# maxnorman569/Variational-Gridded-Gaussian-Processes

Hardware: AMD Instinct MI355X
Metric: ELBO-step grid-points/sec (value + 5-component gradient), 1024x1024 RBF grid per GPU (higher is better)
Workload: dtype f64; 1 GPU; 2D Kronecker rbf GP (points basis), 1024x1024 grid (1024x1024 per GPU), m_d=128, Adam fit loop (lr 0.01), eigensolver warm start on; parallelism=single GPU

## Files before the change

### variational_gridded_gaussian_processes_amd/build.py

```python
from __future__ import annotations

import os
import shutil
import subprocess
import sys

HERE = os.path.dirname(os.path.abspath(__file__))
CSRC = os.path.join(HERE, "csrc")
SOURCES = ["api.hip", "gemm.hip", "factor_build.hip", "chol.hip", "trsm.hip", "eigh.hip", "mspace.hip", "thin.hip", "masked.hip", "comm.hip", "paired.hip"]
HEADERS = ["common.h", "ctx.h", "factor_elem.h", "gemm_body.h", os.path.join("..", "..", "include", "vggp.h")]
LIB = os.path.join(HERE, "libvggp_hip.so")


def _stale() -> bool:
    if not os.path.exists(LIB):
        return True
    t = os.path.getmtime(LIB)
    deps = [os.path.join(CSRC, s) for s in SOURCES] + [os.path.normpath(os.path.join(CSRC, h)) for h in HEADERS]
    return any(os.path.getmtime(d) > t for d in deps)


def build(force: bool = False, verbose: bool = False) -> str:
    if not force and not _stale():
        return LIB
    hipcc = shutil.which("hipcc") or "/opt/rocm/bin/hipcc"
    if not os.path.exists(hipcc):
        raise RuntimeError("hipcc not found: libvggp_hip.so cannot be built (ROCm toolchain required)")
    cmd = [hipcc, "--offload-arch=gfx950", "-O3", "-std=c++17", "-shared", "-fPIC", "-o", LIB + ".tmp"] + \
          [os.path.join(CSRC, s) for s in SOURCES] + ["-ldl"]
    if verbose:
        print(" ".join(cmd), file=sys.stderr)
    subprocess.run(cmd, check=True, cwd=CSRC)
    os.replace(LIB + ".tmp", LIB)
    return LIB


if __name__ == "__main__":
    print(build(force="--force" in sys.argv, verbose=True))
```

### variational_gridded_gaussian_processes_amd/csrc/api.hip

```cpp
#include "common.h"

#include <math.h>
#include <stdarg.h>
#include <stdio.h>
#include <stdlib.h>
#include <string.h>
#include <time.h>

#include <algorithm>
#include <vector>

static thread_local char g_err[512] = "";
void vg_set_error(const char* fmt, ...) {
    va_list ap;
    va_start(ap, fmt);
    vsnprintf(g_err, sizeof(g_err), fmt, ap);
    va_end(ap);
}
extern "C" const char* vggp_last_error(void) { return g_err; }
extern "C" int vggp_version(void) { return VGGP_VERSION; }

#include "ctx.h"
#include "factor_elem.h"
#define VG_CHOL_MAXJOBS_HOST 8
// ... 167 lines not shown
    c->P3 = b.take<double>(3 * m1 * m2);
    c->T3 = b.take<double>(3 * m1 * m2);
    for (int k = 0; k < 2; ++k) {
        VgDim& d = c->d[k];
        const long m = d.m;
        d.TM = b.take<double>(m * m);
        d.TH = b.take<double>(m * m);
        d.Qt = b.take<double>(m * m);
        d.QtPrev = b.take<double>(m * m);
        d.QtPrev2 = b.take<double>(m * m);
        d.U = b.take<double>(m * m);
        d.Ep = b.take<double>(m * m);
        d.Fp = b.take<double>(m * m);
        d.Wp = b.take<double>(m * m);
        d.Id = b.take<double>(m * m);
        d.Gw = b.take<double>(m * m);
        d.GH = b.take<double>(2 * m * m);
        d.Mk = b.take<double>(m * m);
    }
    c->payload_len = 2 * m2 * m2 + 3 * m1 * m2;
    c->payload = b.take<double>(c->payload_len + 8);
    for (int k = 0; k < 2; ++k) {
        VgDim& d = c->d[k];
        const long m = d.m;
        const int glen = (int)vg_grid_len(d.basis, m);
        d.grid = b.take<double>(glen);
        d.K0 = b.take<double>(m * m);
        d.dK0 = b.take<double>(m * m);
        d.L0 = b.take<double>(m * m);
        d.Linv0 = b.take<double>(m * m);
        d.Dinv0 = b.take<double>(((m + 15) / 16) * 256);
        if (m > 128) {
            d.Kc = b.take<double>(4 * m * m); d.Lc = b.take<double>(4 * m * m); d.Dc = b.take<double>(4 * ((m + 15) / 16) * 256);
            d.st8 = b.take<int>(8);
        }
        d.X = b.take<double>(m * m);
        d.chol_scratch = b.take<double>(m * (m + 1));
        d.RQ = b.take<double>(m * m);
        d.RQsq = b.take<double>(m * m);
    }
    c->wq = b.take<double>(2 * m1 * m2);
    for (int k = 0; k < 2; ++k) {
        VgDim& d = c->d[k];
        const long m = d.m, n = d.n, m2e = m + (m & 1);
        d.x = b.take<double>(n);
        d.AD = b.take<double>(2 * m * n);
        d.BV = b.take<double>(2 * m * n);
        static const char* ghe = getenv("VGGP_GH_TARGET");
        d.gh_split = pick_split((int)(((m + 63) / 64) * ((m + 63) / 64)), (int)n, ghe ? atoi(ghe) : 32);
        d.GHslab = b.take<double>((size_t)d.gh_split * 2 * m * m);
        d.gwork = b.take<double>(m2e * (m2e + 1));
        d.max_rounds = (int)(VG_EIG_MAXSWEEP * (m2e - 1));
        d.rotlog = b.take<double2>(vg_eigh_log_bytes((int)m) / sizeof(double2) + 1);
        d.roundlog = b.take<int>(d.max_rounds);
        if (m >= 24 && m <= 256) {
            d.gwork2 = b.take<double>(m2e * (m2e + 1));
            d.rotlog2 = b.take<double2>(vg_eigh_log_bytes((int)m) / sizeof(double2) + 1);
            d.roundlog2 = b.take<int>(d.max_rounds);
            d.Zs = b.take<double>(m * m); d.V1s = b.take<double>(m * m); d.Hs = b.take<double>(m * m); d.Ws = b.take<double>(m * m);
            d.tMV = b.take<double>(VG_THIN_MAXR * m); d.tHV = b.take<double>(VG_THIN_MAXR * m);
            d.tAM = b.take<double>(VG_THIN_MAXR * VG_THIN_MAXR); d.tAH = b.take<double>(VG_THIN_MAXR * VG_THIN_MAXR);
            d.Omega = b.take<double>(VG_THIN_MAXR * m);
        }
    }
    const int st_tiles = (int)(((2 * m2 + 63) / 64) * ((n1 + 63) / 64));
    static const char* ste = getenv("VGGP_ST_TARGET");
    c->st_split = pick_split(st_tiles, (int)n2, ste ? atoi(ste) : 256);
    c->St = b.take<double>((size_t)std::max(c->st_split, VG_SP_SLABS) * 2 * m2 * n1);
    c->Sp = b.take<double>((size_t)VG_SP_SLABS * 2 * m2 * n1);
    const int cc_tiles = (int)(((2 * m1 + 63) / 64) * ((m2 + 63) / 64));
    const char* cce = getenv("VGGP_CC_TARGET");
    c->cc_split = pick_split(cc_tiles, (int)n1, cce ? atoi(cce) : 64);
    c->CCslab = b.take<double>((size_t)c->cc_split * 3 * m1 * m2);
    c->tCV = b.take<double>(3 * m1 * VG_THIN_MAXR);
    c->tAC = b.take<double>(3 * VG_THIN_MAXR * VG_THIN_MAXR + 64);
}

static int check_dim(int kind, int basis, long n, long m, const char* which) {
    VG_REQUIRE(kind >= 0 && kind <= 3, "vggp_plan: bad kind for %s", which);
    VG_REQUIRE(basis >= 0 && basis <= 4, "vggp_plan: bad basis for %s", which);
    VG_REQUIRE(!((basis == VGGP_BASIS_VFF || basis == VGGP_BASIS_B1) && kind != VGGP_KIND_MATERN12),
               "vggp_plan: the VFF and B1 features exist for Matern-1/2 only (%s)", which);
    VG_REQUIRE(!(basis == VGGP_BASIS_VFF && (m < 3 || (m & 1) == 0)), "vggp_plan: VFF needs m = 2M + 1 >= 3 (%s)", which);
    VG_REQUIRE(!(basis == VGGP_BASIS_B1 && m < 2), "vggp_plan: B1 needs at least 2 knots (%s)", which);
    VG_REQUIRE(!(basis == VGGP_BASIS_B0 && kind != VGGP_KIND_MATERN12),
               "vggp_plan: the B0 basis exists for Matern-1/2 only (%s)", which);
    VG_REQUIRE(n >= 1, "vggp_plan: %s has no observations", which);
    VG_REQUIRE(m >= 1 && m <= 256, "vggp_plan: m=%ld for %s outside [1, 256]", m, which);
    VG_REQUIRE(!(basis == VGGP_BASIS_ONE && m != 1), "vggp_plan: BASIS_ONE needs m=1 (%s)", which);
    return VGGP_OK;
}

extern "C" int vggp_plan(vggp_ctx* c, const vggp_desc* desc) {
    if (!c || !desc) { vg_set_error("vggp_plan: null argument"); return VGGP_EINVAL; }
    VG_ENTER_DEVICE(c->device);
    int rc;
    if (desc->flags & VGGP_FLAG_PAIRED_Z) {
        c->planned = false;
        graphs_clear(c);
        VG_HIP(hipDeviceSynchronize());
        c->have_partials = c->have_step = c->have_masked = false;
        c->acc_valid = false; c->last_payload = nullptr;
        c->is_paired = false;
        if ((rc = vg_paired_plan(c, desc))) return rc;
        c->desc = *desc;
        c->desc.x1 = c->desc.x2 = c->desc.grid1 = c->desc.grid2 = nullptr;
        c->desc.n_total = (desc->flags & VGGP_FLAG_SCATTERED) ? desc->n1 : desc->n1 * desc->n2;
        c->payload_len = 0;
        c->is_paired = true;
        c->planned = true;
        return VGGP_OK;
    }
    if (c->is_paired || c->paired) { VG_HIP(hipDeviceSynchronize()); vg_paired_free(c); c->is_paired = false; }
    if ((rc = check_dim(desc->kind1, desc->basis1, desc->n1, desc->m1, "dimension 1"))) return rc;
    if ((rc = check_dim(desc->kind2, desc->basis2, desc->n2, desc->m2, "dimension 2"))) return rc;
    VG_REQUIRE(desc->x1 && desc->x2, "vggp_plan: null coordinate arrays");
    VG_REQUIRE((desc->basis1 == VGGP_BASIS_ONE || desc->grid1) && (desc->basis2 == VGGP_BASIS_ONE || desc->grid2),
               "vggp_plan: null grid arrays");
    if (desc->flags & VGGP_FLAG_SCATTERED)
        VG_REQUIRE(desc->n1 == desc->n2 && desc->basis1 != VGGP_BASIS_ONE && desc->basis2 != VGGP_BASIS_ONE,
                   "vggp_plan: scattered points need n1 == n2 (one coordinate pair per point) and two real dimensions");
    else
        VG_REQUIRE(desc->n_total >= desc->n1 * desc->n2, "vggp_plan: n_total smaller than the local grid");
    VG_REQUIRE(desc->n1 < (1L << 24) && desc->n2 < (1L << 24), "vggp_plan: grid axis too long");
    c->planned = false;
    graphs_clear(c);
    VG_HIP(hipDeviceSynchronize());
    c->warm_run = 0;
    c->refine_next = false;
    c->sub_next = false; c->sub_mode = false; c->sub_r_cap[0] = c->sub_r_cap[1] = 0;
    c->pred_consumed = false;
    c->acc_valid = false; c->last_warm = false; c->last_slabs = false; c->last_payload = nullptr;
    c->last_thin = false; c->thin_off = false; c->thin_block = 0;
    c->cur_newton = 0; c->last_newton = false; c->newton_next = false; c->newton_block = 0; c->newton_iters = 3; c->newton_ok_run = 0;
    c->desc = *desc;
    c->d[0] = VgDim();
    c->d[1] = VgDim();
    c->d[0].kind = desc->kind1; c->d[0].basis = desc->basis1; c->d[0].n = (int)desc->n1; c->d[0].m = (int)desc->m1;
    c->d[1].kind = desc->kind2; c->d[1].basis = desc->basis2; c->d[1].n = (int)desc->n2; c->d[1].m = (int)desc->m2;
    Bump dry{nullptr, 0, true};
    layout(c, dry);
    const size_t need = dry.off + 4096;
    if (need > c->arena_bytes) {
        if (c->arena) { VG_HIP(hipFree(c->arena)); c->arena = nullptr; c->arena_bytes = 0; }
        VG_HIP(hipMalloc(&c->arena, need));
        c->arena_bytes = need;
    }
    Bump wet{reinterpret_cast<char*>(c->arena), 0, false};
    layout(c, wet);
    c->arena_used = wet.off;
    VG_HIP(hipMemset(c->arena, 0, c->arena_used));
    const double one = 1.0;
    for (int k = 0; k < 2; ++k) {
        VgDim& d = c->d[k];
        const double* hx = k == 0 ? desc->x1 : desc->x2;
        const double* hg = k == 0 ? desc->grid1 : desc->grid2;
        VG_HIP(hipMemcpy(d.x, hx, sizeof(double) * d.n, hipMemcpyHostToDevice));
        if (d.basis == VGGP_BASIS_ONE) {
            VG_HIP(hipMemcpy(d.grid, &one, sizeof(double), hipMemcpyHostToDevice));
        } else {
            const int glen = (int)vg_grid_len(d.basis, d.m);
            VG_HIP(hipMemcpy(d.grid, hg, sizeof(double) * glen, hipMemcpyHostToDevice));
        }
    }
    for (int k = 0; k < 2; ++k) VG_HIP(vg_identity_launch(c->d[k].Id, c->d[k].m, nullptr));
    for (int k = 0; k < 2; ++k) {
        VgDim& d = c->d[k];
        if (!d.Omega) continue;
        std::vector<double> om((size_t)VG_THIN_MAXR * d.m);
        unsigned long long z = 0x9E3779B97F4A7C15ull * (unsigned long long)(k + 1);
        for (double& v : om) {
            z += 0x9E3779B97F4A7C15ull;
            unsigned long long x = z;
            x = (x ^ (x >> 30)) * 0xBF58476D1CE4E5B9ull; x = (x ^ (x >> 27)) * 0x94D049BB133111EBull; x ^= x >> 31;
            v = (double)(x >> 11) * (2.0 / 9007199254740992.0) - 1.0;
        }
        VG_HIP(hipMemcpy(d.Omega, om.data(), sizeof(double) * om.size(), hipMemcpyHostToDevice));
    }
    VG_HIP(hipDeviceSynchronize());
    c->desc.x1 = c->desc.x2 = c->desc.grid1 = c->desc.grid2 = nullptr;
    c->have_partials = c->have_step = c->have_masked = false;
    vg_masked_new_plan(c);
    c->planned = true;
    return VGGP_OK;
}

extern "C" int vggp_set_inducing(vggp_ctx* c, int dim, const double* z, int64_t m) {
    if (c && c->is_paired) {
        if (!c->planned) { vg_set_error("context not planned"); return VGGP_ESTATE; }
        VG_ENTER_DEVICE(c->device);
        return vg_paired_set_inducing(c, dim, z, m);
    }
    if (!c || !c->planned) { vg_set_error("vggp_set_inducing: context not planned"); return VGGP_ESTATE; }
    VG_REQUIRE(dim == 0 || dim == 1, "vggp_set_inducing: dim must be 0 or 1");
    VgDim& d = c->d[dim];
    VG_REQUIRE(d.basis == VGGP_BASIS_POINTS, "vggp_set_inducing: dimension %d does not use the points basis", dim + 1);
    VG_REQUIRE(z && m == d.m, "vggp_set_inducing: expected %d coordinates, got %lld", d.m, (long long)m);
    for (int64_t i = 0; i < m; ++i) VG_REQUIRE(std::isfinite(z[i]), "vggp_set_inducing: z[%lld] is not finite", (long long)i);
    VG_ENTER_DEVICE(c->device);
    VG_HIP(hipStreamSynchronize(c->own_stream));
    VG_HIP(hipMemcpy(d.grid, z, sizeof(double) * m, hipMemcpyHostToDevice));
    c->have_step = false; c->have_partials = false; c->have_masked = false; c->acc_valid = false;
    return VGGP_OK;
}

extern "C" int64_t vggp_payload_len(const vggp_ctx* c) { return (c && c->planned) ? c->payload_len : 0; }
extern "C" int64_t vggp_workspace_bytes(const vggp_ctx* c) { return c ? (int64_t)c->arena_used : 0; }

static int trsm_batch(const VgTrsmSpec* sp, int n, hipStream_t st) {
    int max_nblk = 0;
    for (int j = 0; j < n; ++j) max_nblk = std::max(max_nblk, (int)((sp[j].m + VG_TRSM_BLK - 1) / VG_TRSM_BLK));
    for (int s = 0; s < max_nblk; ++s) {
        VgGemmBatch g;
        vg_gemm_init(&g);
        VgTrsmJob tj[12];
        int nt = 0;
        for (int j = 0; j < n; ++j) {
            const VgTrsmSpec& q = sp[j];
            const int nblk = (int)((q.m + VG_TRSM_BLK - 1) / VG_TRSM_BLK);
            if (s >= nblk) continue;
            const int b = q.trans ? nblk - 1 - s : s;
            const long r0 = (long)b * VG_TRSM_BLK, rb = std::min<long>(VG_TRSM_BLK, q.m - r0), r1 = r0 + rb;
            const long k0 = q.trans ? r1 : 0, kn = q.trans ? q.m - r1 : r0;
            if (kn > 0) {
                const double* Tp = q.trans ? q.L + k0 * q.ldl + r0 : q.L + r0 * q.ldl + k0;
                const long t_i = q.trans ? 1 : q.ldl, t_k = q.trans ? q.ldl : 1;
                if (q.sc == 1)
                    vg_gemm_add(&g, Tp, t_i, t_k, q.X + k0 * q.sk, q.sk, 1, q.X + r0 * q.sk, (int)q.sk, (int)rb, (int)q.ncols, (int)kn,
                                1, 0, 1, 0, -1.0, 1);
                else
                    vg_gemm_add(&g, q.X + k0, q.sc, 1, Tp, t_k, t_i, q.X + r0, (int)q.sc, (int)q.ncols, (int)rb, (int)kn, 1, 0, 1, 0,
                                -1.0, 1);
            }
            if (nt >= 12) { vg_set_error("trsm_batch: too many jobs"); return VGGP_EINVAL; }
            tj[nt++] = VgTrsmJob{q.L + r0 * q.ldl + r0, q.Dinv + (r0 / 16) * q.dinv_blk, q.X + r0 * q.sk, q.X + r0 * q.sk, q.ldl,
                                 q.dinv_blk, q.dinv_ld, q.sk, q.sc, q.sk, q.sc, q.ncols, (int)rb, q.trans};
        }
        if (g.nprob) VG_HIP(vg_gemm_launch(&g, st));
        if (nt) VG_HIP(vg_trsm_launch(tj, nt, st));
    }
    return VGGP_OK;
}
static int trsm_inplace(const double* L, long m, long ldl, const double* Dinv, double* X, long x_sk, long x_sc, long ncols,
                        int trans, hipStream_t st) {
    VgTrsmSpec q{L, ldl, Dinv, 256, 16, X, x_sk, x_sc, ncols, m, trans};
    return trsm_batch(&q, 1, st);
}

static bool vg_ride(const vggp_ctx* c) {
    static const bool off = getenv("VGGP_NO_RIDE") != nullptr;
    return !off && !c->prof && c->desc.m1 <= 128 && c->desc.m2 <= 128;
}

static int vg_chol_big_enqueue(vggp_ctx* c, const int* dims, int ndims, hipStream_t st) {
    VgCholJob cj[VG_CHOL_MAXJOBS_HOST];
    int nj = 0;
    for (int t = 0; t < ndims; ++t) {
        VgDim& d = c->d[dims[t]];
        VG_HIP(vg_jitcopy_launch(d.K0, d.m, d.Kc, st));
    }
    const long NB = 128;
    for (int stage = 0; stage < 2; ++stage) {
        if (stage == 1) {
            VgTrsmJob tj[8];
            int nt = 0;
            VgGemmBatch g;
            vg_gemm_init(&g);
            for (int t = 0; t < ndims; ++t) {
                VgDim& d = c->d[dims[t]];
                const long m = d.m, mm = m * m, rest = m - NB, nb16 = (m + 15) / 16;
                for (int l = 0; l < 4; ++l) {
                    double* Kl = d.Kc + l * mm;
                    double* Ll = d.Lc + l * mm;
                    tj[nt++] = VgTrsmJob{Ll, d.Dc + l * nb16 * 256, Kl + NB * m, Ll + NB * m, m, 256, 16, 1, m, 1, m, rest, (int)NB, 0};
                    vg_gemm_add(&g, Ll + NB * m, m, 1, Ll + NB * m, 1, m, Kl + NB * m + NB, (int)m, (int)rest, (int)rest, (int)NB, 1, 0, 1, 0, -1.0, 1);
                }
            }
            VG_HIP(vg_trsm_launch(tj, nt, st));
            VG_HIP(vg_gemm_launch(&g, st));
        }
        nj = 0;
        for (int t = 0; t < ndims; ++t) {
            VgDim& d = c->d[dims[t]];
            const long m = d.m, mm = m * m, nb16 = (m + 15) / 16;
            const long o = stage ? NB : 0;
            const int mb = stage ? (int)(m - NB) : (int)NB;
            for (int l = 0; l < 4; ++l) {
                VgCholJob j{d.Kc + l * mm + o * m + o, d.Lc + l * mm + o * m + o, nullptr, d.chol_scratch, nullptr, d.st8 + 2 * l + stage, mb};
                j.ldk = (int)m; j.ldl = (int)m; j.only_level0 = 1;
                j.Dinv_out = d.Dc + l * nb16 * 256 + (o / 16) * 256;
                cj[nj++] = j;
            }
        }
        VG_HIP(vg_chol_launch(cj, nj, st));
    }
    for (int t = 0; t < ndims; ++t) {
        VgDim& d = c->d[dims[t]];
        VG_HIP(vg_cholsel_launch(d.Lc, d.Dc, d.st8, d.m, d.L0, d.Dinv0, d.jitter, d.status, st));
    }
    return VGGP_OK;
}

int vg_partials_enqueue(vggp_ctx* c, const double* Y, double* payload, hipStream_t st, bool reduce, bool extrap, bool fused, bool apply_ns,
                        int early) {
    const long n1 = c->desc.n1, n2 = c->desc.n2, m1 = c->desc.m1, m2 = c->desc.m2;
    VgDim &d1 = c->d[0], &d2 = c->d[1];
    hipStream_t sx = vg_side(c, st);
    VgGemmBatch g;
    VG_MARK(-1);

    VgFactorJob fj[2];
    VgCholJob cj[2];
    static const bool chol_legacy = getenv("VGGP_CHOL_LEGACY") != nullptr;
    const bool dinv_path = d1.m <= VG_TRSM_BLK && d2.m <= VG_TRSM_BLK && !chol_legacy;
    VgClearArgs clr;
    clr.n = 0;
    for (int k = 0; k < 2; ++k) {
        VgDim& d = c->d[k];
        fj[k] = VgFactorJob{d.x, d.grid, d.AD, d.AD + (long)d.m * d.n, d.K0, d.dK0, d.n, d.m, d.kind, d.basis, k, 0.0, c->desc.flags};
        clr.ptr[clr.n] = d.status; clr.nwords[clr.n++] = 2;
        clr.ptr[clr.n] = reinterpret_cast<int*>(d.chol_scratch); clr.nwords[clr.n++] = 16;
        clr.ptr[clr.n] = d.counters; clr.nwords[clr.n++] = 8;
        if (k == 0) { clr.ptr[clr.n] = reinterpret_cast<int*>(c->payload + c->payload_len); clr.nwords[clr.n++] = 2; }
        if (d.st8) { clr.ptr[clr.n] = d.st8; clr.nwords[clr.n++] = 8; }
        cj[k] = VgCholJob{d.K0, d.L0, dinv_path ? nullptr : d.Linv0, d.chol_scratch, d.jitter, d.status, d.m};
        cj[k].Dinv_out = d.Dinv0;
    }
    VG_HIP(vg_factor_build_launch(fj, 2, c->d_htheta, st, c->theta, &clr));
    VG_MARK(0);

    const bool ns_on_chol = extrap && apply_ns && dinv_path;
    VgGemmBatch gns;
    vg_gemm_init(&gns);
    if (ns_on_chol)
        for (int k = 0; k < 2; ++k) {
            VgDim& d = c->d[k];
            vg_gemm_add(&gns, d.Wp, d.m, 1, d.Ep, d.m, 1, d.Fp, d.m, d.m, d.m, d.m, 1, 0, 1, 0, -0.5, 1);
        }
    static const bool chol_big_off = getenv("VGGP_NO_CHOL_BIG") != nullptr;
    const bool any_big = (d1.m > VG_TRSM_BLK || d2.m > VG_TRSM_BLK) && !chol_legacy && !chol_big_off;
    VgGemmBatch gsp;
    vg_gemm_init(&gsp);
    int sp_slabs = 1;
    if (early) {
        const bool ok_fused = fused && !reduce && (vg_ride(c) || c->prof);
        const bool ok_partials = reduce;
        if (!(dinv_path && !any_big && (ok_fused || ok_partials) && Y && sx == st)) {
            vg_set_error("internal: the early projection was requested where it cannot run");
            return VGGP_ESTATE;
        }
        vg_gemm_add(&gsp, d2.AD, n2, 1, Y, n1, 1, c->Sp, (int)n1, (int)(2 * m2), (int)n1, (int)n2, std::min(c->st_split, VG_SP_SLABS), 2L * m2 * n1);
        sp_slabs = gsp.p[0].ksplit;
        if (c->prof) {
            vg_gemm_xcd_group(&gsp, 0);
            VG_HIP(vg_gemm_launch(&gsp, st, VG_GEMM_TAG_GRAM_PROJECT));
            VG_MARK(4);
        }
    }
    if (!any_big) {
        VgGemmBatch gr2 = gns;
        if (early && !c->prof) {
            gr2 = gsp;
            if (ns_on_chol)
                for (int k = 0; k < 2; ++k) {
                    VgDim& d = c->d[k];
                    vg_gemm_add(&gr2, d.Wp, d.m, 1, d.Ep, d.m, 1, d.Fp, d.m, d.m, d.m, d.m, 1, 0, 1, 0, -0.5, 1);
                }
        }
        VG_HIP(vg_chol_launch(cj, 2, st, ((early && !c->prof) || ns_on_chol) ? &gr2 : nullptr));
    } else {
        int big[2], nbig = 0;
        for (int k = 0; k < 2; ++k) {
            if (c->d[k].m > VG_TRSM_BLK) big[nbig++] = k;
            else { cj[k].Linv = nullptr; VG_HIP(vg_chol_launch(&cj[k], 1, st)); }
        }
        const int rcb = vg_chol_big_enqueue(c, big, nbig, st);
        if (rcb) return rcb;
    }
    c->dinv_valid = dinv_path || any_big;
    VG_MARK(1);

    {
        const bool big = d1.m > VG_TRSM_BLK || d2.m > VG_TRSM_BLK;
        if (!big) {
            VgTrsmJob tj[16];
            int nt = 0;
            for (int k = 0; k < 2; ++k) {
                VgDim& d = c->d[k];
                const long mn = (long)d.m * d.n;
                const double* dv = dinv_path ? d.Dinv0 : d.Linv0;
                const long dblk = dinv_path ? 256 : 16L * d.m + 16, dld = dinv_path ? 16 : d.m;
                for (int b = 0; b < 2; ++b)
                    tj[nt++] = VgTrsmJob{d.L0, dv, d.AD + b * mn, d.BV + b * mn, d.m, dblk, dld, d.n, 1, d.n, 1, d.n, d.m, 0};
                tj[nt++] = VgTrsmJob{d.L0, dv, d.dK0, d.X, d.m, dblk, dld, d.m, 1, d.m, 1, d.m, d.m, 0};
                if (dinv_path) {
                    tj[nt] = VgTrsmJob{d.L0, dv, d.L0, d.Linv0, d.m, dblk, dld, d.m, 1, d.m, 1, d.m, d.m, 0};
                    tj[nt++].rhs_ident = 1;
                }
            }
            if (early)
                for (int sl = 0; sl < sp_slabs; ++sl)
                    for (int b = 0; b < 2; ++b) {
                        const long o = (long)sl * 2 * m2 * n1 + (long)b * m2 * n1;
                        tj[nt++] = VgTrsmJob{d2.L0, d2.Dinv0, c->Sp + o, c->St + o, m2, 256, 16, n1, 1, n1, 1, n1, (int)m2, 0};
                    }
            VG_HIP(vg_trsm_launch(tj, nt, st));
        } else {
            VgTrsmSpec q[8];
            int nq = 0;
            for (int k = 0; k < 2; ++k) {
                VgDim& d = c->d[k];
                const long mn = (long)d.m * d.n;
                const double* dv = any_big ? d.Dinv0 : d.Linv0;
                const long dblk = any_big ? 256 : 16L * d.m + 16, dld = any_big ? 16 : d.m;
                VG_HIP(hipMemcpyAsync(d.BV, d.AD, sizeof(double) * 2 * mn, hipMemcpyDeviceToDevice, st));
                VG_HIP(hipMemcpyAsync(d.X, d.dK0, sizeof(double) * d.m * d.m, hipMemcpyDeviceToDevice, st));
                for (int b = 0; b < 2; ++b) q[nq++] = VgTrsmSpec{d.L0, d.m, dv, dblk, dld, d.BV + b * mn, d.n, 1, d.n, d.m, 0};
                q[nq++] = VgTrsmSpec{d.L0, d.m, dv, dblk, dld, d.X, d.m, 1, d.m, d.m, 0};
                if (any_big) {
                    VG_HIP(hipMemcpyAsync(d.Linv0, d.Id, sizeof(double) * d.m * d.m, hipMemcpyDeviceToDevice, st));
                    q[nq++] = VgTrsmSpec{d.L0, d.m, dv, dblk, dld, d.Linv0, d.m, 1, d.m, d.m, 0};
                }
            }
            const int rc = trsm_batch(q, nq, st);
            if (rc) return rc;
        }
    }
    VG_MARK(2);

    if (!Y) {
        vg_gemm_init(&g);
        for (int k = 0; k < 2; ++k) {
            VgDim& d = c->d[k];
            vg_gemm_add(&g, d.X, d.m, 1, d.Linv0, 1, d.m, d.Mk, d.m, d.m, d.m, d.m);
        }
        VG_HIP(vg_gemm_launch(&g, st));
        return VGGP_OK;
    }
    hipStream_t sp = (fused && !extrap) ? sx : st;
    const bool ride = fused && !reduce && sp == st && vg_ride(c);
    if (sp != st) VG_FORK(1);
    VgGemmBatch gp, gc;
    vg_gemm_init(&gp);
    vg_gemm_add(&gp, d2.BV, n2, 1, Y, n1, 1, c->St, (int)n1, (int)(2 * m2), (int)n1, (int)n2, c->st_split, 2L * m2 * n1);
    const int st_slabs = early ? sp_slabs : gp.p[0].ksplit;
    vg_gemm_xcd_group(&gp, 0);
    auto add_ns = [&](VgGemmBatch* b) {
        if (extrap && apply_ns && !ns_on_chol)
            for (int k = 0; k < 2; ++k) {
                VgDim& d = c->d[k];
                vg_gemm_add(b, d.Wp, d.m, 1, d.Ep, d.m, 1, d.Fp, d.m, d.m, d.m, d.m, 1, 0, 1, 0, -0.5, 1);
            }
    };
    if (!ride && !early) {
        add_ns(&gp);
        VG_HIP(vg_gemm_launch(&gp, sp, VG_GEMM_TAG_GRAM_PROJECT));
        if (sp == st) VG_MARK(4);
    }
    vg_gemm_init(&gc);
    const long cc_slab = 3L * m1 * m2;
    vg_gemm_add(&gc, d1.BV, n1, 1, c->St, 1, n1, c->CCslab, (int)m2, (int)(2 * m1), (int)m2, (int)n1, c->cc_split, cc_slab,
                st_slabs, 2L * m2 * n1);
    vg_gemm_add(&gc, d1.BV, n1, 1, c->St + m2 * n1, 1, n1, c->CCslab + 2 * m1 * m2, (int)m2, (int)m1, (int)m2, (int)n1,
                c->cc_split, cc_slab, st_slabs, 2L * m2 * n1);
    const int cc_slabs = gc.p[0].ksplit;
    int gh_slabs[2] = {1, 1};
    auto add_gram = [&](VgGemmBatch* b) {
        for (int k = 0; k < 2; ++k) {
            VgDim& d = c->d[k];
            const int ig = vg_gemm_add(b, d.BV, d.n, 1, d.BV, 1, d.n, d.GHslab, d.m, 2 * d.m, d.m, d.n, d.gh_split, 2L * d.m * d.m);
            gh_slabs[k] = b->p[ig].ksplit;
            vg_gemm_add(b, d.X, d.m, 1, d.Linv0, 1, d.m, d.Mk, d.m, d.m, d.m, d.m);
        }
    };
    if (ride) {
        vg_gemm_init(&g);
        add_gram(&g);
        add_ns(&g);
        VG_HIP(vg_gemm_launch(&g, st));
        c->ride_proj = gp; c->ride_cc = gc;
        c->ride_pending = early != 1;
        c->ride_stage0 = early == 2 ? 1 : 0;
    } else {
        if (sp == st) add_gram(&gc);
        VG_HIP(vg_gemm_launch(&gc, sp));
        if (sp == st) { VG_MARK(5); VG_MARK(6); }
        if (sp != st) {
            VG_JOIN_RECORD(1);
            vg_gemm_init(&g);
            add_gram(&g);
            VG_HIP(vg_gemm_launch(&g, st));
            VG_MARK(6);
        }
    }

    c->gh_slabs[0] = gh_slabs[0]; c->gh_slabs[1] = gh_slabs[1]; c->cc_slabs = cc_slabs; c->st_slabs = st_slabs;
    if (!reduce) return VGGP_OK;
    if (sp != st) VG_JOIN_WAIT(1);
    VgRedBatch r;
    vg_red_init(&r);
    vg_red_add(&r, d1.GHslab, d1.GH, 2L * m1 * m1, 2L * m1 * m1, gh_slabs[0]);
    vg_red_add(&r, d2.GHslab, payload, 2L * m2 * m2, 2L * m2 * m2, gh_slabs[1]);
    vg_red_add(&r, c->CCslab, payload + 2 * m2 * m2, 3L * m1 * m2, cc_slab, cc_slabs);
    VG_HIP(vg_red_launch(&r, st));
    VG_MARK(7);
    return VGGP_OK;
}

static bool vg_sub_ident() { static const bool ex = getenv("VGGP_SUB_EXTRAP") != nullptr; return !ex; }

static int finish_enqueue(vggp_ctx* c, const double* payload, double yy_total, bool warm, hipStream_t st, bool copy_theta,
                          bool from_slabs = false, bool extrap = false, bool refine = false, bool subspace = false, bool thin = false,
                          int newton = 0, bool thin_early = false) {
    if (copy_theta) VG_HIP(hipMemcpyAsync(c->theta, c->h_theta, 6 * sizeof(double), hipMemcpyHostToDevice, st));
    const long m1 = c->desc.m1, m2 = c->desc.m2;
    VgDim &d1 = c->d[0], &d2 = c->d[1];
    const double* G0[2] = {from_slabs ? d1.GHslab : d1.GH, from_slabs ? d2.GHslab : payload};
    const double* H0[2] = {G0[0] + m1 * m1, G0[1] + m2 * m2};
    const double* C3 = from_slabs ? c->CCslab : payload + 2 * m2 * m2;
    const int ghn[2] = {from_slabs ? c->gh_slabs[0] : 1, from_slabs ? c->gh_slabs[1] : 1};
    const long ghs[2] = {2L * m1 * m1, 2L * m2 * m2};
    const int ccn = from_slabs ? c->cc_slabs : 1;
    const long ccs = 3L * m1 * m2;
    VgGemmBatch g;
    const bool ride = from_slabs && c->ride_pending;
    int ride_stage = ride ? c->ride_stage0 : 0;

    hipStream_t sx = vg_side(c, st);
    VG_MARK(-1);
    const double* Hr[2] = {H0[0], H0[1]};
    int hrn[2] = {ghn[0], ghn[1]};
    VgEigJob ej[2];
    if (warm && subspace && thin) {
        const bool early = thin_early && !ride;
        const double* Gr[2] = {G0[0], G0[1]};
        int grn[2] = {ghn[0], ghn[1]};
        double* gdst[2] = {d1.GH, c->payload};
        vg_gemm_init(&g);
        for (int k = 0; k < 2; ++k) {
            VgDim& d = c->d[k];
            vg_gemm_add(&g, d.QtPrev, d.m, 1, G0[k], d.m, 1, d.TM, d.m, d.sub_r, d.m, d.m, 1, 0, ghn[k], ghs[k]);
            if (from_slabs && ghn[k] > 1) {
                vg_gemm_add(&g, d.Id, d.m, 1, G0[k], d.m, 1, gdst[k], d.m, d.m, d.m, d.m, 1, 0, ghn[k], ghs[k]);
                vg_gemm_add(&g, d.Id, d.m, 1, H0[k], d.m, 1, gdst[k] + (long)d.m * d.m, d.m, d.m, d.m, d.m, 1, 0, ghn[k], ghs[k]);
            }
        }
        VG_HIP(vg_gemm_launch(&g, st));
        VG_MARK(8);
        for (int k = 0; k < 2; ++k)
            if (from_slabs && ghn[k] > 1) { Gr[k] = gdst[k]; grn[k] = 1; Hr[k] = gdst[k] + (long)c->d[k].m * c->d[k].m; hrn[k] = 1; }
        VgRowQrJob qj[2];
        for (int k = 0; k < 2; ++k) { VgDim& d = c->d[k]; qj[k] = VgRowQrJob{d.TM, d.V1s, d.sub_r, d.m, nullptr, nullptr, 0}; }
        VG_HIP(vg_rowqr_launch(qj, 2, st, early ? ((c->prof || !from_slabs) ? nullptr : &c->ride_cc) : (ride ? &c->ride_proj : nullptr)));
        if (ride) ride_stage = 1;
        VG_MARK(9);
        vg_gemm_init(&g);
        for (int k = 0; k < 2; ++k) {
            VgDim& d = c->d[k];
            const int r = d.sub_r;
            vg_gemm_add(&g, d.V1s, d.m, 1, Gr[k], d.m, 1, d.Zs, d.m, r, d.m, d.m, 1, 0, grn[k], ghs[k]);
            vg_gemm_add(&g, d.V1s, d.m, 1, d.Mk, d.m, 1, d.tMV, d.m, r, d.m, d.m);
            vg_gemm_add(&g, d.V1s, d.m, 1, Hr[k], d.m, 1, d.tHV, d.m, r, d.m, d.m, 1, 0, hrn[k], ghs[k]);
        }
        if (early) {
            const int ic = vg_gemm_add(&g, C3, m2, 1, d2.V1s, 1, m2, c->tCV, d2.sub_r, (int)(3 * m1), d2.sub_r, (int)m2);
            g.p[ic].a_nslab = ccn; g.p[ic].a_slab = ccs;
        }
        VG_HIP(vg_gemm_launch(&g, st));
        VG_MARK(10);
        VgGemmBatch gx;
        vg_gemm_init(&gx);
        if (ride) gx = c->ride_cc;
        for (int k = 0; k < 2; ++k) {
            VgDim& d = c->d[k];
            const int r = d.sub_r;
            vg_gemm_add(&gx, d.tMV, d.m, 1, d.V1s, 1, d.m, d.tAM, r, r, r, d.m);
            vg_gemm_add(&gx, d.tHV, d.m, 1, d.V1s, 1, d.m, d.tAH, r, r, r, d.m);
        }
        if (early)
            for (int q = 0; q < 3; ++q)
                vg_gemm_add(&gx, d1.V1s, m1, 1, c->tCV + (long)q * m1 * d2.sub_r, d2.sub_r, 1, c->tAC + (long)q * d1.sub_r * d2.sub_r,
                            d2.sub_r, d1.sub_r, d2.sub_r, (int)m1);
        VgEigJob sj[2];
        for (int k = 0; k < 2; ++k) {
            VgDim& d = c->d[k];
            sj[k] = VgEigJob{nullptr, d.lam_s, d.Ws, nullptr, d.gwork2, d.rotlog2, d.roundlog2, d.counters2, d.sub_r, d.max_rounds,
                             (long)vg_eigh_log_bytes(d.m), 0};
            sj[k].Hl = d.Zs; sj[k].Hr = d.V1s; sj[k].hk = d.m;
            sj[k].perm = d.perm2;
            sj[k].err = d.status + 1;
            sj[k].newton = 1;
        }
        VG_HIP(vg_eigh_launch(sj, 2, st, &gx));
        if (ride) ride_stage = 2;
        c->ride_pending = false;
        VG_MARK(11);
        const int ac_nslab = 1;
        const long ac_slab = 3L * d1.sub_r * d2.sub_r;
        if (!early) {
            vg_gemm_init(&g);
            {
                const int ic = vg_gemm_add(&g, C3, m2, 1, d2.V1s, 1, m2, c->tCV, d2.sub_r, (int)(3 * m1), d2.sub_r, (int)m2);
                g.p[ic].a_nslab = ccn; g.p[ic].a_slab = ccs;
            }
            for (int k = 0; k < 2; ++k) {
                VgDim& d = c->d[k];
                vg_gemm_add(&g, d.Ws, d.sub_r, 1, d.V1s, d.m, 1, d.QtPrev, d.m, d.sub_r, d.m, d.sub_r);
            }
            VG_HIP(vg_gemm_launch(&g, st));
            VG_MARK(14);
            vg_gemm_init(&g);
            for (int q = 0; q < 3; ++q)
                vg_gemm_add(&g, d1.V1s, m1, 1, c->tCV + (long)q * m1 * d2.sub_r, d2.sub_r, 1, c->tAC + (long)q * d1.sub_r * d2.sub_r, d2.sub_r,
                            d1.sub_r, d2.sub_r, (int)m1);
            VG_HIP(vg_gemm_launch(&g, st));
            VG_MARK(15);
        }
        VgThinTail tt{};
        tt.theta = c->theta; tt.n_total = (double)c->desc.n_total; tt.yy = yy_total;
        tt.r1 = d1.sub_r; tt.r2 = d2.sub_r; tt.m1 = (int)m1; tt.m2 = (int)m2;
        tt.W1 = d1.Ws; tt.W2 = d2.Ws; tt.lam1 = d1.lam_s; tt.lam2 = d2.lam_s;
        tt.AM1 = d1.tAM; tt.AH1 = d1.tAH; tt.AM2 = d2.tAM; tt.AH2 = d2.tAH; tt.AC = c->tAC;
        tt.ac_nslab = ac_nslab; tt.ac_slab = ac_slab;
        tt.G1 = Gr[0]; tt.H1 = Hr[0]; tt.G2 = Gr[1]; tt.H2 = Hr[1];
        tt.out = c->out; tt.hout = c->d_hout;
        tt.beta_out = c->beta; tt.invd_out = c->invD;
        tt.peer_fail = (payload == c->payload && (c->n_ranks > 1 || c->comm || c->cb)) ? c->payload + c->payload_len : nullptr;
        for (int k = 0; k < 2; ++k) { tt.jit[k] = c->d[k].jitter; tt.status[k] = c->d[k].status; tt.rcounters[k] = c->d[k].counters2; }
#ifdef VGGP_DIAG
        tt.stamps = reinterpret_cast<unsigned long long*>(c->tAC + 3 * VG_THIN_MAXR * VG_THIN_MAXR);
#endif
        VG_HIP(vg_thin_tail_launch(&tt, st));
        VG_MARK(18);
        if (early) {
            vg_gemm_init(&g);
            for (int k = 0; k < 2; ++k) {
                VgDim& d = c->d[k];
                vg_gemm_add(&g, d.Ws, d.sub_r, 1, d.V1s, d.m, 1, d.QtPrev, d.m, d.sub_r, d.m, d.sub_r);
            }
            VG_HIP(vg_gemm_launch(&g, st));
        }
        return VGGP_OK;
    }
    if (warm && subspace) {
        VgRowQrJob qj[2];
        const double* Gr[2] = {G0[0], G0[1]};
        int grn[2] = {ghn[0], ghn[1]};
        double* gdst[2] = {d1.GH, c->payload};
        vg_gemm_init(&g);
        for (int k = 0; k < 2; ++k) {
            VgDim& d = c->d[k];
            vg_gemm_add(&g, d.Fp, d.m, 1, G0[k], d.m, 1, d.TM, d.m, d.m, d.m, d.m, 1, 0, ghn[k], ghs[k]);
            if (from_slabs && ghn[k] > 1) {
                vg_gemm_add(&g, d.Id, d.m, 1, G0[k], d.m, 1, gdst[k], d.m, d.m, d.m, d.m, 1, 0, ghn[k], ghs[k]);
                vg_gemm_add(&g, d.Id, d.m, 1, H0[k], d.m, 1, gdst[k] + (long)d.m * d.m, d.m, d.m, d.m, d.m, 1, 0, ghn[k], ghs[k]);
            }
        }
        VG_HIP(vg_gemm_launch(&g, st));
        VG_MARK(8);
        for (int k = 0; k < 2; ++k)
            if (from_slabs && ghn[k] > 1) { Gr[k] = gdst[k]; grn[k] = 1; Hr[k] = gdst[k] + (long)c->d[k].m * c->d[k].m; hrn[k] = 1; }
        for (int k = 0; k < 2; ++k) {
            VgDim& d = c->d[k];
            const long r = d.sub_r;
            qj[k] = VgRowQrJob{d.TM, d.V1s, d.sub_r, d.m, d.Fp + r * d.m, d.E + r * d.m, (long)(d.m - r) * d.m};
        }
        VG_HIP(vg_rowqr_launch(qj, 2, st, ride ? &c->ride_proj : nullptr));
        if (ride) ride_stage = 1;
        VG_MARK(9);
        vg_gemm_init(&g);
        for (int k = 0; k < 2; ++k) {
            VgDim& d = c->d[k];
// ... 282 lines not shown
        const int idot[4] = {
            vg_gemm_add(&g, d1.E, 1, m1, c->beta, m2, 1, nullptr, (int)m2, (int)m1, (int)m2, (int)m1),
            vg_gemm_add(&g, d1.F, 1, m1, c->bl2, m2, 1, nullptr, (int)m2, (int)m1, (int)m2, (int)m1),
            vg_gemm_add(&g, c->beta, m2, 1, d2.E, m2, 1, nullptr, (int)m2, (int)m1, (int)m2, (int)m2),
            vg_gemm_add(&g, c->bl1, m2, 1, d2.F, m2, 1, nullptr, (int)m2, (int)m1, (int)m2, (int)m2)};
        for (int q = 0; q < 4; ++q) { g.p[idot[q]].dotw = c->beta; g.p[idot[q]].dotw_ld = (int)m2; g.p[idot[q]].dot_out = c->dotpart + 64 * q; }
        vg_gemm_add(&g, c->ol, m1, 1, c->invD, m2, 1, c->r2, (int)m2, 2, (int)m2, (int)m1);
    }
    if (predict)
        for (int k = 0; k < 2; ++k) {
            VgDim& d = c->d[k];
            vg_gemm_add(&g, d.Ep, d.m, 1, d.Ep, 1, d.m, d.Wp, d.m, d.m, d.m, d.m);
        }
    VG_HIP(vg_gemm_launch(&g, st));
    VG_MARK(17);
    VG_HIP(vg_final_launch(&ms, st));
    VG_MARK(18);

    return VGGP_OK;
}

enum { VG_G_PARTIALS = 0, VG_G_PARTIALS_X, VG_G_FINISH_COLD, VG_G_FINISH_WARM, VG_G_FINISH_WARM_X, VG_G_STEP_COLD, VG_G_STEP_WARM,
       VG_G_STEP_WARM_X, VG_G_FINISH_WARM_XR, VG_G_STEP_WARM_XR, VG_G_FINISH_WARM_S, VG_G_STEP_WARM_S, VG_G_FINISH_WARM_T, VG_G_STEP_WARM_T,
       VG_G_FINISH_WARM_N, VG_G_STEP_WARM_N, VG_G_PARTIALS_E, VG_G_FINISH_WARM_TE, VG_G_STEP_COLD_T, VG_G_PARTIALS_XE, VG_G_COUNT };
static_assert(VG_G_COUNT <= 20, "vggp_ctx::gexec");

static void graphs_clear(vggp_ctx* c) {
    (void)vg_quiesce(c);
    for (int i = 0; i < VG_G_COUNT; ++i) {
        if (c->gexec[i]) { (void)hipGraphExecDestroy(c->gexec[i]); c->gexec[i] = nullptr; }
        c->gkey[i] = VgGraphKey();
    }
}

template <typename F>
static int run_graph(vggp_ctx* c, int which, const VgGraphKey& key, hipStream_t st, F enqueue, bool bypass = false) {
    if (!c->use_graph || c->prof || bypass) return enqueue();
    if (!c->gexec[which] || !(c->gkey[which] == key)) {
        if (c->gexec[which]) { (void)vg_quiesce(c); (void)hipGraphExecDestroy(c->gexec[which]); c->gexec[which] = nullptr; }
        VG_HIP(hipStreamBeginCapture(st, hipStreamCaptureModeThreadLocal));
        const int rc = enqueue();
        hipGraph_t graph = nullptr;
        const hipError_t e = hipStreamEndCapture(st, &graph);
        if (rc) { if (graph) (void)hipGraphDestroy(graph); return rc; }
        if (e != hipSuccess) { vg_set_error("hipStreamEndCapture -> %s", hipGetErrorString(e)); return VGGP_EHIP; }
        const hipError_t ei = hipGraphInstantiate(&c->gexec[which], graph, nullptr, nullptr, 0);
        (void)hipGraphDestroy(graph);
        if (ei != hipSuccess) { c->gexec[which] = nullptr; vg_set_error("hipGraphInstantiate -> %s", hipGetErrorString(ei)); return VGGP_EHIP; }
        c->gkey[which] = key;
    }
    VG_HIP(hipGraphLaunch(c->gexec[which], st));
    return VGGP_OK;
}

static bool vg_refine(const vggp_ctx* c, bool extrap) {
    static const bool off = getenv("VGGP_NO_REFINE") != nullptr;
    return !off && extrap && c->refine_next;
}

static bool vg_extrapolate(const vggp_ctx* c) {
    static const bool off = getenv("VGGP_NO_EXTRAP") != nullptr;
    return !off && c->desc.warm_start && !(c->desc.flags & VGGP_FLAG_BLOCK_JACOBI) && c->d[0].have_prev && c->d[1].have_prev &&
           c->d[0].have_prev2 && c->d[1].have_prev2;
}

struct VgStart { bool extrap, refine, subspace, thin; int newton; };
static bool vg_thin_ok(const vggp_ctx* c, bool own_payload) {
    static const bool off = getenv("VGGP_NO_THIN") != nullptr;
    if (off || c->thin_off || c->thin_block > 0 || !own_payload || !c->desc.warm_start || (c->desc.flags & VGGP_FLAG_BLOCK_JACOBI) || !c->sub_next) return false;
    for (int k = 0; k < 2; ++k) {
        const VgDim& d = c->d[k];
        if (!d.have_prev || !d.tMV || d.sub_r < 1 || d.sub_r > VG_THIN_MAXR || d.sub_r > d.thin_rows) return false;
    }
    return true;
}
static bool vg_warm(vggp_ctx* c, bool own_payload) {
    bool warm = c->desc.warm_start && c->d[0].have_prev && c->d[1].have_prev;
    if (warm && (c->d[0].thin_rows < c->d[0].m || c->d[1].thin_rows < c->d[1].m) && !vg_thin_ok(c, own_payload)) {
        c->warm_run = 0;
        for (int k = 0; k < 2; ++k) c->d[k].have_prev = c->d[k].have_prev2 = false;
        warm = false;
    }
    return warm;
}
static int vg_start_prepare(vggp_ctx* c, bool warm, hipStream_t st, VgStart* out, bool own_payload) {
    out->thin = warm && vg_thin_ok(c, own_payload);
    out->extrap = !out->thin && vg_extrapolate(c);
    const bool lds_sized = c->d[0].m <= 128 && c->d[1].m <= 128;
    out->subspace = out->thin || (lds_sized && warm && out->extrap && c->sub_next && c->d[0].sub_r > 0 && c->d[1].sub_r > 0);
    {
        static const bool off = getenv("VGGP_NO_NEWTON_CHAIN") != nullptr;
        static const char* ite = getenv("VGGP_NEWTON_ITERS");
        const bool big = c->d[0].m > 128 || c->d[1].m > 128;
        const bool roomy = c->d[0].m >= 96 && c->d[1].m >= 96;
        const bool want = warm && !out->subspace && out->extrap && !off && c->newton_block == 0 && (big || (c->newton_next && roomy)) &&
                          !(c->desc.flags & VGGP_FLAG_BLOCK_JACOBI) && c->d[0].m >= 8 && c->d[1].m >= 8;
        out->newton = want ? (ite ? atoi(ite) : c->newton_iters) : 0;
        if (c->newton_block > 0) --c->newton_block;
    }
    out->refine = warm && !out->subspace && !out->newton && vg_refine(c, out->extrap);
    c->sub_mode = out->subspace;
    if (out->subspace && (c->sub_r_cap[0] != c->d[0].sub_r || c->sub_r_cap[1] != c->d[1].sub_r)) {
        for (int v : {(int)VG_G_FINISH_WARM_S, (int)VG_G_STEP_WARM_S, (int)VG_G_FINISH_WARM_T, (int)VG_G_STEP_WARM_T, (int)VG_G_FINISH_WARM_TE})
            if (c->gexec[v]) { (void)vg_quiesce(c); (void)hipGraphExecDestroy(c->gexec[v]); c->gexec[v] = nullptr; c->gkey[v] = VgGraphKey(); }
        c->sub_r_cap[0] = c->d[0].sub_r; c->sub_r_cap[1] = c->d[1].sub_r;
    }
    if (out->newton && out->newton != c->newton_cap) {
        for (int v : {(int)VG_G_FINISH_WARM_N, (int)VG_G_STEP_WARM_N})
            if (c->gexec[v]) { (void)vg_quiesce(c); (void)hipGraphExecDestroy(c->gexec[v]); c->gexec[v] = nullptr; c->gkey[v] = VgGraphKey(); }
        c->newton_cap = out->newton;
    }
    c->cur_thin = out->thin;
    c->cur_extrap = out->extrap;
    c->cur_newton = out->newton;
    c->cur_r[0] = c->d[0].sub_r; c->cur_r[1] = c->d[1].sub_r;
    return VGGP_OK;
}

static int set_theta(vggp_ctx* c, const double theta[5]) {
    for (int i = 0; i < 5; ++i) {
        VG_REQUIRE(theta[i] > 0.0 && std::isfinite(theta[i]), "theta[%d]=%g must be positive and finite", i, theta[i]);
        c->h_theta[i] = theta[i];
    }
    c->h_theta[5] = (double)(++c->seq);
    return VGGP_OK;
}

static int vg_quiesce(vggp_ctx* c) {
    if (c->poll_stream_valid) { c->poll_stream_valid = false; VG_HIP(hipStreamSynchronize(c->poll_stream)); }
    return VGGP_OK;
}
static int vg_wait_step(vggp_ctx* c, hipStream_t st) {
    static const bool nopoll = getenv("VGGP_NO_POLL") != nullptr;
    const volatile double* seq = &c->h_out->seq;
    const double want = c->h_theta[5];
    if (nopoll || c->prof || (c->n_ranks > 1 && !c->comm && !c->cb)) { c->poll_stream_valid = false; return vg_comm_wait(c, st); }
    if (c->comm && !c->cb) {
        const int wrc = vg_comm_wait(c, st, seq, want);
        c->poll_stream = st; c->poll_stream_valid = (wrc == VGGP_OK);
        return wrc;
    }
    timespec t0, t1;
    clock_gettime(CLOCK_MONOTONIC, &t0);
    for (long spin = 0;; ++spin) {
        if (*seq == want) {
            __atomic_thread_fence(__ATOMIC_ACQUIRE);
            c->poll_stream = st; c->poll_stream_valid = true;
            return VGGP_OK;
        }
        __builtin_ia32_pause();
        if ((spin & 4095) == 4095) {
            clock_gettime(CLOCK_MONOTONIC, &t1);
            if ((double)(t1.tv_sec - t0.tv_sec) + 1e-9 * (double)(t1.tv_nsec - t0.tv_nsec) > 0.02) break;
        }
    }
    c->poll_stream_valid = false;
    VG_HIP(hipStreamSynchronize(st));
    return VGGP_OK;
}

static int finish_collect(vggp_ctx* c, double* elbo_out, double grad_out[5], vggp_info* info, hipStream_t st) {
    {
        const int wrc = vg_wait_step(c, st);
        if (wrc) {
            c->warm_run = 0;
            for (int k = 0; k < 2; ++k) c->d[k].have_prev = c->d[k].have_prev2 = false;
            c->have_step = false;
            return wrc;
        }
    }
    c->pred_consumed = false;
    c->acc_valid = false;
    if (c->prof && c->nev > 1) {
        for (int i = 1; i < c->nev; ++i) {
            const int id = c->ev_stage[i];
            float ms = 0.f;
            if (id >= 0 && id < VGGP_NSTAGE && hipEventElapsedTime(&ms, c->ev[i - 1], c->ev[i]) == hipSuccess) c->prof_ms[id] += ms;
        }
        c->prof_steps++;
    }
    c->nev = 0;
    if (c->h_out->seq != c->h_theta[5]) {
        vg_set_error("step %.0f: the result block carries sequence number %.0f (stale results)", c->h_theta[5], c->h_out->seq);
        c->warm_run = 0;
        for (int k = 0; k < 2; ++k) c->d[k].have_prev = c->d[k].have_prev2 = false;
        c->have_step = false;
        return VGGP_ESTATE;
    }
    if (c->h_out->out[6] != 0.0) {
        vg_set_error("rank %d / %d: %.0f rank(s) of the job failed their half of this step; the result is discarded", c->rank,
                     c->n_ranks, c->h_out->out[6]);
        c->warm_run = 0;
        for (int k = 0; k < 2; ++k) c->d[k].have_prev = c->d[k].have_prev2 = false;
        c->have_step = false;
        return VGGP_ERCCL;
    }
    *elbo_out = c->h_out->out[0];
    for (int i = 0; i < 5; ++i) grad_out[i] = c->h_out->out[1 + i];
    int status = 0;
    for (int k = 0; k < 2; ++k) {
        if (c->h_out->status[k]) status = c->h_out->status[k];
        else if (c->h_out->counters[k][2]) status = c->h_out->counters[k][2];
    }
    if (info) {
        info->jitter1 = c->h_out->jitter[0]; info->jitter2 = c->h_out->jitter[1];
        info->sweeps1 = c->h_out->counters[0][1] & 0xff; info->sweeps2 = c->h_out->counters[1][1] & 0xff;
        info->rounds1 = c->h_out->counters[0][0]; info->rounds2 = c->h_out->counters[1][0];
        info->status = status;
        info->polished = ((c->h_out->counters[0][3] >> 28) & 1) | (((c->h_out->counters[1][3] >> 28) & 1) << 1);
    }
    {
        static const bool off = getenv("VGGP_NO_SUBSPACE") != nullptr;
        bool ok = !status && !off && c->desc.warm_start && !(c->desc.flags & VGGP_FLAG_BLOCK_JACOBI);
        for (int k = 0; k < 2; ++k) {
            VgDim& d = c->d[k];
            const int rank = (c->h_out->counters[k][1] >> 8) & 0x1ff;
            int want = 0;
            static const bool relax = getenv("VGGP_NO_SUB_RELAX") == nullptr;
            if (d.Zs && rank >= 1 && 3 * rank <= d.m) {
                static const bool m8 = getenv("VGGP_SUB_MARGIN8") != nullptr;
                want = m8 ? ((rank + 4 + 7) / 8) * 8 : ((rank + 3 + 1) / 2) * 2;
                if (want < 16) want = 16;
                if (want > 64 || 2 * want > d.m) want = 0;
            } else if (relax && d.Zs && rank >= 1 && d.m <= 64 && rank + 2 <= d.m - 8) {
                want = ((rank + 2 + 3) / 4) * 4;
                if (want > d.m - 8) want = d.m - 8;
                if (want < 8 || want > 48) want = 0;
            }
            if (d.m > 128 && want > VG_THIN_MAXR) want = 0;
            if (want == 0) d.sub_r = 0;
            else if (want > d.sub_r || want < d.sub_r - 8) d.sub_r = want;
            ok = ok && d.sub_r > 0;
        }
        c->sub_next = ok;
    }
    c->refine_next = !status && ((c->h_out->counters[0][3] >> 28) & 1) && ((c->h_out->counters[1][3] >> 28) & 1) &&
                     (c->h_out->counters[0][1] & 0xff) <= 1 && (c->h_out->counters[1][1] & 0xff) <= 1;
    if (status == VG_ESUBMISS && c->cur_newton) {
        static const bool dbg = getenv("VGGP_NEWTON_DBG") != nullptr;
        if (dbg)
            fprintf(stderr, "[vggp] step %ld: Newton chain (%d iterations) missed: dim1 flags %d, 10 log10(offdiag / thr) = %d; dim2 flags %d, %d\n",
                    c->seq, c->cur_newton, c->h_out->counters[0][3] & 0xff, (c->h_out->counters[0][3] >> 8) - 100,
                    c->h_out->counters[1][3] & 0xff, (c->h_out->counters[1][3] >> 8) - 100);
        c->newton_block = (c->d[0].m > 128 || c->d[1].m > 128) ? 2 : 16; c->newton_next = false;
        if (c->newton_iters < 5) ++c->newton_iters;
        c->newton_ok_run = 0;
        c->have_step = false;
        return VG_ESUBMISS;
    }
    if (status) {
        c->warm_run = 0;
        for (int k = 0; k < 2; ++k) c->d[k].have_prev = c->d[k].have_prev2 = false;
        c->have_step = false;
    }
    if (status == VG_ESUBMISS) {
        c->sub_next = false;
        if (c->cur_thin) c->thin_block = 32;
        return VG_ESUBMISS;
    }
    if (status == VGGP_ENOTPD) { vg_set_error("a Kuu factor is not positive definite after jitter 1e-6"); return VGGP_ENOTPD; }
    if (status == VGGP_ENOCONV) { vg_set_error("Jacobi eigensolver did not converge"); return VGGP_ENOCONV; }
    for (int k = 0; k < 2; ++k) {
        c->d[k].have_prev2 = c->d[k].have_prev;
        c->d[k].have_prev = true;
        c->d[k].thin_rows = c->cur_thin ? c->cur_r[k] : c->d[k].m;
    }
    c->last_thin = c->cur_thin;
    if (c->thin_block > 0) --c->thin_block;
    c->last_newton = c->cur_newton > 0;
    if (c->cur_newton > 0 && ++c->newton_ok_run >= 64) {
        c->newton_ok_run = 0;
        if (c->newton_iters > 3) --c->newton_iters;
    }
    {
        const bool polished = ((c->h_out->counters[0][3] >> 28) & 1) && ((c->h_out->counters[1][3] >> 28) & 1);
        c->newton_next = c->cur_newton > 0 ||
                         (c->last_warm && c->cur_extrap && !c->cur_thin && !polished && (c->h_out->counters[0][0] + c->h_out->counters[1][0]) > 0) ||
                         (c->last_warm && c->cur_extrap && !c->cur_thin && c->d[0].m >= 96 && c->d[1].m >= 96 &&
                          (2 * c->h_out->counters[0][0] >= 3 * c->d[0].m || 2 * c->h_out->counters[1][0] >= 3 * c->d[1].m));
    }
    if (++c->warm_run >= 512) {
        c->warm_run = 0;
        for (int k = 0; k < 2; ++k) c->d[k].have_prev = c->d[k].have_prev2 = false;
    }
    c->have_step = true;
    return VGGP_OK;
}

extern "C" int vggp_elbo_partials(vggp_ctx* c, const double* Y, const double theta[5], double* payload, void* stream) {
    VG_NOT_PAIRED(c, "vggp_elbo_partials");
    if (!c || !c->planned) { vg_set_error("vggp_elbo_partials: context not planned"); return VGGP_ESTATE; }
    VG_REQUIRE(Y && theta && payload, "vggp_elbo_partials: null argument");
    VG_ENTER_DEVICE(c->device);
    hipStream_t st = stream ? (hipStream_t)stream : c->own_stream;
    int rc = set_theta(c, theta);
    if (rc) return rc;
    c->nev = 0;
    const VgGraphKey key{Y, payload, 0.0};
    VgStart sp;
    if ((rc = vg_start_prepare(c, vg_warm(c, false), st, &sp, false))) return rc;
    const bool extrap = sp.extrap;
    const bool apply_ns = extrap && !c->pred_consumed;
    rc = run_graph(c, extrap ? VG_G_PARTIALS_X : VG_G_PARTIALS, key, st,
                   [&] { return vg_partials_enqueue(c, Y, payload, st, true, extrap, false, apply_ns); }, extrap && !apply_ns);
    if (rc) return rc;
    if (extrap) c->pred_consumed = true;
    c->have_partials = true;
    return VGGP_OK;
}

static int elbo_finish_once(vggp_ctx* c, const double* payload, double yy_total, const double theta[5],
                            double* elbo_out, double grad_out[5], vggp_info* info, void* stream);
extern "C" int vggp_elbo_finish(vggp_ctx* c, const double* payload, double yy_total, const double theta[5],
                                double* elbo_out, double grad_out[5], vggp_info* info, void* stream) {
    VG_NOT_PAIRED(c, "vggp_elbo_finish");
    int rc = elbo_finish_once(c, payload, yy_total, theta, elbo_out, grad_out, info, stream);
    if (rc == VG_ESUBMISS) rc = elbo_finish_once(c, payload, yy_total, theta, elbo_out, grad_out, info, stream);
    if (rc == VG_ESUBMISS) { vg_set_error("the eigensolver chain failed twice on the same step"); rc = VGGP_ENOCONV; }
    return rc;
}

static int elbo_finish_once(vggp_ctx* c, const double* payload, double yy_total, const double theta[5],
                            double* elbo_out, double grad_out[5], vggp_info* info, void* stream) {
    if (!c || !c->planned || !c->have_partials) { vg_set_error("vggp_elbo_finish: call vggp_elbo_partials first"); return VGGP_ESTATE; }
    VG_REQUIRE(payload && theta && elbo_out && grad_out, "vggp_elbo_finish: null argument");
    VG_ENTER_DEVICE(c->device);
    hipStream_t st = stream ? (hipStream_t)stream : c->own_stream;
    int rc = set_theta(c, theta);
    if (rc) return rc;
    const bool warm = vg_warm(c, false);
    const VgGraphKey key{nullptr, payload, yy_total};
    VgStart sp;
    if ((rc = vg_start_prepare(c, warm, st, &sp, false))) return rc;
    const bool extrap = sp.extrap, refine = sp.refine, subspace = sp.subspace;
    const int newton = sp.newton;
    rc = run_graph(c, warm ? (newton ? VG_G_FINISH_WARM_N : subspace ? VG_G_FINISH_WARM_S : extrap ? (refine ? VG_G_FINISH_WARM_XR : VG_G_FINISH_WARM_X) : VG_G_FINISH_WARM)
                            : VG_G_FINISH_COLD, key, st,
                   [&] { return finish_enqueue(c, payload, yy_total, warm, st, true, false, extrap, refine, subspace, false, newton); });
    if (rc) return rc;
    c->last_warm = warm; c->last_slabs = false; c->last_payload = payload; c->last_yy = yy_total;
    return finish_collect(c, elbo_out, grad_out, info, st);
}

#define VG_COLD_THIN_R 32
static bool vg_cold_thin_ok(const vggp_ctx* c) {
    static const bool off = getenv("VGGP_NO_COLD_THIN") != nullptr || getenv("VGGP_NO_THIN") != nullptr || getenv("VGGP_NO_SUBSPACE") != nullptr;
    if (off || c->thin_off || c->thin_block > 0 || c->prof || (c->desc.flags & (VGGP_FLAG_BLOCK_JACOBI | VGGP_FLAG_SCATTERED))) return false;
    if (c->n_ranks > 1 || c->comm || c->cb) return false;
    for (int k = 0; k < 2; ++k) {
        const VgDim& d = c->d[k];
        if (!d.Omega || !d.tMV || d.kind != VGGP_KIND_RBF || d.m < 3 * VG_COLD_THIN_R || d.m > 256) return false;
    }
    return true;
}
static int vg_cold_thin_prepass(vggp_ctx* c, const double* payload, hipStream_t st) {
    const double* Gk[2] = {c->d[0].GH, payload};
    VgPivCholJob pj[2];
    for (int k = 0; k < 2; ++k) { VgDim& d = c->d[k]; pj[k] = VgPivCholJob{Gk[k], d.Omega, d.TM, d.m, VG_COLD_THIN_R}; }
    VG_HIP(vg_pivchol_launch(pj, 2, st));
    VgRowQrJob qj[2];
    for (int k = 0; k < 2; ++k) { VgDim& d = c->d[k]; qj[k] = VgRowQrJob{d.TM, d.QtPrev, VG_COLD_THIN_R, d.m, nullptr, nullptr, 0}; }
    VG_HIP(vg_rowqr_launch(qj, 2, st, nullptr));
    return VGGP_OK;
}

static int elbo_step_once(vggp_ctx* c, const double* Y, double yy_total, const double theta[5], double* elbo_out,
                          double grad_out[5], vggp_info* info, void* stream);
extern "C" int vggp_elbo_step(vggp_ctx* c, const double* Y, double yy_total, const double theta[5], double* elbo_out,
                              double grad_out[5], vggp_info* info, void* stream) {
    if (c && c->is_paired) {
        if (!c->planned) { vg_set_error("context not planned"); return VGGP_ESTATE; }
        VG_ENTER_DEVICE(c->device);
        return vg_paired_step(c, Y, yy_total, theta, elbo_out, grad_out, info, stream ? (hipStream_t)stream : c->own_stream, false);
    }
    if (c && c->planned && theta) {
        bool jump = false;
        for (int k = 0; k < 2; ++k) jump = jump || (c->last_ell[k] > 0.0 && std::fabs(theta[k] / c->last_ell[k] - 1.0) > 0.05);
        if (jump && c->sub_next) { c->warm_run = 0; for (int k = 0; k < 2; ++k) c->d[k].have_prev = c->d[k].have_prev2 = false; }
        c->last_ell[0] = theta[0]; c->last_ell[1] = theta[1];
    }
    int rc = elbo_step_once(c, Y, yy_total, theta, elbo_out, grad_out, info, stream);
    if (rc == VG_ESUBMISS) rc = elbo_step_once(c, Y, yy_total, theta, elbo_out, grad_out, info, stream);
    if (rc == VG_ESUBMISS) { vg_set_error("the eigensolver chain failed twice on the same step"); rc = VGGP_ENOCONV; }
    return rc;
}

static int elbo_step_once(vggp_ctx* c, const double* Y, double yy_total, const double theta[5], double* elbo_out,
                          double grad_out[5], vggp_info* info, void* stream) {
    if (!c || !c->planned) { vg_set_error("vggp_elbo_step: context not planned"); return VGGP_ESTATE; }
    if (c->desc.flags & VGGP_FLAG_SCATTERED) { vg_set_error("vggp_elbo_step: the context was planned for scattered points (use vggp_elbo_step_scattered)"); return VGGP_ESTATE; }
    VG_REQUIRE(Y && theta && elbo_out && grad_out, "vggp_elbo_step: null argument");
    VG_ENTER_DEVICE(c->device);
    hipStream_t st = stream ? (hipStream_t)stream : c->own_stream;
    int rc = set_theta(c, theta);
    if (rc) return rc;
    c->nev = 0;
    const bool warm = vg_warm(c, true);
    VgStart sp;
    if ((rc = vg_start_prepare(c, warm, st, &sp, true))) return rc;
    const bool extrap = sp.extrap, refine = sp.refine, subspace = sp.subspace, thin = sp.thin;
    const int newton = sp.newton;
    const bool apply_ns = extrap && !c->pred_consumed;
    if (c->n_ranks > 1 || c->comm || c->cb) {
        const VgGraphKey kp{Y, c->payload, 0.0}, kf{nullptr, c->payload, yy_total};
        static const bool no_early_mr = getenv("VGGP_NO_EARLY") != nullptr;
        const bool early_ok = !no_early_mr && !c->prof && c->desc.m1 <= 128 && c->desc.m2 <= 128 && vg_side(c, st) == st &&
                              getenv("VGGP_CHOL_LEGACY") == nullptr;
        const bool thin_early = thin && early_ok && !extrap;
        static const bool no_early_reg_mr = getenv("VGGP_NO_EARLY_REG") != nullptr;
        const bool early_mr = thin_early || (warm && !thin && !subspace && early_ok && !no_early_reg_mr);
        rc = run_graph(c, early_mr ? (extrap ? VG_G_PARTIALS_XE : VG_G_PARTIALS_E) : extrap ? VG_G_PARTIALS_X : VG_G_PARTIALS, kp, st,
                       [&] { return vg_partials_enqueue(c, Y, c->payload, st, true, extrap, false, apply_ns, early_mr ? 1 : 0); }, extrap && !apply_ns);
        {
            static const long fault_at = [] { const char* e = getenv("VGGP_FAULT_PARTIALS_AT"); return e ? atol(e) : -1L; }();
            if (!rc && fault_at >= 0 && c->seq == fault_at) { vg_set_error("injected fault in the partials of step %ld", c->seq); rc = VGGP_EHIP; }
        }
        if (rc) {
            char msg[512];
            snprintf(msg, sizeof(msg), "%s", vggp_last_error());
            static const double one = 1.0;
            hipStreamCaptureStatus cs = hipStreamCaptureStatusNone;
            if (hipStreamIsCapturing(st, &cs) == hipSuccess && cs != hipStreamCaptureStatusNone) { hipGraph_t gdrop = nullptr; (void)hipStreamEndCapture(st, &gdrop); if (gdrop) (void)hipGraphDestroy(gdrop); }
            (void)hipMemsetAsync(c->payload, 0, sizeof(double) * c->payload_len, st);
            (void)hipMemcpyAsync(c->payload + c->payload_len, &one, sizeof(double), hipMemcpyHostToDevice, st);
            if (vg_allreduce(c, c->payload, c->payload_len + 1, st) == VGGP_OK) (void)vg_comm_wait(c, st);
            else vg_comm_abort(c);
            c->warm_run = 0;
            for (int k = 0; k < 2; ++k) c->d[k].have_prev = c->d[k].have_prev2 = false;
            c->have_step = false;
            vg_set_error("%s", msg);
            return rc;
        }
        if (extrap) c->pred_consumed = true;
        c->have_partials = true;
        if ((rc = vg_allreduce(c, c->payload, c->payload_len + 1, st))) return rc;
        rc = run_graph(c, warm ? (thin ? (thin_early ? VG_G_FINISH_WARM_TE : VG_G_FINISH_WARM_T) : newton ? VG_G_FINISH_WARM_N : subspace ? VG_G_FINISH_WARM_S : extrap ? (refine ? VG_G_FINISH_WARM_XR : VG_G_FINISH_WARM_X) : VG_G_FINISH_WARM)
                                : VG_G_FINISH_COLD, kf, st,
                       [&] { return finish_enqueue(c, c->payload, yy_total, warm, st, false, false, extrap, refine, subspace, thin, newton, thin_early); });
        if (rc) return rc;
        c->last_warm = warm; c->last_slabs = false; c->last_payload = c->payload; c->last_yy = yy_total;
        return finish_collect(c, elbo_out, grad_out, info, st);
    }
    const VgGraphKey key{Y, c->payload, yy_total};
    static const bool no_early = getenv("VGGP_NO_EARLY") != nullptr;
    static const bool no_ride = getenv("VGGP_NO_RIDE") != nullptr;
    if (!warm && vg_cold_thin_ok(c)) {
        const bool early = !no_early && c->desc.m1 <= 128 && c->desc.m2 <= 128 && vg_side(c, st) == st && getenv("VGGP_CHOL_LEGACY") == nullptr;
        const int keep[2] = {c->d[0].sub_r, c->d[1].sub_r};
        c->d[0].sub_r = c->d[1].sub_r = VG_COLD_THIN_R;
        rc = run_graph(c, VG_G_STEP_COLD_T, key, st, [&] {
            int r1 = vg_partials_enqueue(c, Y, c->payload, st, true, false, true, false, early);
            if (!r1) r1 = vg_cold_thin_prepass(c, c->payload, st);
            return r1 ? r1 : finish_enqueue(c, c->payload, yy_total, true, st, false, false, false, false, true,
                                            true, 0, early);
        });
        c->d[0].sub_r = keep[0]; c->d[1].sub_r = keep[1];
        if (rc) return rc;
        c->cur_thin = true; c->cur_extrap = false; c->cur_newton = 0;
        c->cur_r[0] = c->cur_r[1] = VG_COLD_THIN_R;
        c->have_partials = true;
        c->last_warm = true;
        c->last_slabs = false; c->last_payload = c->payload; c->last_yy = yy_total;
        return finish_collect(c, elbo_out, grad_out, info, st);
    }
    const bool thin_early = thin && !no_early && !no_ride && c->desc.m1 <= 128 && c->desc.m2 <= 128 && vg_side(c, st) == st &&
                            getenv("VGGP_CHOL_LEGACY") == nullptr;
    static const bool no_early_reg = getenv("VGGP_NO_EARLY_REG") != nullptr;
    const bool early_reg = warm && !thin && !subspace && !no_early && !no_early_reg && !no_ride && c->desc.m1 <= 128 && c->desc.m2 <= 128 &&
                           vg_side(c, st) == st && getenv("VGGP_CHOL_LEGACY") == nullptr && (vg_ride(c) || c->prof);
    const int early_mode = thin_early ? 1 : (early_reg ? 2 : 0);
    rc = run_graph(c, warm ? (thin ? VG_G_STEP_WARM_T : newton ? VG_G_STEP_WARM_N : subspace ? VG_G_STEP_WARM_S : extrap ? (refine ? VG_G_STEP_WARM_XR : VG_G_STEP_WARM_X) : VG_G_STEP_WARM)
                            : VG_G_STEP_COLD, key, st, [&] {
        const int r1 = vg_partials_enqueue(c, Y, c->payload, st, !warm, extrap, true, apply_ns, early_mode);
        return r1 ? r1 : finish_enqueue(c, c->payload, yy_total, warm, st, false, warm, extrap, refine, subspace, thin, newton,
                                        thin_early);
    }, extrap && !apply_ns);
    if (rc) return rc;
    if (extrap) c->pred_consumed = true;
    c->have_partials = true;
    c->last_warm = warm; c->last_slabs = warm; c->last_payload = c->payload; c->last_yy = yy_total;
    return finish_collect(c, elbo_out, grad_out, info, st);
}

static int vg_accurate_state(vggp_ctx* c, hipStream_t st) {
    static const bool skip = getenv("VGGP_FAST_READOUT") != nullptr;
    if ((skip && !c->last_thin) || !c->last_warm || c->acc_valid || !c->have_step) return VGGP_OK;
    if (c->last_payload != c->payload) return VGGP_OK;
    const long m1 = c->desc.m1, m2 = c->desc.m2;
    if (c->last_slabs) {
        VgRedBatch r;
        vg_red_init(&r);
        vg_red_add(&r, c->d[0].GHslab, c->d[0].GH, 2L * m1 * m1, 2L * m1 * m1, c->gh_slabs[0]);
        vg_red_add(&r, c->d[1].GHslab, c->payload, 2L * m2 * m2, 2L * m2 * m2, c->gh_slabs[1]);
        vg_red_add(&r, c->CCslab, c->payload + 2 * m2 * m2, 3L * m1 * m2, 3L * m1 * m2, c->cc_slabs);
        VG_HIP(vg_red_launch(&r, st));
    }
    VgClearArgs clr;
    clr.n = 0;
    for (int k = 0; k < 2; ++k) { clr.ptr[clr.n] = c->d[k].counters; clr.nwords[clr.n++] = 8; clr.ptr[clr.n] = c->d[k].status + 1; clr.nwords[clr.n++] = 1; }
    VG_HIP(vg_clear_launch(&clr, st));
    const bool prof = c->prof;
    c->prof = false;
    const int rc = finish_enqueue(c, c->payload, c->last_yy, false, st, false);
    c->prof = prof;
    if (rc) return rc;
    VG_HIP(hipStreamSynchronize(st));
    int status = 0;
    for (int k = 0; k < 2; ++k) {
        if (c->h_out->status[k]) status = c->h_out->status[k];
        else if (c->h_out->counters[k][2]) status = c->h_out->counters[k][2];
    }
    if (status) { vg_set_error("accurate read-out: the cold eigensolve failed (status %d)", status); return status; }
    for (int k = 0; k < 2; ++k) { c->d[k].have_prev2 = false; c->d[k].thin_rows = c->d[k].m; }
    c->last_thin = false;
    c->pred_consumed = false;
    c->acc_valid = true;
    return VGGP_OK;
}

static bool vg_thin_readout(const vggp_ctx* c) {
    static const bool off = getenv("VGGP_NO_THIN_READOUT") != nullptr;
    return !off && c->have_step && c->last_thin && !c->acc_valid;
}
__global__ void vg_rowsq_kernel(const double* L, int m, double* out) {
    const int a = blockIdx.x * blockDim.x + threadIdx.x;
    if (a >= m) return;
    double s = 0.0;
    for (int k = 0; k <= a; ++k) s += L[(long)a * m + k] * L[(long)a * m + k];
    out[a] = s;
}
__global__ void vg_add_outer_kernel(double* x, const double* u, const double* v, int m1, int m2) {
    const long i = (long)blockIdx.x * blockDim.x + threadIdx.x;
    if (i < (long)m1 * m2) x[i] += u[i / m2] * v[i % m2];
}
static int vg_qv_thin(vggp_ctx* c, double* mean, double* var, hipStream_t st) {
    const long m1 = c->desc.m1, m2 = c->desc.m2;
    VgDim &d1 = c->d[0], &d2 = c->d[1];
    const int r1 = d1.thin_rows, r2 = d2.thin_rows;
    VgGemmBatch g;
    vg_gemm_init(&g);
    for (int k = 0; k < 2; ++k) {
        VgDim& d = c->d[k];
        vg_gemm_add(&g, d.L0, d.m, 1, d.QtPrev, 1, d.m, d.RQ, d.thin_rows, d.m, d.thin_rows, d.m);
    }
    VG_HIP(vg_gemm_launch(&g, st));
    for (int k = 0; k < 2; ++k) VG_HIP(vg_scale_sq_launch(c->d[k].RQ, c->d[k].RQsq, (long)c->d[k].m * c->d[k].thin_rows, st));
    VG_HIP(vg_qv_weights_launch(c->theta, c->beta, c->invD, c->wq, (long)r1 * r2, st, vg_uexp(d1.basis), vg_uexp(d2.basis)));
    vg_gemm_init(&g);
    vg_gemm_add(&g, d1.RQ, r1, 1, c->wq, r2, 1, c->T3, r2, (int)m1, r2, r1);
    vg_gemm_add(&g, d1.RQsq, r1, 1, c->wq + (long)r1 * r2, r2, 1, c->T3 + m1 * m2, r2, (int)m1, r2, r1);
    VG_HIP(vg_gemm_launch(&g, st));
    vg_gemm_init(&g);
    vg_gemm_add(&g, c->T3, r2, 1, d2.RQ, 1, r2, mean, (int)m2, (int)m1, (int)m2, r2);
    vg_gemm_add(&g, c->T3 + m1 * m2, r2, 1, d2.RQsq, 1, r2, var, (int)m2, (int)m1, (int)m2, r2);
    VG_HIP(vg_gemm_launch(&g, st));
    double* rs1 = c->rowpart;
    double* rs2 = c->r2;
    hipLaunchKernelGGL(vg_rowsq_kernel, dim3((unsigned)((m1 + 127) / 128)), dim3(128), 0, st, d1.L0, (int)m1, rs1);
    hipLaunchKernelGGL(vg_rowsq_kernel, dim3((unsigned)((m2 + 127) / 128)), dim3(128), 0, st, d2.L0, (int)m2, rs2);
    hipLaunchKernelGGL(vg_add_outer_kernel, dim3((unsigned)((m1 * m2 + 255) / 256)), dim3(256), 0, st, var, rs1, rs2, (int)m1, (int)m2);
    VG_HIP(hipGetLastError());
    VG_HIP(vg_scale_launch(var, m1 * m2, c->theta, 0, st, vg_uexp(d1.basis), vg_uexp(d2.basis)));
    return VGGP_OK;
}

static int build_RQ(vggp_ctx* c, hipStream_t st) {
    VgGemmBatch g;
    vg_gemm_init(&g);
    for (int k = 0; k < 2; ++k) {
        VgDim& d = c->d[k];
        vg_gemm_add(&g, d.L0, d.m, 1, d.QtPrev, 1, d.m, d.RQ, d.m, d.m, d.m, d.m);
    }
    VG_HIP(vg_gemm_launch(&g, st));
    for (int k = 0; k < 2; ++k) VG_HIP(vg_scale_sq_launch(c->d[k].RQ, c->d[k].RQsq, (long)c->d[k].m * c->d[k].m, st));
    return VGGP_OK;
}

extern "C" int vggp_qv(vggp_ctx* c, double* mean, double* var, void* stream) {
    VG_NOT_PAIRED(c, "vggp_qv");
    if (!c || !c->have_step) { vg_set_error("vggp_qv: no finished ELBO step"); return VGGP_ESTATE; }
    VG_REQUIRE(mean && var, "vggp_qv: null output");
    VG_ENTER_DEVICE(c->device);
    hipStream_t st = stream ? (hipStream_t)stream : c->own_stream;
    const long m1 = c->desc.m1, m2 = c->desc.m2;
    VgDim &d1 = c->d[0], &d2 = c->d[1];
    if (vg_thin_readout(c)) return vg_qv_thin(c, mean, var, st);
    int rc = vg_accurate_state(c, st);
    if (rc) return rc;
    if ((rc = build_RQ(c, st))) return rc;
    VG_HIP(vg_qv_weights_launch(c->theta, c->beta, c->invD, c->wq, m1 * m2, st, vg_uexp(d1.basis), vg_uexp(d2.basis)));
    VgGemmBatch g;
    vg_gemm_init(&g);
    vg_gemm_add(&g, d1.RQ, m1, 1, c->wq, m2, 1, c->T3, (int)m2, (int)m1, (int)m2, (int)m1);
    vg_gemm_add(&g, d1.RQsq, m1, 1, c->invD, m2, 1, c->T3 + m1 * m2, (int)m2, (int)m1, (int)m2, (int)m1);
    VG_HIP(vg_gemm_launch(&g, st));
    vg_gemm_init(&g);
    vg_gemm_add(&g, c->T3, m2, 1, d2.RQ, 1, m2, mean, (int)m2, (int)m1, (int)m2, (int)m2);
    vg_gemm_add(&g, c->T3 + m1 * m2, m2, 1, d2.RQsq, 1, m2, var, (int)m2, (int)m1, (int)m2, (int)m2);
    VG_HIP(vg_gemm_launch(&g, st));
    VG_HIP(vg_scale_launch(var, m1 * m2, c->theta, 0, st, vg_uexp(d1.basis), vg_uexp(d2.basis)));
    return VGGP_OK;
}

__global__ void vg_kron_rows_kernel(const double* R1, const double* R2, const double* w, int m1, int m2, double* Rk,
                                    double* Rs) {
    const long M = (long)m1 * m2;
    const long idx = (long)blockIdx.x * blockDim.x + threadIdx.x;
    if (idx >= M * M) return;
    const long row = idx / M, col = idx - row * M;
    const int a = (int)(row / m2), b = (int)(row - (long)a * m2);
    const int i1 = (int)(col / m2), i2 = (int)(col - (long)i1 * m2);
    const double v = R1[a * m1 + i1] * R2[b * m2 + i2];
    Rk[idx] = v;
    Rs[idx] = v * w[col];
}

extern "C" int vggp_qv_cov(vggp_ctx* c, double* cov, void* stream) {
    VG_NOT_PAIRED(c, "vggp_qv_cov");
    if (!c || !c->have_step) { vg_set_error("vggp_qv_cov: no finished ELBO step"); return VGGP_ESTATE; }
    VG_REQUIRE(cov, "vggp_qv_cov: null output");
    VG_ENTER_DEVICE(c->device);
    hipStream_t st = stream ? (hipStream_t)stream : c->own_stream;
    const long m1 = c->desc.m1, m2 = c->desc.m2, M = m1 * m2;
    VG_REQUIRE(M <= 8192, "vggp_qv_cov: M=%ld too large for a dense covariance (use vggp_qv for mean/variance)", M);
    int rc = vg_accurate_state(c, st);
    if (rc) return rc;
    if ((rc = build_RQ(c, st))) return rc;
    rc = vg_ensure_misc(c, 2 * M * M * sizeof(double));
    if (rc) return rc;
    double* Rk = (double*)c->misc;
    double* Rs = Rk + M * M;
    hipLaunchKernelGGL(vg_kron_rows_kernel, dim3((unsigned)((M * M + 255) / 256)), dim3(256), 0, st, c->d[0].RQ,
                       c->d[1].RQ, c->invD, (int)m1, (int)m2, Rk, Rs);
    VG_HIP(hipGetLastError());
    VgGemmBatch g;
    vg_gemm_init(&g);
    vg_gemm_add(&g, Rs, M, 1, Rk, 1, M, cov, (int)M, (int)M, (int)M, (int)M);
    VG_HIP(vg_gemm_launch(&g, st));
    VG_HIP(vg_scale_launch(cov, M * M, c->theta, 0, st, vg_uexp(c->d[0].basis), vg_uexp(c->d[1].basis)));
    return VGGP_OK;
}

extern "C" int vggp_posterior(vggp_ctx* c, const double* xs1, const double* xs2, int64_t ns, double* mean, double* var,
                              void* stream) {
    VG_NOT_PAIRED(c, "vggp_posterior");
    if (!c || !c->have_step) { vg_set_error("vggp_posterior: no finished ELBO step"); return VGGP_ESTATE; }
    VG_REQUIRE(xs1 && xs2 && mean && var && ns >= 0, "vggp_posterior: bad argument");
    VG_ENTER_DEVICE(c->device);
    hipStream_t st = stream ? (hipStream_t)stream : c->own_stream;
    const long m1 = c->desc.m1, m2 = c->desc.m2;
    const long chunk = std::min<long>(ns, 65536);
    if (ns == 0) return VGGP_OK;
    const size_t per = (size_t)chunk * (2 * m1 + 3 * m2 + 2 * m1) + (size_t)(m1 * m1 + m2 * m2);
    const bool thin_ro = vg_thin_readout(c);
    int rc = thin_ro ? VGGP_OK : vg_accurate_state(c, st);
    if (rc) return rc;
    const int q1 = thin_ro ? c->d[0].thin_rows : (int)m1, q2 = thin_ro ? c->d[1].thin_rows : (int)m2;
    if ((rc = vg_ensure_misc(c, per * sizeof(double)))) return rc;
    double* p = (double*)c->misc;
    double* A1 = p; p += m1 * chunk;
    double* T1 = p; p += m1 * chunk;
    double* A2 = p; p += m2 * chunk;
    double* T2 = p; p += m2 * chunk;
    double* T2sq = p; p += m2 * chunk;
    double* U = p; p += m1 * chunk;
    double* Uv = p; p += m1 * chunk;
    double* W1 = p; p += m1 * m1;
    double* W2 = p;
    VgDim &d1 = c->d[0], &d2 = c->d[1];
    VG_HIP(vg_qv_weights_launch(c->theta, c->beta, c->invD, c->wq, (long)q1 * q2, st));
    {
        VgGemmBatch g;
        vg_gemm_init(&g);
        vg_gemm_add(&g, d1.QtPrev, m1, 1, d1.Linv0, m1, 1, W1, (int)m1, q1, (int)m1, (int)m1);
        vg_gemm_add(&g, d2.QtPrev, m2, 1, d2.Linv0, m2, 1, W2, (int)m2, q2, (int)m2, (int)m2);
        VG_HIP(vg_gemm_launch(&g, st));
    }
    for (long off = 0; off < ns; off += chunk) {
        const int cn = (int)std::min<long>(chunk, ns - off);
        VgFactorJob fj[2] = {
            VgFactorJob{xs1 + off, d1.grid, A1, nullptr, nullptr, nullptr, cn, d1.m, d1.kind, d1.basis, 0, 0.0, c->desc.flags},
            VgFactorJob{xs2 + off, d2.grid, A2, nullptr, nullptr, nullptr, cn, d2.m, d2.kind, d2.basis, 1, 0.0, c->desc.flags}};
        VG_HIP(vg_factor_build_launch(fj, 2, c->theta, st));
        VgGemmBatch g;
        vg_gemm_init(&g);
        vg_gemm_add(&g, W1, m1, 1, A1, cn, 1, T1, cn, q1, cn, (int)m1);
        vg_gemm_add(&g, W2, m2, 1, A2, cn, 1, T2, cn, q2, cn, (int)m2);
        VG_HIP(vg_gemm_launch(&g, st));
        VG_HIP(vg_scale_sq_launch(T2, T2sq, (long)q2 * cn, st));
        vg_gemm_init(&g);
        vg_gemm_add(&g, c->wq, q2, 1, T2, cn, 1, U, cn, q1, cn, q2);
        vg_gemm_add(&g, c->wq + (long)q1 * q2, q2, 1, T2sq, cn, 1, Uv, cn, q1, cn, q2);
        VG_HIP(vg_gemm_launch(&g, st));
        VG_HIP(vg_post_combine_launch(c->theta, T1, U, Uv, nullptr, q1, q2, cn, mean + off, var + off, st));
    }
    return VGGP_OK;
}

__global__ void vg_khatri_rao_kernel(const double* U1, const double* U2, const double* w, int m1, int m2, long ns, double* T,
                                     double* Tw) {
    const long idx = (long)blockIdx.x * blockDim.x + threadIdx.x;
    const long total = (long)m1 * m2 * ns;
    if (idx >= total) return;
    const long u = idx / ns, p = idx - u * ns;
    const int i1 = (int)(u / m2), i2 = (int)(u - (long)i1 * m2);
    const double v = U1[(long)i1 * ns + p] * U2[(long)i2 * ns + p];
    T[idx] = v;
    if (Tw) Tw[idx] = v * w[u];
}
__global__ void vg_prior_cov_kernel(const double* xs1, const double* xs2, long ns, int kind1, int kind2, const double* theta,
                                    double* cov) {
    const long idx = (long)blockIdx.x * blockDim.x + threadIdx.x;
    if (idx >= ns * ns) return;
    const long p = idx / ns, q = idx - p * ns;
    double k1, k2, d;
    vg_kappa(kind1, fabs(xs1[p] - xs1[q]), 1.0 / theta[0], k1, d);
    vg_kappa(kind2, fabs(xs2[p] - xs2[q]), 1.0 / theta[1], k2, d);
    cov[idx] += theta[2] * theta[3] * k1 * k2;
}
hipError_t vg_prior_cov_launch(const double* xs1, const double* xs2, long ns, int kind1, int kind2, const double* theta,
                               double* cov, hipStream_t st) {
    hipLaunchKernelGGL(vg_prior_cov_kernel, dim3((unsigned)((ns * ns + 255) / 256)), dim3(256), 0, st, xs1, xs2, ns, kind1,
                       kind2, theta, cov);
    return hipGetLastError();
}

static int posterior_factors(vggp_ctx* c, const double* xs1, const double* xs2, int ns, double* A1, double* A2, double* U1,
                             double* U2, hipStream_t st, bool rotate) {
    VgDim &d1 = c->d[0], &d2 = c->d[1];
    VgFactorJob fj[2] = {
        VgFactorJob{xs1, d1.grid, A1, nullptr, nullptr, nullptr, ns, d1.m, d1.kind, d1.basis, 0, 0.0, c->desc.flags},
        VgFactorJob{xs2, d2.grid, A2, nullptr, nullptr, nullptr, ns, d2.m, d2.kind, d2.basis, 1, 0.0, c->desc.flags}};
    VG_HIP(vg_factor_build_launch(fj, 2, c->theta, st));
    VgTrsmSpec q[2] = {{d1.L0, d1.m, d1.Linv0, 16L * d1.m + 16, d1.m, A1, ns, 1, ns, d1.m, 0},
                       {d2.L0, d2.m, d2.Linv0, 16L * d2.m + 16, d2.m, A2, ns, 1, ns, d2.m, 0}};
    int rc = trsm_batch(q, 2, st);
    if (rc || !rotate) return rc;
    VgGemmBatch g;
    vg_gemm_init(&g);
    vg_gemm_add(&g, d1.QtPrev, d1.m, 1, A1, ns, 1, U1, ns, d1.m, ns, d1.m);
    vg_gemm_add(&g, d2.QtPrev, d2.m, 1, A2, ns, 1, U2, ns, d2.m, ns, d2.m);
    VG_HIP(vg_gemm_launch(&g, st));
    return VGGP_OK;
}

extern "C" int vggp_posterior_cov(vggp_ctx* c, const double* xs1, const double* xs2, int64_t ns, double* cov, void* stream) {
    VG_NOT_PAIRED(c, "vggp_posterior_cov");
    if (!c || !c->have_step) { vg_set_error("vggp_posterior_cov: no finished ELBO step"); return VGGP_ESTATE; }
    VG_REQUIRE(xs1 && xs2 && cov && ns >= 1, "vggp_posterior_cov: bad argument");
    const long m1 = c->desc.m1, m2 = c->desc.m2, M = m1 * m2;
    VG_REQUIRE(ns <= 8192 && M * ns <= (1L << 27), "vggp_posterior_cov: ns=%ld points x M=%ld is too large for a dense covariance "
               "(use vggp_posterior for mean / variance)", (long)ns, M);
    VG_ENTER_DEVICE(c->device);
    hipStream_t st = stream ? (hipStream_t)stream : c->own_stream;
    const size_t need = (size_t)(2 * (m1 + m2) * ns + 2 * M * ns + M) * sizeof(double);
    int rc = vg_accurate_state(c, st);
    if (rc) return rc;
    if ((rc = vg_ensure_misc(c, need))) return rc;
    double* p = (double*)c->misc;
    double* A1 = p; p += m1 * ns;
    double* A2 = p; p += m2 * ns;
    double* U1 = p; p += m1 * ns;
    double* U2 = p; p += m2 * ns;
    double* T = p; p += M * ns;
    double* Tw = p; p += M * ns;
    if ((rc = posterior_factors(c, xs1, xs2, (int)ns, A1, A2, U1, U2, st, true))) return rc;
    VG_HIP(vg_qv_weights_launch(c->theta, c->beta, c->invD, c->wq, M, st));
    hipLaunchKernelGGL(vg_khatri_rao_kernel, dim3((unsigned)((M * ns + 255) / 256)), dim3(256), 0, st, U1, U2, c->wq + M, (int)m1,
                       (int)m2, (long)ns, T, Tw);
    VG_HIP(hipGetLastError());
    VgGemmBatch g;
    vg_gemm_init(&g);
    vg_gemm_add(&g, Tw, 1, ns, T, ns, 1, cov, (int)ns, (int)ns, (int)ns, (int)M, 1, 0, 1, 0, c->h_theta[2] * c->h_theta[3], 0);
    VG_HIP(vg_gemm_launch(&g, st));
    VG_HIP(vg_prior_cov_launch(xs1, xs2, ns, c->d[0].kind, c->d[1].kind, c->theta, cov, st));
    return VGGP_OK;
// ... 477 lines not shown
```

### variational_gridded_gaussian_processes_amd/csrc/chol.hip

```cpp
#include "gemm_body.h"

#include <cstdlib>

static const int VG_CHOL_FAST_MAX_M = 128;
__constant__ double VG_JITTERS[4] = {0.0, 1e-8, 1e-7, 1e-6};

#define VG_CHOL_MAXJOBS 8
struct VgCholArgs {
    VgCholJob job[VG_CHOL_MAXJOBS];
    int njobs;
    int fast[VG_CHOL_MAXJOBS];
};

__device__ __forceinline__ int vg_ctri(int i) { return (i * (i + 1)) >> 1; }

template <int MT>
__device__ void vg_chol_fast(const VgCholJob& J, int lvl, double* W, double* rsd, double* rowbuf, int* s_i) {
    const int m = J.m;
    const int tid = threadIdx.x, tx = tid & 31, ty = tid >> 5;
    const double jit = VG_JITTERS[lvl];
    const int ldk = J.ldk ? J.ldk : m, ldl = J.ldl ? J.ldl : m;
    int* flags = reinterpret_cast<int*>(J.scratch);

    double a[MT][MT];
    int trow[MT], tcol[MT];
#pragma unroll
    for (int ia = 0; ia < MT; ++ia) {
        trow[ia] = vg_ctri(ty + 32 * ia);
        tcol[ia] = vg_ctri(tx + 32 * ia);
#pragma unroll
        for (int ib = 0; ib < MT; ++ib) {
            const int i = ty + 32 * ia, j = tx + 32 * ib;
            a[ia][ib] = (i < m && j <= i) ? J.K[(long)i * ldk + j] + (i == j ? jit : 0.0) : 0.0;
        }
    }

#ifdef VG_CHOL_STAMP
    unsigned long long tA = 0, tB = 0, tC = 0, s0, s1, tstart, tend;
#define CS(var) do { __builtin_amdgcn_sched_barrier(0); asm volatile("s_memtime %0\n\ts_waitcnt lgkmcnt(0)" : "=s"(var) :: "memory"); __builtin_amdgcn_sched_barrier(0); } while (0)
    CS(tstart);
#else
#define CS(var)
#endif
    bool ok = true;
    int pivoff = 0;
    for (int k = 0; k < m; ++k) {
#ifdef VG_CHOL_STAMP
        CS(s0);
#endif
        const int kb = k >> 5, kx = k & 31;
        if (tx == kx) {
#define VG_PUB(KB)                                                                  \
    if (KB < MT && kb == KB) {                                                      \
        _Pragma("unroll") for (int ia = 0; ia < MT; ++ia)                           \
            if (ty + 32 * ia >= k) W[trow[ia] + k] = a[ia][KB < MT ? KB : 0];       \
    }
            VG_PUB(0) else VG_PUB(1) else VG_PUB(2) else VG_PUB(3)
#undef VG_PUB
        }
#ifdef VG_CHOL_STAMP
        CS(s1); tA += s1 - s0;
#endif
        __syncthreads();
#ifdef VG_CHOL_STAMP
        CS(s0); tB += s0 - s1;
#endif
        const double piv = W[pivoff];
        pivoff += k + 2;
        double li[MT], lj[MT];
#pragma unroll
        for (int ia = 0; ia < MT; ++ia) {
            li[ia] = W[trow[ia] + k];
            lj[ia] = W[tcol[ia] + k];
        }
        if (!(piv > 0.0) || !(piv < 1.0e300)) { ok = false; break; }
        double rp = __builtin_amdgcn_rcp(piv);
        rp = fma(rp, fma(-piv, rp, 1.0), rp);
        rp = fma(rp, fma(-piv, rp, 1.0), rp);
#pragma unroll
        for (int ia = 0; ia < MT; ++ia) {
            const double lr = li[ia] * rp;
#pragma unroll
            for (int ib = 0; ib < MT; ++ib) a[ia][ib] -= lr * lj[ib];
        }
#ifdef VG_CHOL_STAMP
        CS(s1); tC += s1 - s0;
#endif
    }
#ifdef VG_CHOL_STAMP
    CS(tend);
    if ((tid & 63) == 0 && lvl == 0) {
        unsigned long long* dbg = reinterpret_cast<unsigned long long*>(J.scratch) + 16 + (tid >> 6) * 4;
        dbg[0] = tA; dbg[1] = tB; dbg[2] = tC; dbg[3] = tend - tstart;
    }
#endif

    __syncthreads();
    if (J.only_level0) {
        if (tid == 0) { s_i[0] = ok ? 1 : 0; s_i[1] = ok ? 0 : 1; }
    } else if (tid == 0) {
        __hip_atomic_store(&flags[lvl], ok ? 1 : 2, __ATOMIC_RELAXED, __HIP_MEMORY_SCOPE_AGENT);
        int win = ok ? 1 : 0, spins = 0;
        bool all_failed = !ok;
        for (int l = 0; l < lvl; ++l) {
            int f;
            while ((f = __hip_atomic_load(&flags[l], __ATOMIC_RELAXED, __HIP_MEMORY_SCOPE_AGENT)) == 0) {
                if (++spins > (1 << 22)) { f = 2; break; }
                __builtin_amdgcn_s_sleep(4);
            }
            if (f == 1) { win = 0; all_failed = false; }
        }
        s_i[0] = win;
        s_i[1] = (lvl == 3 && all_failed) ? 1 : 0;
    }
    __syncthreads();
    const bool winner = s_i[0] != 0, report_fail = s_i[1] != 0;
    if (report_fail) {
        if (tid == 0) { *J.status = VGGP_ENOTPD; if (J.jitter_out) *J.jitter_out = -1.0; }
        const double qnan = __longlong_as_double(0x7ff8000000000000LL);
        for (int idx = tid; idx < m * m; idx += blockDim.x) { J.L[(long)(idx / m) * ldl + idx % m] = qnan; J.Linv[idx] = qnan; }
    }
    if (!winner) return;
    if (tid == 0 && J.jitter_out) *J.jitter_out = jit;

    for (int k = tid; k < m; k += blockDim.x) rsd[k] = 1.0 / sqrt(W[vg_ctri(k) + k]);
    __syncthreads();
    for (int i = ty; i < m; i += 32)
        for (int k = tx; k <= i; k += 32) {
            const double v = W[vg_ctri(i) + k] * rsd[k];
            W[vg_ctri(i) + k] = v;
            J.L[(long)i * ldl + k] = v;
        }
    for (int i = ty; i < m; i += 32)
        for (int k = tx; k < m; k += 32)
            if (k > i) J.L[(long)i * ldl + k] = 0.0;
    __syncthreads();

#pragma unroll
    for (int ia = 0; ia < MT; ++ia)
#pragma unroll
        for (int ib = 0; ib < MT; ++ib) a[ia][ib] = (ty + 32 * ia == tx + 32 * ib) ? 1.0 : 0.0;
    for (int k = 0; k < m; ++k) {
        const int ka = k >> 5, ky = k & 31;
        double* rb = rowbuf + (k & 1) * 192;
        if (ty == ky) {
            const double rk = rsd[k];
#define VG_PUBR(KA)                                                                 \
    if (KA < MT && ka == KA) {                                                      \
        _Pragma("unroll") for (int ib = 0; ib < MT; ++ib) {                         \
            a[KA < MT ? KA : 0][ib] *= rk;                                          \
            rb[tx + 32 * ib] = a[KA < MT ? KA : 0][ib];                             \
        }                                                                           \
    }
            VG_PUBR(0) else VG_PUBR(1) else VG_PUBR(2) else VG_PUBR(3)
#undef VG_PUBR
        }
        __syncthreads();
        double li[MT], xr[MT];
#pragma unroll
        for (int ia = 0; ia < MT; ++ia) {
            const int i = ty + 32 * ia;
            li[ia] = (i > k) ? W[trow[ia] + k] : 0.0;
            xr[ia] = rb[tx + 32 * ia];
        }
#pragma unroll
        for (int ia = 0; ia < MT; ++ia)
#pragma unroll
            for (int ib = 0; ib < MT; ++ib) a[ia][ib] -= li[ia] * xr[ib];
    }
#pragma unroll
    for (int ia = 0; ia < MT; ++ia)
#pragma unroll
        for (int ib = 0; ib < MT; ++ib) {
            const int i = ty + 32 * ia, j = tx + 32 * ib;
            if (i < m && j < m) J.Linv[(long)i * m + j] = (j <= i) ? a[ia][ib] : 0.0;
        }
}

__device__ void vg_chol_generic(const VgCholJob& J, double* sd) {
    const int m = J.m, ld = m + 1;
    double* W = J.scratch;
    const int tid = threadIdx.x, nthr = blockDim.x;
    const int tx = tid & 31, ty = tid >> 5, nty = nthr >> 5;
    int used = -1;
    for (int attempt = 0; attempt < 4; ++attempt) {
        const double jit = VG_JITTERS[attempt];
        for (int idx = tid; idx < m * m; idx += nthr) {
            const int i = idx / m, j = idx - i * m;
            W[i * ld + j] = J.K[idx] + (i == j ? jit : 0.0);
        }
        __threadfence_block();
        __syncthreads();
        bool ok = true;
        for (int k = 0; k < m; ++k) {
            const double piv = W[k * ld + k];
            if (!(piv > 0.0) || !(piv < 1.0e300)) { ok = false; break; }
            const double rp = 1.0 / piv;
            for (int i = k + 1 + ty; i < m; i += nty) {
                const double lik = W[i * ld + k] * rp;
                for (int j = k + 1 + tx; j <= i; j += 32) W[i * ld + j] -= lik * W[j * ld + k];
            }
            __threadfence_block();
            __syncthreads();
        }
        if (ok) { used = attempt; break; }
        __syncthreads();
    }
    if (used < 0) {
        if (tid == 0) { *J.status = VGGP_ENOTPD; if (J.jitter_out) *J.jitter_out = -1.0; }
        const double qnan = __longlong_as_double(0x7ff8000000000000LL);
        for (int idx = tid; idx < m * m; idx += nthr) { J.L[idx] = qnan; J.Linv[idx] = qnan; }
        return;
    }
    if (tid == 0 && J.jitter_out) *J.jitter_out = VG_JITTERS[used];
    for (int k = tid; k < m; k += nthr) sd[k] = sqrt(W[k * ld + k]);
    __syncthreads();
    for (int idx = tid; idx < m * m; idx += nthr) {
        const int i = idx / m, k = idx - i * m;
        if (i > k) W[i * ld + k] /= sd[k];
        else if (i == k) W[i * ld + k] = sd[k];
    }
    __threadfence_block();
    __syncthreads();
    for (int idx = tid; idx < m * m; idx += nthr) {
        const int i = idx / m, j = idx - i * m;
        J.L[idx] = (j <= i) ? W[i * ld + j] : 0.0;
    }
    const int sub = tid & 7, grp = tid >> 3, ngrp = nthr >> 3;
    for (int jb = 0; jb < m; jb += ngrp) {
        const int j = jb + grp;
        if (j < m) {
            const double xj = 1.0 / W[j * ld + j];
            for (int i = j + 1; i < m; ++i) {
                double part = 0.0;
                for (int k = j + sub; k < i; k += 8) {
                    const double xk = (k == j) ? xj : W[j * ld + k];
                    part += W[i * ld + k] * xk;
                }
                part += __shfl_xor(part, 1);
                part += __shfl_xor(part, 2);
                part += __shfl_xor(part, 4);
                const double xi = -part / W[i * ld + i];
                if (sub == 0) W[j * ld + i] = xi;
                __threadfence_block();
            }
        }
    }
    __threadfence_block();
    __syncthreads();
    for (int idx = tid; idx < m * m; idx += nthr) {
        const int i = idx / m, j = idx - i * m;
        double v = 0.0;
        if (i == j) v = 1.0 / W[i * ld + i];
        else if (i > j) v = W[j * ld + i];
        J.Linv[idx] = v;
    }
}


#define VG_CB 16
#define VG_CLD 132
typedef double vg_cd4 __attribute__((ext_vector_type(4)));

__device__ __forceinline__ double vg_crcp(double x) {
    double r = __builtin_amdgcn_rcp(x);
    r = fma(r, fma(-x, r, 1.0), r);
    r = fma(r, fma(-x, r, 1.0), r);
    return r;
}
__device__ __forceinline__ double vg_crsq(double x) {
    double y = __builtin_amdgcn_rsq(x);
    y = fma(y * 0.5, fma(-x * y, y, 1.0), y);
    y = fma(y * 0.5, fma(-x * y, y, 1.0), y);
    return y;
}
#define VG_WAVE_SYNC() do { __builtin_amdgcn_fence(__ATOMIC_RELEASE, "wavefront"); __builtin_amdgcn_wave_barrier(); __builtin_amdgcn_fence(__ATOMIC_ACQUIRE, "wavefront"); } while (0)

__device__ void vg_chol_mfma(const VgCholJob& J, int lvl, double* Lm, double* Dinv, double* Db, double* colbuf, double* xrow,
                             double* sdv, int* s_i) {
    const int m = J.m, nb = (m + VG_CB - 1) / VG_CB, mp = nb * VG_CB;
    const int tid = threadIdx.x, nthr = blockDim.x, lane = tid & 63, wave = tid >> 6;
    const int fi = lane & 15, fk = lane >> 4;
    const double jit = VG_JITTERS[lvl];
    const int ldk = J.ldk ? J.ldk : m, ldl = J.ldl ? J.ldl : m;
    int* flags = reinterpret_cast<int*>(J.scratch);
#ifdef VG_CHOL_STAMP
    unsigned long long T[8] = {0, 0, 0, 0, 0, 0, 0, 0}, tF = 0, tU = 0, tS = 0, q0, q1;
#define CM(var) do { __builtin_amdgcn_sched_barrier(0); asm volatile("s_memtime %0\n\ts_waitcnt lgkmcnt(0)" : "=s"(var) :: "memory"); __builtin_amdgcn_sched_barrier(0); } while (0)
    CM(T[0]);
#else
#define CM(var)
#endif

    {
        const int nw = nthr >> 6;
        double v[16][2];
#pragma unroll
        for (int u = 0; u < 16; ++u) {
            const int i = wave + u * nw;
#pragma unroll
            for (int h = 0; h < 2; ++h) {
                const int j = lane + 64 * h;
                v[u][h] = (i < m && j <= i) ? J.K[(long)i * ldk + j] : 0.0;
            }
        }
#pragma unroll
        for (int u = 0; u < 16; ++u) {
            const int i = wave + u * nw;
#pragma unroll
            for (int h = 0; h < 2; ++h) {
                const int j = lane + 64 * h;
                if (i < mp && j < mp) Lm[i * VG_CLD + j] = v[u][h] + (i == j ? (i < m ? jit : 1.0) : 0.0);
            }
        }
        for (int i = wave + 16 * nw; i < mp; i += nw)
            for (int h = 0; h < 2; ++h) {
                const int j = lane + 64 * h;
                if (j < mp) Lm[i * VG_CLD + j] = ((i < m && j <= i) ? J.K[(long)i * ldk + j] : 0.0) + (i == j ? (i < m ? jit : 1.0) : 0.0);
            }
    }
    for (int idx = tid; idx < nb * VG_CB * VG_CB; idx += nthr) Dinv[idx] = 0.0;
    if (tid == 0) s_i[2] = 0;
    __syncthreads();
    CM(T[1]);

    bool ok = true;
    for (int p = 0; p < nb; ++p) {
        CM(q0);
        const int bi = p + wave;
        vg_cd4 ut = {0.0, 0.0, 0.0, 0.0};
        const bool mine = bi < nb;
        if (mine) {
            vg_cd4 acc = {0.0, 0.0, 0.0, 0.0};
            const double* ap = Lm + (p * VG_CB + fi) * VG_CLD + fk;
            const double* bp = Lm + (bi * VG_CB + fi) * VG_CLD + fk;
            if (wave > 0)
                for (int k0 = 0; k0 < p * VG_CB; k0 += 4) acc = __builtin_amdgcn_mfma_f64_16x16x4f64(ap[k0], bp[k0], acc, 0, 0, 0);
#pragma unroll
            for (int r = 0; r < 4; ++r) {
                const int c = fk + 4 * r, i = fi;
                int gr = bi * VG_CB + i, gc = p * VG_CB + c;
                if (gc > gr) { const int t = gr; gr = gc; gc = t; }
                ut[r] = Lm[gr * VG_CLD + gc] - acc[r];
            }
            if (wave == 0) {
#pragma unroll
                for (int r = 0; r < 4; ++r) Db[(fk + 4 * r) * 17 + fi] = ut[r];
            }
        }
        CM(q1);
#ifdef VG_CHOL_STAMP
        tU += q1 - q0;
#endif
        if (wave == 0) {
            VG_WAVE_SYNC();
            const int i = fi, q = fk;
            double a[4], x[4];
#pragma unroll
            for (int c = 0; c < 4; ++c) { a[c] = Db[i * 17 + 4 * q + c]; x[c] = (i == 4 * q + c) ? 1.0 : 0.0; }
            bool good = true;
#pragma unroll
            for (int k = 0; k < VG_CB; k += 4) {
                if (q == (k >> 2)) {
#pragma unroll
                    for (int c = 0; c < 4; ++c) colbuf[(k + c) * 16 + i] = a[c];
                }
                if ((i >> 2) == (k >> 2)) {
#pragma unroll
                    for (int c = 0; c < 4; ++c) xrow[(i & 3) * 16 + 4 * q + c] = x[c];
                }
                VG_WAVE_SYNC();
                double Cp[4][4], Ci[4], Cj[4][4], Yr[4][4];
#pragma unroll
                for (int r = 0; r < 4; ++r) {
                    Ci[r] = colbuf[(k + r) * 16 + i];
#pragma unroll
                    for (int c = 0; c < 4; ++c) {
                        Cp[r][c] = colbuf[(k + r) * 16 + k + c];
                        Cj[r][c] = colbuf[(k + r) * 16 + 4 * q + c];
                        Yr[r][c] = xrow[r * 16 + 4 * q + c];
                    }
                }
                double l[4];
#pragma unroll
                for (int r = 0; r < 4; ++r) {
                    const double pr = Cp[r][r];
                    if (!(pr > 0.0) || !(pr < 1.0e300)) { good = false; break; }
                    const double inv = vg_crcp(pr);
                    l[r] = (i > k + r) ? Ci[r] * inv : 0.0;
#pragma unroll
                    for (int t = r + 1; t < 4; ++t) {
                        const double f = Cp[r][t] * inv;
#pragma unroll
                        for (int sidx = t; sidx < 4; ++sidx) Cp[t][sidx] -= Cp[r][sidx] * f;
                        Ci[t] -= Ci[r] * f;
#pragma unroll
                        for (int c = 0; c < 4; ++c) { Cj[t][c] -= Cj[r][c] * f; Yr[t][c] -= Yr[r][c] * f; }
                    }
                }
                if (!good) break;
                VG_WAVE_SYNC();
                if (q == 0 && i > k) {
#pragma unroll
                    for (int t = 1; t < 4; ++t) colbuf[(k + t) * 16 + i] = Ci[t];
                }
#pragma unroll
                for (int c = 0; c < 4; ++c) {
                    a[c] -= l[0] * Cj[0][c] + l[1] * Cj[1][c] + l[2] * Cj[2][c] + l[3] * Cj[3][c];
                    x[c] -= l[0] * Yr[0][c] + l[1] * Yr[1][c] + l[2] * Yr[2][c] + l[3] * Yr[3][c];
                }
            }
            if (good) {
                if (lane < 16) sdv[lane] = vg_crsq(colbuf[lane * 16 + lane]);
                VG_WAVE_SYNC();
                const double si = sdv[i];
#pragma unroll
                for (int c = 0; c < 4; ++c) {
                    const int k = 4 * q + c;
                    Lm[(p * VG_CB + i) * VG_CLD + p * VG_CB + k] = (k <= i) ? colbuf[k * 16 + i] * sdv[k] : 0.0;
                    Dinv[(p * VG_CB + i) * VG_CB + k] = (k <= i) ? x[c] * si : 0.0;
                }
            } else if (lane == 0) {
                s_i[2] = 1;
            }
        }
        CM(q0);
#ifdef VG_CHOL_STAMP
        tF += q0 - q1;
#endif
        __syncthreads();
        if (s_i[2]) { ok = false; break; }
        if (mine && wave > 0) {
            vg_cd4 lt = {0.0, 0.0, 0.0, 0.0};
            const double* xp = Dinv + (p * VG_CB + fi) * VG_CB + fk;
#pragma unroll
            for (int r = 0; r < 4; ++r) lt = __builtin_amdgcn_mfma_f64_16x16x4f64(xp[4 * r], ut[r], lt, 0, 0, 0);
#pragma unroll
            for (int r = 0; r < 4; ++r) Lm[(bi * VG_CB + fi) * VG_CLD + p * VG_CB + fk + 4 * r] = lt[r];
            vg_cd4 dd = {0.0, 0.0, 0.0, 0.0};
#pragma unroll
            for (int r = 0; r < 4; ++r) dd = __builtin_amdgcn_mfma_f64_16x16x4f64(lt[r], lt[r], dd, 0, 0, 0);
#pragma unroll
            for (int r = 0; r < 4; ++r) {
                const int row = fk + 4 * r;
                if (fi <= row) Lm[(bi * VG_CB + row) * VG_CLD + bi * VG_CB + fi] -= dd[r];
            }
        }
        __syncthreads();
        CM(q1);
#ifdef VG_CHOL_STAMP
        tS += q1 - q0;
#endif
    }
    CM(T[2]);

    if (J.only_level0) {
        if (tid == 0) { s_i[0] = ok ? 1 : 0; s_i[1] = ok ? 0 : 1; }
    } else if (tid == 0) {
        __hip_atomic_store(&flags[lvl], ok ? 1 : 2, __ATOMIC_RELAXED, __HIP_MEMORY_SCOPE_AGENT);
        int win = ok ? 1 : 0, spins = 0;
        bool all_failed = !ok;
        for (int l = 0; l < lvl; ++l) {
            int f;
            while ((f = __hip_atomic_load(&flags[l], __ATOMIC_RELAXED, __HIP_MEMORY_SCOPE_AGENT)) == 0) {
                if (++spins > (1 << 22)) { f = 2; break; }
                __builtin_amdgcn_s_sleep(4);
            }
            if (f == 1) { win = 0; all_failed = false; }
        }
        s_i[0] = win;
        s_i[1] = (lvl == 3 && all_failed) ? 1 : 0;
    }
    __syncthreads();
    const bool winner = s_i[0] != 0, report_fail = s_i[1] != 0;
    if (report_fail) {
        if (tid == 0) { *J.status = VGGP_ENOTPD; if (J.jitter_out) *J.jitter_out = -1.0; }
        const double qnan = __longlong_as_double(0x7ff8000000000000LL);
        for (int idx = tid; idx < m * m; idx += nthr) { J.L[(long)(idx / m) * ldl + idx % m] = qnan; if (J.Linv) J.Linv[idx] = qnan; }
        if (J.Dinv_out) for (int idx = tid; idx < nb * VG_CB * VG_CB; idx += nthr) J.Dinv_out[idx] = qnan;
    }
    if (!winner) return;
    if (tid == 0 && J.jitter_out) *J.jitter_out = jit;
    CM(T[3]);
    if (J.Dinv_out) for (int idx = tid; idx < nb * VG_CB * VG_CB; idx += nthr) J.Dinv_out[idx] = Dinv[idx];

    for (int i = wave; i < m; i += (nthr >> 6))
#pragma unroll
        for (int h = 0; h < 2; ++h) {
            const int j = lane + 64 * h;
            if (j < m) J.L[(long)i * ldl + j] = (j <= i) ? Lm[i * VG_CLD + j] : 0.0;
        }
    CM(T[4]);
    if (!J.Linv) return;
    for (int bj = wave; bj < nb; bj += (nthr >> 6)) {
        for (int bi = bj + 1; bi < nb; ++bi) {
            vg_cd4 t = {0.0, 0.0, 0.0, 0.0};
            const double* ap = Lm + (bi * VG_CB + fi) * VG_CLD + fk;
            {
                const double* bp = Dinv + (bj * VG_CB + fk) * VG_CB + fi;
#pragma unroll
                for (int k0 = 0; k0 < VG_CB; k0 += 4)
                    t = __builtin_amdgcn_mfma_f64_16x16x4f64(ap[bj * VG_CB + k0], bp[k0 * VG_CB], t, 0, 0, 0);
            }
            for (int bk = bj + 1; bk < bi; ++bk) {
                const double* bp = Lm + (bj * VG_CB + fk) * VG_CLD + bk * VG_CB + fi;
#pragma unroll
                for (int k0 = 0; k0 < VG_CB; k0 += 4)
                    t = __builtin_amdgcn_mfma_f64_16x16x4f64(ap[bk * VG_CB + k0], bp[k0 * VG_CLD], t, 0, 0, 0);
            }
            vg_cd4 xb = {0.0, 0.0, 0.0, 0.0};
            const double* xp = Dinv + (bi * VG_CB + fi) * VG_CB + fk;
#pragma unroll
            for (int r = 0; r < 4; ++r) xb = __builtin_amdgcn_mfma_f64_16x16x4f64(xp[4 * r], t[r], xb, 0, 0, 0);
#pragma unroll
            for (int r = 0; r < 4; ++r) Lm[(bj * VG_CB + fk + 4 * r) * VG_CLD + bi * VG_CB + fi] = -xb[r];
            VG_WAVE_SYNC();
        }
    }
    __syncthreads();
    CM(T[5]);
    for (int i = wave; i < m; i += (nthr >> 6))
#pragma unroll
        for (int h = 0; h < 2; ++h) {
            const int j = lane + 64 * h;
            const int bi = i >> 4, bj = j >> 4;
            double v = 0.0;
            if (bi == bj) v = Dinv[i * VG_CB + (j & 15)];
            else if (bi > bj) v = Lm[(bj * VG_CB + (i & 15)) * VG_CLD + bi * VG_CB + (j & 15)];
            if (j < m) J.Linv[(long)i * m + j] = v;
        }
#ifdef VG_CHOL_STAMP
    CM(T[6]);
    if (lane == 0) {
        unsigned long long* dbg = reinterpret_cast<unsigned long long*>(J.scratch) + 16 + wave * 12;
        for (int i = 0; i < 7; ++i) dbg[i] = T[i] - T[0];
        dbg[7] = tU; dbg[8] = tF; dbg[9] = tS;
    }
#endif
}

__global__ __launch_bounds__(512) void vg_chol_mfma_kernel(const VgCholArgs a, const VgGemmBatch rider) {
    extern __shared__ double vg_cm_dyn[];
    if ((int)blockIdx.x >= 4 * a.njobs) {
        vg_gemm_body<64, 16, 512>(rider, vg_cm_dyn, blockIdx.x - 4 * a.njobs);
        return;
    }
    __shared__ double Db[16 * 17];
    __shared__ double colbuf[16 * 16];
    __shared__ double xrow[4 * 16];
    __shared__ double sdv[16];
    __shared__ int s_i[4];
    const VgCholJob& J = a.job[blockIdx.x >> 2];
    const int lvl = blockIdx.x & 3;
    if (J.only_level0 && lvl > 0) return;
    const int nb = (J.m + VG_CB - 1) / VG_CB, mp = nb * VG_CB;
    vg_chol_mfma(J, lvl, vg_cm_dyn, vg_cm_dyn + mp * VG_CLD, Db, colbuf, xrow, sdv, s_i);
}

__global__ __launch_bounds__(1024) void vg_chol_kernel(const VgCholArgs a) {
    extern __shared__ double vg_chol_dyn[];
    __shared__ double sd[1024];
    __shared__ double rowbuf[2 * 192];
    __shared__ int s_i[2];
    const VgCholJob& J = a.job[blockIdx.y];
    const int lvl = blockIdx.x;
    if (J.only_level0 && lvl > 0) return;
    if (a.fast[blockIdx.y]) {
        if (J.m <= 64) vg_chol_fast<2>(J, lvl, vg_chol_dyn, sd, rowbuf, s_i);
        else vg_chol_fast<4>(J, lvl, vg_chol_dyn, sd, rowbuf, s_i);
    } else if (lvl == 0) {
        vg_chol_generic(J, sd);
    }
}


__global__ void vg_jitcopy_kernel(const double* K, int m, double* Kc) {
    const long idx = (long)blockIdx.x * blockDim.x + threadIdx.x, mm = (long)m * m;
    if (idx >= 4 * mm) return;
    const int lvl = (int)(idx / mm);
    const long e = idx - lvl * mm;
    Kc[idx] = K[e] + ((e / m == e % m) ? VG_JITTERS[lvl] : 0.0);
}
hipError_t vg_jitcopy_launch(const double* K, int m, double* Kc, hipStream_t st) {
    hipLaunchKernelGGL(vg_jitcopy_kernel, dim3((unsigned)((4L * m * m + 255) / 256)), dim3(256), 0, st, K, m, Kc);
    return hipGetLastError();
}
__global__ void vg_cholsel_kernel(const double* Lc, const double* Dc, const int* st8, int m, int nb16, double* L0, double* Dinv0,
                                  double* jitter_out, int* status) {
    __shared__ int s_lvl;
    if (threadIdx.x == 0 && blockIdx.x == 0) {}
    if (threadIdx.x == 0) {
        int lvl = -1;
        for (int l = 3; l >= 0; --l) if (st8[2 * l] == 0 && st8[2 * l + 1] == 0) lvl = l;
        s_lvl = lvl;
    }
    __syncthreads();
    const int lvl = s_lvl;
    const long mm = (long)m * m;
    if (blockIdx.x == 0 && threadIdx.x == 0) {
        if (lvl < 0) { *status = VGGP_ENOTPD; *jitter_out = -1.0; }
        else *jitter_out = VG_JITTERS[lvl];
    }
    const double qnan = __longlong_as_double(0x7ff8000000000000LL);
    for (long e = (long)blockIdx.x * blockDim.x + threadIdx.x; e < mm; e += (long)gridDim.x * blockDim.x) {
        const int i = (int)(e / m), j = (int)(e - (long)i * m);
        L0[e] = lvl < 0 ? qnan : (j <= i ? Lc[lvl * mm + e] : 0.0);
    }
    for (long e = (long)blockIdx.x * blockDim.x + threadIdx.x; e < (long)nb16 * 256; e += (long)gridDim.x * blockDim.x)
        Dinv0[e] = lvl < 0 ? qnan : Dc[(long)lvl * nb16 * 256 + e];
}
hipError_t vg_cholsel_launch(const double* Lc, const double* Dc, const int* st8, int m, double* L0, double* Dinv0, double* jitter_out,
                             int* status, hipStream_t st) {
    hipLaunchKernelGGL(vg_cholsel_kernel, dim3(64), dim3(256), 0, st, Lc, Dc, st8, m, (m + 15) / 16, L0, Dinv0, jitter_out, status);
    return hipGetLastError();
}

hipError_t vg_chol_setup() {
    hipError_t e = hipFuncSetAttribute(reinterpret_cast<const void*>(vg_chol_mfma_kernel),
                                       hipFuncAttributeMaxDynamicSharedMemorySize, 152 * 1024);
    if (e != hipSuccess) return e;
    return hipFuncSetAttribute(reinterpret_cast<const void*>(vg_chol_kernel),
                               hipFuncAttributeMaxDynamicSharedMemorySize, 140 * 1024);
}

hipError_t vg_chol_launch(const VgCholJob* jobs, int njobs, hipStream_t st, const VgGemmBatch* rider) {
    if (njobs < 1 || njobs > VG_CHOL_MAXJOBS) return hipErrorInvalidValue;
    VgCholArgs a;
    a.njobs = njobs;
    size_t lds = 0;
    static const bool legacy = getenv("VGGP_CHOL_LEGACY") != nullptr;
    bool all_fast = !legacy;
    for (int j = 0; j < njobs; ++j) all_fast = all_fast && jobs[j].m >= 1 && jobs[j].m <= VG_CHOL_FAST_MAX_M;
    for (int j = 0; j < njobs; ++j)
        if (!jobs[j].Linv && !all_fast) return hipErrorInvalidValue;
    if (all_fast) {
        for (int j = 0; j < njobs; ++j) {
            a.job[j] = jobs[j];
            a.fast[j] = 1;
            const size_t mp = (size_t)((jobs[j].m + VG_CB - 1) / VG_CB) * VG_CB;
            const size_t need = (mp * VG_CLD + mp * VG_CB) * sizeof(double);
            if (need > lds) lds = need;
        }
        VgGemmBatch rb;
        rb.nprob = 0; rb.total_tiles = 0;
        if (rider && rider->nprob > 0 && rider->total_tiles > 0) {
            rb = *rider;
            const size_t rl = 2 * VgTile<64, 16>::TILE * sizeof(double);
            if (rl > lds) lds = rl;
        }
        hipLaunchKernelGGL(vg_chol_mfma_kernel, dim3(4 * njobs + rb.total_tiles), dim3(512), lds, st, a, rb);
        return hipGetLastError();
    }
    if (rider && rider->nprob > 0) return hipErrorInvalidValue;
    for (int j = 0; j < njobs; ++j) {
        a.job[j] = jobs[j];
        if (jobs[j].m > 1024 || jobs[j].m < 1) return hipErrorInvalidValue;
        a.fast[j] = jobs[j].m <= VG_CHOL_FAST_MAX_M;
        if (a.fast[j]) {
            const size_t mp = jobs[j].m <= 64 ? 64 : 128;
            const size_t need = mp * (mp + 1) / 2 * sizeof(double);
            if (need > lds) lds = need;
        }
    }
    hipLaunchKernelGGL(vg_chol_kernel, dim3(4, njobs), dim3(1024), lds, st, a);
    return hipGetLastError();
}
```

### variational_gridded_gaussian_processes_amd/csrc/common.h

```cpp
#pragma once
#if defined(__HIP_DEVICE_COMPILE__) && !defined(__gfx950__)
#error "libvggp_hip is written for gfx950 (MI355X) only: kernels rely on its wave64 barrier semantics, MFMA shapes and LDS size"
#endif
#include <hip/hip_runtime.h>
#include <stdint.h>
#include "../../include/vggp.h"

#define VG_WAVE 64

void vg_set_error(const char* fmt, ...);
#define VG_HIP(call)                                                              \
    do {                                                                          \
        hipError_t _e = (call);                                                   \
        if (_e != hipSuccess) {                                                   \
            vg_set_error("%s:%d: %s -> %s", __FILE__, __LINE__, #call,            \
                         hipGetErrorString(_e));                                  \
            return VGGP_EHIP;                                                     \
        }                                                                         \
    } while (0)
#define VG_REQUIRE(cond, ...)                                                     \
    do {                                                                          \
        if (!(cond)) {                                                            \
            vg_set_error(__VA_ARGS__);                                            \
            return VGGP_EINVAL;                                                   \
        }                                                                         \
    } while (0)

struct VgDeviceGuard {
    int prev = -1;
    bool switched = false;
    hipError_t enter(int dev) {
        hipError_t e = hipGetDevice(&prev);
        if (e != hipSuccess) return e;
        if (prev != dev) { e = hipSetDevice(dev); switched = (e == hipSuccess); }
        return e;
    }
    ~VgDeviceGuard() { if (switched) (void)hipSetDevice(prev); }
};
#define VG_ENTER_DEVICE(dev) VgDeviceGuard vg_dev_guard_; VG_HIP(vg_dev_guard_.enter(dev))

#define VG_GEMM_MAXP 12
#define VG_BM 64
#define VG_BN 64
#define VG_BK 16

struct VgGemmP {
    const double* A;
    const double* B;
    double* C;
    long sa_m, sa_k, sb_k, sb_n;
    long c_slab;
    long b_slab;
    long a_slab;
    int a_nslab;
    int M, N, K;
    int ldc;
    int ksplit;
    int b_nslab;
    int tiles_m, tiles_n;
    int tile_start;
    int kchunk;
    double alpha;
    int accum;
    int xcd_group;
    int tri;
    const double* dotw;
    double* dot_out;
    int dotw_ld;
    int deep;
    int rev;
};
#define VG_TRI_NONE 0
#define VG_TRI_A_LOWER 1
#define VG_TRI_A_UPPER 2
#define VG_TRI_B_UPPER 3
#define VG_TRI_B_LOWER 4
#define VG_TRI_A_UPPER_B_LOWER 5
struct VgGemmBatch {
    int nprob;
    int total_tiles;
    VgGemmP p[VG_GEMM_MAXP];
};

void vg_gemm_init(VgGemmBatch* b);
int vg_gemm_add(VgGemmBatch* b, const double* A, long sa_m, long sa_k, const double* B, long sb_k,
                long sb_n, double* C, int ldc, int M, int N, int K, int ksplit = 1, long c_slab = 0,
                int b_nslab = 1, long b_slab = 0, double alpha = 1.0, int accum = 0);
#define VG_GEMM_TAG_GRAM_PROJECT 1
#define VG_GEMM_TAG_WIDE 2
void vg_gemm_xcd_group(VgGemmBatch* b, int prob);
hipError_t vg_gemm_launch(const VgGemmBatch* b, hipStream_t st, int tag = 0);
const char* vg_last_project_kernel();

#define VG_RED_MAXSEG 8
struct VgRedSeg { const double* in; double* out; long n; long slab; int nslab; int block_start; };
struct VgRedBatch { int nseg; int total_blocks; VgRedSeg s[VG_RED_MAXSEG]; };
void vg_red_init(VgRedBatch* b);
void vg_red_add(VgRedBatch* b, const double* in, double* out, long n, long slab, int nslab);
hipError_t vg_red_launch(const VgRedBatch* b, hipStream_t st);

struct VgFactorJob {
    const double* x;
    const double* grid;
    double* A0;
    double* dA0;
    double* K0;
    double* dK0;
    int n, m, kind, basis;
    int theta_idx;
    double ell_imm;
    int flags;
};
struct VgClearArgs;
hipError_t vg_factor_build_launch(const VgFactorJob* jobs, int njobs, const double* theta_dev, hipStream_t st,
                                  double* theta_copy = nullptr, const VgClearArgs* clr = nullptr);

struct VgCholJob {
    const double* K;
    double* L;
    double* Linv;
    double* scratch;
    double* jitter_out;
    int* status;
    int m;
    int ldk = 0, ldl = 0;
    int only_level0 = 0;
    double* Dinv_out = nullptr;
};
struct VgGemmBatch;
hipError_t vg_chol_launch(const VgCholJob* jobs, int njobs, hipStream_t st, const VgGemmBatch* rider = nullptr);
hipError_t vg_chol_setup();
hipError_t vg_jitcopy_launch(const double* K, int m, double* Kc, hipStream_t st);
hipError_t vg_cholsel_launch(const double* Lc, const double* Dc, const int* st8, int m, double* L0, double* Dinv0, double* jitter_out,
                             int* status, hipStream_t st);

struct VgTrsmJob {
    const double* L;
    const double* Dinv;
    const double* R;
    double* X;
    long ldl, dinv_blk, dinv_ld;
    long r_sk, r_sc, x_sk, x_sc;
    long ncols;
    int m;
    int trans;
    int rhs_ident = 0;
};
hipError_t vg_trsm_launch(const VgTrsmJob* jobs, int njobs, hipStream_t st);
hipError_t vg_trsm_setup();
hipError_t vg_tri_diaginv_launch(const double* L, long ldl, int m, double* out , hipStream_t st,
                                 const double* L2 = nullptr, long ldl2 = 0, int m2 = 0, double* out2 = nullptr);

#define VG_EIG_MAXSWEEP 60
struct VgEigJob {
    const double* G;
    double* lam;
    double* Qt;
    const double* Qt0;
    double* gwork;
    double2* rotlog;
    int* roundlog;
    int* counters;
    int m;
    int max_rounds;
    long log_bytes;
    int block;
    double tol = 0.0;
    double* Qt2 = nullptr;
    const double* cp_src = nullptr;
    double* cp_dst = nullptr;
    int* perm = nullptr;
    int fast_switch = 112;
    int polish = 1;
    int* err = nullptr;
    int polish0 = 0;
    const double* Hl = nullptr;
    const double* Hr = nullptr;
    int hk = 0;
    int null_from = 0;
    int newton = 0;
    int sparse_first = 0;
};
#define VG_EIG_RANK_CUT 1e-14
struct VgRowQrJob { const double* Z; double* V1; int r; int m; const double* cp_src; double* cp_dst; long cp_n; };
struct VgGemmBatch;
hipError_t vg_rowqr_launch(const VgRowQrJob* jobs, int njobs, hipStream_t st, const VgGemmBatch* rider = nullptr);
hipError_t vg_identity_launch(double* A, int m, hipStream_t st);
struct VgRefineJob { const double* Gw; double* E; double* R1; int m; double tol;
                     double emax = 0.0;
                     int* flag = nullptr;
                     double noise = 0.0;
                     const double* lam_prev = nullptr;
                     double null_cut = 0.0;
};
struct VgNewtonCheckJob { const double* Gw; double* lam; int* counters; int* err; const int* flag; int m; int iters; double tol; double noise;
                          double null_cut = 0.0;
};
hipError_t vg_newton_check_launch(const VgNewtonCheckJob* jobs, int njobs, hipStream_t st);
hipError_t vg_copy_if_launch(const int* const* err, const double* const* src_a, double* const* dst_a, const double* const* src_b,
                             double* const* dst_b, const long* n, int njobs, hipStream_t st);
hipError_t vg_refine_launch(const VgRefineJob* jobs, int njobs, hipStream_t st, const VgGemmBatch* rider = nullptr);
size_t vg_eigh_log_bytes(int m);
hipError_t vg_eigh_launch(const VgEigJob* jobs, int njobs, hipStream_t st, const VgGemmBatch* rider = nullptr);
hipError_t vg_eigh_setup();

#define VG_ESUBMISS (-100)
struct VgHostOut {
    double out[8];
    double jitter[2];
    int counters[2][4];
    int status[2];
    double seq;
};
struct VgMspace {
    const double* theta;
    const double* lam1;
    const double* lam2;
    const double* P3;
    const double* E1;
    const double* F1;
    const double* E2;
    const double* F2;
    double* beta;
    double* bl2;
    double* bl1;
    double* invD;
    double* rowpart;
    double* r1;
    double* r1l;
    double* ol;
    const double* dotp;
    double* r2;
    double* r2l;
    double* dotpart;
    double* out;
    int m1, m2;
    double n_total;
    double yy;
    int* ticket = nullptr;
    VgHostOut* hout = nullptr;
    const double* peer_fail = nullptr;
    const double* jit[2] = {nullptr, nullptr};
    const int* status[2] = {nullptr, nullptr};
    const int* counters[2] = {nullptr, nullptr};
};
hipError_t vg_dstage_launch(const VgMspace* ms, hipStream_t st);
#define VG_THIN_MAXR 32
#define VG_THIN_ELBO_TOL 1e-10
#define VG_THIN_MISS 1e-12
struct VgThinTail {
    const double* theta;
    double n_total, yy;
    int r1, r2, m1, m2;
    const double *W1, *W2;
    const double *lam1, *lam2;
    const double *AM1, *AH1, *AM2, *AH2;
    const double* AC;
    int ac_nslab; long ac_slab;
    const double *G1, *H1, *G2, *H2;
    double* out;
    double *beta_out, *invd_out;
    VgHostOut* hout;
    const double* peer_fail;
    const double* jit[2];
    const int* status[2];
    const int* rcounters[2];
    unsigned long long* stamps = nullptr;
};
hipError_t vg_thin_tail_launch(const VgThinTail* tt, hipStream_t st);
struct VgPivCholJob { const double* G; const double* Omega; double* V; int m; int r; };
struct VgPivCholArgs { VgPivCholJob job[2]; };
hipError_t vg_pivchol_launch(const VgPivCholJob* jobs, int njobs, hipStream_t st);
hipError_t vg_thin_tail_setup();
hipError_t vg_final_launch(const VgMspace* ms, hipStream_t st);
hipError_t vg_zw_launch(const double* theta, int self, const double* lam_self, const double* lam_other, int m, int m_other,
                        const double* X, const double* Xl, const double* r, const double* rl, double* WE, double* WFs, hipStream_t st);
hipError_t vg_zdot_launch(const double* theta, int self, const double* z, const double* x, int m, long n, const double* Abar,
                          const double* dA0, const double* Kbar, const double* dK0, double* out, hipStream_t st);

#define VG_CLEAR_MAX 12
struct VgClearArgs { int* ptr[VG_CLEAR_MAX]; int nwords[VG_CLEAR_MAX]; int n; };
hipError_t vg_clear_launch(const VgClearArgs* a, hipStream_t st);

hipError_t vg_readout_weights_launch(const double* theta, const double* beta, const double* invD, double* w, long n, int literal,
                                     hipStream_t st);
hipError_t vg_readout_var_launch(const double* theta, const double* kd1, const double* kd2, long mv1, long mv2, double* var, hipStream_t st);
hipError_t vg_scale_sq_launch(const double* in, double* out_sq, long n, hipStream_t st);
hipError_t vg_qv_weights_launch(const double* theta, const double* beta, const double* invD, double* w_mean,
                                long n, hipStream_t st, int e1 = 1, int e2 = 1);
hipError_t vg_sumsq_launch(const double* y, long n, double* partial, double* out, hipStream_t st);
hipError_t vg_post_combine_launch(const double* theta, const double* T1, const double* T2, const double* beta,
                                  const double* invD, int m1, int m2, long ns, double* mean, double* var,
                                  hipStream_t st);
hipError_t vg_scale_launch(double* x, long n, const double* theta, int mode, hipStream_t st, int e1 = 1, int e2 = 1);
```

### variational_gridded_gaussian_processes_amd/csrc/ctx.h

```cpp
#pragma once
#include "common.h"

#define VG_MAXEV 40
#define VG_NFORK 4

struct VgDim {
    int kind = 0, basis = 0, n = 0, m = 0;
    double *x = nullptr, *grid = nullptr;
    double *K0 = nullptr, *dK0 = nullptr, *AD = nullptr, *L0 = nullptr, *Linv0 = nullptr, *BV = nullptr;
    double *Kc = nullptr, *Lc = nullptr, *Dc = nullptr;
    int* st8 = nullptr;
    double* Dinv0 = nullptr;
    double *X = nullptr, *Mk = nullptr, *GH = nullptr, *GHslab = nullptr, *Gw = nullptr;
    double *lam0 = nullptr, *Qt = nullptr, *QtPrev = nullptr, *QtPrev2 = nullptr, *U = nullptr;
    double *Ep = nullptr, *Fp = nullptr, *Wp = nullptr;
    double *TM = nullptr, *TH = nullptr, *E = nullptr, *F = nullptr, *RQ = nullptr, *RQsq = nullptr;
    double *chol_scratch = nullptr, *gwork = nullptr, *jitter = nullptr;
    double2* rotlog = nullptr;
    int *roundlog = nullptr, *counters = nullptr, *status = nullptr, *perm = nullptr;
    int gh_split = 1, max_rounds = 0;
    double* Id = nullptr;
    double *Zs = nullptr, *V1s = nullptr, *Hs = nullptr, *Ws = nullptr, *lam_s = nullptr, *gwork2 = nullptr;
    double2* rotlog2 = nullptr;
    int *roundlog2 = nullptr, *counters2 = nullptr, *perm2 = nullptr;
    int sub_r = 0;
    double *tMV = nullptr, *tHV = nullptr, *tAM = nullptr, *tAH = nullptr;
    double* Omega = nullptr;
    int thin_rows = 0;
    bool have_prev = false, have_prev2 = false;
};

struct VgGraphKey {
    const void* y = nullptr;
    const void* payload = nullptr;
    double yy = 0.0;
    bool operator==(const VgGraphKey& o) const { return y == o.y && payload == o.payload && yy == o.yy; }
};

typedef VgHostOut HostOut;

struct vggp_ctx {
    int device = 0;
    bool planned = false;
    vggp_desc desc{};
    VgDim d[2];
    void* arena = nullptr;
    size_t arena_bytes = 0, arena_used = 0;
    double* Sp = nullptr;
    double *St = nullptr, *CCslab = nullptr, *payload = nullptr, *GH1 = nullptr;
    double *T3 = nullptr, *P3 = nullptr, *beta = nullptr, *bl2 = nullptr, *bl1 = nullptr, *invD = nullptr;
    double *rowpart = nullptr, *r1 = nullptr, *r1l = nullptr, *r2 = nullptr, *r2l = nullptr, *dotpart = nullptr, *ol = nullptr;
    double *out = nullptr, *theta = nullptr, *wq = nullptr;
    int st_split = 1, cc_split = 1;
    int st_slabs = 1;
    bool dinv_valid = false;
    int ride_stage0 = 0;
    int gh_slabs[2] = {1, 1}, cc_slabs = 1;
    long payload_len = 0;
    bool have_partials = false, have_step = false, have_masked = false;
    void* masked = nullptr;
    void* paired = nullptr;
    bool is_paired = false;
    double* h_theta = nullptr;
    HostOut* h_out = nullptr;
    HostOut* d_hout = nullptr;
    double* d_htheta = nullptr;
    int* ticket = nullptr;
    void* misc = nullptr;
    size_t misc_bytes = 0;
    double* sumsq_partial = nullptr;
    double* sumsq_out = nullptr;
    hipStream_t own_stream = nullptr;
    hipStream_t side_stream = nullptr;
    hipEvent_t ev_fork[VG_NFORK] = {}, ev_join[VG_NFORK] = {};
    bool use_graph = true;
    hipGraphExec_t gexec[20] = {};
    VgGraphKey gkey[20];
    bool last_warm = false, last_slabs = false, acc_valid = false;
    const double* last_payload = nullptr;
    double last_yy = 0.0;
    VgGemmBatch ride_proj, ride_cc;
    bool ride_pending = false;
    double last_ell[2] = {0.0, 0.0};
    bool pred_consumed = false;
    bool refine_next = false;
    bool sub_next = false;
    int sub_r_cap[2] = {0, 0};
    double *tCV = nullptr, *tAC = nullptr;
    bool cur_thin = false;
    int cur_r[2] = {0, 0};
    bool cur_extrap = false;
    int cur_newton = 0;
    bool last_newton = false, newton_next = false;
    int newton_block = 0;
    int newton_iters = 3, newton_cap = 0;
    int newton_ok_run = 0;
    bool last_thin = false;
    int thin_block = 0;
    bool thin_off = false;
    bool sub_mode = false;
    int n_ranks = 1, rank = 0;
    void* comm = nullptr;
    bool comm_dead = false;
    vggp_allreduce_fn cb = nullptr;
    void* cb_user = nullptr;
    double* h_stage = nullptr;
    long h_stage_count = 0;
    hipStream_t poll_stream = nullptr;
    bool poll_stream_valid = false;
    long seq = 0;
    int warm_run = 0;
    bool prof = false;
    hipEvent_t ev[VG_MAXEV] = {};
    int ev_stage[VG_MAXEV] = {};
    int nev = 0;
    double prof_ms[VGGP_NSTAGE] = {};
    int prof_steps = 0;
};


int vg_ensure_misc(vggp_ctx* c, size_t bytes);
int vg_comm_init(vggp_ctx* c, int n_ranks, int rank, const void* unique_id);
void vg_comm_destroy(vggp_ctx* c);
int vg_allreduce(vggp_ctx* c, double* buf, long count, hipStream_t st);
void vg_comm_abort(vggp_ctx* c);
int vg_comm_wait(vggp_ctx* c, hipStream_t st, const volatile double* seq = nullptr, double want = 0.0);
#define VG_DENSE_MB 128
struct VgDenseChol { double *S, *L, *X, *DI, *Tmp, *scratch, *jit; int* status; long M; double* Sinv; };
int vg_blocked_chol_inverse(const VgDenseChol& w, hipStream_t st);
int vg_partials_enqueue(vggp_ctx* c, const double* Y, double* payload, hipStream_t st, bool reduce = true, bool extrap = false, bool fused = false,
                        bool apply_ns = false, int early = 0);
void vg_masked_free(vggp_ctx* c);
int vg_paired_plan(vggp_ctx* c, const vggp_desc* desc);
void vg_paired_free(vggp_ctx* c);
int vg_paired_set_inducing(vggp_ctx* c, int dim, const double* z, int64_t m);
int vg_paired_step(vggp_ctx* c, const double* Y, double yy, const double theta[5], double* elbo_out, double grad_out[5],
                   vggp_info* info, hipStream_t st, bool scattered_entry);
int vg_paired_zgrad(vggp_ctx* c, const double* Y, double* gz1, double* gz2, hipStream_t st, bool scattered_entry);
int vg_paired_qv(vggp_ctx* c, double* mean, double* var, hipStream_t st);
int vg_paired_qv_cov(vggp_ctx* c, double* cov, hipStream_t st);
int vg_paired_readout(vggp_ctx* c, const double* C1, int64_t mv1, const double* C2, int64_t mv2, const double* kd1, const double* kd2,
                      double* mean, double* var, int flags, hipStream_t st);
int vg_paired_posterior(vggp_ctx* c, const double* xs1, const double* xs2, int64_t ns, double* mean, double* var, hipStream_t st);
int vg_paired_posterior_cov(vggp_ctx* c, const double* xs1, const double* xs2, int64_t ns, double* cov, hipStream_t st);
#define VG_NOT_PAIRED(c, fn)                                                                                            \
    do {                                                                                                                \
        if ((c) && (c)->is_paired) {                                                                                    \
            vg_set_error("%s: not available on a context planned with VGGP_FLAG_PAIRED_Z (see vggp.h)", fn);          \
            return VGGP_EINVAL;                                                                                         \
        }                                                                                                               \
    } while (0)
void vg_masked_new_plan(vggp_ctx* c);
#define VG_TRSM_BLK 128
struct VgTrsmSpec {
    const double* L; long ldl;
    const double* Dinv; long dinv_blk, dinv_ld;
    double* X; long sk, sc, ncols;
    long m; int trans;
};
int vg_trsm_batch(const VgTrsmSpec* sp, int n, hipStream_t st);
```

### variational_gridded_gaussian_processes_amd/csrc/factor_build.hip

```cpp
#include "common.h"
#include "factor_elem.h"

#define VG_FB_MAXJOBS 4
struct VgFactorArgs {
    VgFactorJob job[VG_FB_MAXJOBS];
    int block_start[2 * VG_FB_MAXJOBS + 1];
    int njobs;
};

#define VG_FB_TN_WIDE 512
#define VG_FB_TN_TALL 128
#define VG_FB_MAXROWS 64

struct VgFbPart {
    int job, kpart;
    int ncols, tiles_c, tmw, wide, block_start;
};
struct VgFactorArgs2 {
    VgFactorJob job[VG_FB_MAXJOBS];
    VgFbPart part[2 * VG_FB_MAXJOBS];
    int nparts;
};

__global__ __launch_bounds__(256) void vg_factor_kernel(const VgFactorArgs2 args, const double* __restrict__ theta,
                                                       double* theta_copy, const VgClearArgs clr) {
    __shared__ double s_grid[VG_FB_MAXROWS + 2];
    const int bid = blockIdx.x, tid = threadIdx.x;
    if (bid == 0) {
        if (theta_copy && tid < 6) theta_copy[tid] = theta[tid];
        for (int k = 0; k < clr.n; ++k)
            for (int i = tid; i < clr.nwords[k]; i += 256) clr.ptr[k][i] = 0;
    }
    int pi = 0;
    for (int i = 1; i < args.nparts; ++i)
        if (bid >= args.part[i].block_start) pi = i;
    const VgFbPart& P = args.part[pi];
    const VgFactorJob& J = args.job[P.job];
    const bool kpart = P.kpart != 0;
    const double ell = (J.theta_idx >= 0) ? theta[J.theta_idx] : J.ell_imm;
    const int m = J.m, ncols = P.ncols, tmw = P.tmw;
    const int t = bid - P.block_start;
    const int tr = t / P.tiles_c, tc = t - tr * P.tiles_c;
    const int lane = tid & 63, wave = tid >> 6;
    const int rows_tile = P.wide ? tmw : 4 * tmw;
    const int row0 = tr * rows_tile;
    const int c = tc * (P.wide ? VG_FB_TN_WIDE : VG_FB_TN_TALL) + (P.wide ? wave * 128 : 0) + 2 * lane;
    const int rw0 = P.wide ? 0 : wave * tmw;

    const int glen = (J.basis == VGGP_BASIS_B0) ? m + 1 : m;
    const bool rowgrid = J.basis == VGGP_BASIS_B0 || J.basis == VGGP_BASIS_POINTS || J.basis == VGGP_BASIS_B1;
    if (tid <= rows_tile) {
        const int gi = row0 + tid;
        s_grid[tid] = (rowgrid && gi < glen) ? J.grid[gi] : 0.0;
    }
    const double* __restrict__ xsrc = kpart ? J.grid : J.x;
    const bool colcoord = !(kpart && (J.basis == VGGP_BASIS_VFF)) && J.basis != VGGP_BASIS_ONE && xsrc != nullptr;
    double x0 = 0.0, x1 = 0.0;
    if (colcoord) {
        if (c + 1 < ncols && ((reinterpret_cast<uintptr_t>(xsrc + c) & 15) == 0)) {
            const double2 xx = *reinterpret_cast<const double2*>(xsrc + c);
            x0 = xx.x; x1 = xx.y;
        } else {
            if (c < ncols) x0 = xsrc[c];
            if (c + 1 < ncols) x1 = xsrc[c + 1];
        }
    }
    __syncthreads();
    if (c >= ncols) return;
    double* __restrict__ O = kpart ? J.K0 : J.A0;
    double* __restrict__ dO = kpart ? J.dK0 : J.dA0;
    const bool vec = c + 1 < ncols && (ncols & 1) == 0 && ((reinterpret_cast<uintptr_t>(O) | reinterpret_cast<uintptr_t>(dO)) & 15) == 0;
    const bool two = c + 1 < ncols;

    if (J.basis == VGGP_BASIS_B0 && !kpart) {
        auto edge = [&](double g, double x, double& E, double& dE) {
            const double u = fabs(x - g), e = exp(-u / ell);
            E = ell * e;
            dE = e * (1.0 + u / ell);
        };
        double Ea0, dEa0, Ea1, dEa1;
        edge(s_grid[rw0], x0, Ea0, dEa0);
        edge(s_grid[rw0], x1, Ea1, dEa1);
        for (int r = 0; r < tmw; ++r) {
            const int k = row0 + rw0 + r;
            if (k >= m) break;
            const double a = s_grid[rw0 + r], b = s_grid[rw0 + r + 1];
            double Eb0, dEb0, Eb1, dEb1;
            edge(b, x0, Eb0, dEb0);
            edge(b, x1, Eb1, dEb1);
            double v0, d0, v1, d1;
            if (x0 > a && x0 <= b) { v0 = 2.0 * ell - (Ea0 + Eb0); d0 = 2.0 - (dEa0 + dEb0); }
            else { const double sg = (x0 <= a) ? 1.0 : -1.0; v0 = sg * (Ea0 - Eb0); d0 = sg * (dEa0 - dEb0); }
            if (x1 > a && x1 <= b) { v1 = 2.0 * ell - (Ea1 + Eb1); d1 = 2.0 - (dEa1 + dEb1); }
            else { const double sg = (x1 <= a) ? 1.0 : -1.0; v1 = sg * (Ea1 - Eb1); d1 = sg * (dEa1 - dEb1); }
            const long o = (long)k * ncols + c;
            if (vec) {
                if (O) *reinterpret_cast<double2*>(O + o) = make_double2(v0, v1);
                if (dO) *reinterpret_cast<double2*>(dO + o) = make_double2(d0, d1);
            } else {
                if (O) { O[o] = v0; if (two) O[o + 1] = v1; }
                if (dO) { dO[o] = d0; if (two) dO[o + 1] = d1; }
            }
            Ea0 = Eb0; dEa0 = dEb0; Ea1 = Eb1; dEa1 = dEb1;
        }
        return;
    }
    if (J.basis == VGGP_BASIS_B0 && kpart && !(J.flags & VGGP_FLAG_B0_F32_KDELTA)) {
        const double t = (J.grid[1] - J.grid[0]) / ell, sh = sinh(0.5 * t), s4 = 4.0 * sh * sh, sh2 = 2.0 * sinh(t);
        const double em1 = expm1(-t), l2 = ell * ell, toe = t / ell;
        const double v_diag = l2 * 2.0 * (em1 + t), d_diag = 2.0 * ell * 2.0 * (em1 + t) + l2 * (2.0 * toe) * em1;
        auto el = [&](int kd, double& v, double& dv) {
            const double e = exp(-(double)kd * t), r = e * s4, dr = toe * e * ((double)kd * s4 - sh2);
            v = kd ? l2 * r : v_diag;
            dv = kd ? 2.0 * ell * r + l2 * dr : d_diag;
        };
        for (int r = 0; r < tmw; ++r) {
            const int k = row0 + rw0 + r;
            if (k >= m) break;
            double v0, d0, v1, d1;
            el(k > c ? k - c : c - k, v0, d0);
            el(k > c + 1 ? k - c - 1 : c + 1 - k, v1, d1);
            const long o = (long)k * ncols + c;
            if (vec) {
                if (O) *reinterpret_cast<double2*>(O + o) = make_double2(v0, v1);
                if (dO) *reinterpret_cast<double2*>(dO + o) = make_double2(d0, d1);
            } else {
                if (O) { O[o] = v0; if (two) O[o + 1] = v1; }
                if (dO) { dO[o] = d0; if (two) dO[o + 1] = d1; }
            }
        }
        return;
    }
    for (int r = 0; r < tmw; ++r) {
        const int k = row0 + rw0 + r;
        if (k >= m) break;
        const double gk = s_grid[rw0 + r], gk1 = s_grid[rw0 + r + 1];
        double v0, d0, v1 = 0.0, d1 = 0.0;
        vg_factor_elem(J, kpart, k, c, x0, gk, gk1, ell, v0, d0);
        if (two) vg_factor_elem(J, kpart, k, c + 1, x1, gk, gk1, ell, v1, d1);
        const long o = (long)k * ncols + c;
        if (vec) {
            if (O) *reinterpret_cast<double2*>(O + o) = make_double2(v0, v1);
            if (dO) *reinterpret_cast<double2*>(dO + o) = make_double2(d0, d1);
        } else {
            if (O) { O[o] = v0; if (two) O[o + 1] = v1; }
            if (dO) { dO[o] = d0; if (two) dO[o + 1] = d1; }
        }
    }
}

hipError_t vg_factor_build_launch(const VgFactorJob* jobs, int njobs, const double* theta_dev, hipStream_t st,
                                  double* theta_copy, const VgClearArgs* clr) {
    if (njobs < 1 || njobs > VG_FB_MAXJOBS) return hipErrorInvalidValue;
    VgFactorArgs2 a;
    a.nparts = 0;
    int blocks = 0;
    long total = 0;
    for (int j = 0; j < njobs; ++j) {
        total += ((jobs[j].A0 || jobs[j].dA0) ? (long)jobs[j].m * jobs[j].n : 0) + ((jobs[j].K0 || jobs[j].dK0) ? (long)jobs[j].m * jobs[j].m : 0);
    }
    const int tmw = total >= (1L << 24) ? 16 : (total >= (1L << 21) ? 8 : (total >= (1L << 18) ? 4 : 2));
    for (int j = 0; j < njobs; ++j) {
        a.job[j] = jobs[j];
        for (int kp = 0; kp < 2; ++kp) {
            const bool want = kp ? (jobs[j].K0 || jobs[j].dK0) : (jobs[j].A0 || jobs[j].dA0);
            const int ncols = kp ? jobs[j].m : jobs[j].n;
            if (!want || ncols <= 0 || jobs[j].m <= 0) continue;
            VgFbPart& P = a.part[a.nparts++];
            P.job = j; P.kpart = kp; P.ncols = ncols; P.tmw = tmw;
            P.wide = ncols >= VG_FB_TN_WIDE ? 1 : 0;
            const int tn = P.wide ? VG_FB_TN_WIDE : VG_FB_TN_TALL, rows = P.wide ? tmw : 4 * tmw;
            P.tiles_c = (ncols + tn - 1) / tn;
            P.block_start = blocks;
            blocks += P.tiles_c * ((jobs[j].m + rows - 1) / rows);
        }
    }
    if (blocks == 0) return hipSuccess;
    VgClearArgs c0;
    c0.n = 0;
    hipLaunchKernelGGL(vg_factor_kernel, dim3(blocks), dim3(256), 0, st, a, theta_dev, theta_copy, clr ? *clr : c0);
    return hipGetLastError();
}
```

### variational_gridded_gaussian_processes_amd/csrc/gemm_body.h

```cpp
#pragma once
#include "common.h"

typedef double vg_d4 __attribute__((ext_vector_type(4)));

template <int T, int BK>
struct VgTile {
    static constexpr int RPAD = BK == 16 ? 1 : 4;
    static constexpr int RS = BK + RPAD;
    static constexpr int KS = T + 16;
    static constexpr int TILE = (BK * KS > T * RS) ? BK * KS : T * RS;
    static constexpr int MB = T / 32;
};

template <int T, int BK, int NT = 256>
__device__ __forceinline__ void vg_gemm_body(const VgGemmBatch& b, double* lds, const int bid) {
    using C_ = VgTile<T, BK>;
    constexpr int NR = T * BK / NT;
    constexpr int WC = NT / 128;
    constexpr int MB = T / 32;
    constexpr int NB = T / (16 * WC);
    double* As = lds;
    double* Bs = lds + C_::TILE;

    int pi = 0;
    for (int i = 1; i < b.nprob; ++i)
        if (bid >= b.p[i].tile_start) pi = i;
    const VgGemmP& p = b.p[pi];

    int t = bid - p.tile_start;
    const int tiles = p.tiles_m * p.tiles_n;
    int ks, tm, tn;
    if (p.xcd_group) {
        const int nx = 8 / p.ksplit;
        const int xcd = t & 7, j = t >> 3;
        ks = xcd / nx;
        const int gi = j / p.tiles_m;
        tm = j - gi * p.tiles_m;
        tn = gi * nx + (xcd - ks * nx);
    } else {
        ks = t / tiles;
        t -= ks * tiles;
        tm = t / p.tiles_n;
        tn = t - tm * p.tiles_n;
    }
    const int row0 = tm * T, col0 = tn * T;
    int k_begin = ks * p.kchunk;
    int k_end = min(p.K, k_begin + p.kchunk);
    if (p.tri) {
        if (p.tri == VG_TRI_A_LOWER) k_end = min(k_end, ((row0 + T + 127) >> 7) << 7);
        else if (p.tri == VG_TRI_A_UPPER) k_begin = max(k_begin, (row0 >> 7) << 7);
        else if (p.tri == VG_TRI_B_UPPER) k_end = min(k_end, ((col0 + T + 127) >> 7) << 7);
        else if (p.tri == VG_TRI_B_LOWER) k_begin = max(k_begin, (col0 >> 7) << 7);
        else k_begin = max(k_begin, (max(row0, col0) >> 7) << 7);
    }

    const int tid = threadIdx.x;
    const int lane = tid & 63, wave = tid >> 6;
    const int wr = wave / WC, wc = wave % WC;

    const double* __restrict__ A = p.A;
    const double* __restrict__ B = p.B;
    const long sa_m = p.sa_m, sa_k = p.sa_k, sb_k = p.sb_k, sb_n = p.sb_n;
    const bool a_kc = (sa_k == 1);
    const bool b_nc = (sb_n == 1);
    const int M = p.M, N = p.N;
    const int nslab = p.b_nslab, anslab = p.a_nslab;
    const long bslab = p.b_slab, aslab = p.a_slab;

    int a_i[NR], a_k[NR], b_k[NR], b_j[NR];
#pragma unroll
    for (int r = 0; r < NR; ++r) {
        if (a_kc) { a_k[r] = tid % BK; a_i[r] = tid / BK + (NT / BK) * r; }
        else      { a_i[r] = tid % T; a_k[r] = tid / T + (NT / T) * r; }
        if (b_nc) { b_j[r] = tid % T; b_k[r] = tid / T + (NT / T) * r; }
        else      { b_k[r] = tid % BK; b_j[r] = tid / BK + (NT / BK) * r; }
    }
    const int a_si = a_kc ? C_::RS : 1, a_sk = a_kc ? 1 : C_::KS;
    const int b_sj = b_nc ? 1 : C_::RS, b_sk = b_nc ? C_::KS : 1;

    double ra0[NR], rb0[NR], ra1[NR], rb1[NR];
    auto load_tile = [&](int k0, double (&ra)[NR], double (&rb)[NR]) {
        const double* bp[NR];
        const double* ap[NR];
        bool bok[NR], aok[NR];
#pragma unroll
        for (int r = 0; r < NR; ++r) {
            const int gi = row0 + a_i[r], gk = k0 + a_k[r];
            aok[r] = gi < M && gk < k_end;
            ap[r] = A + (aok[r] ? gi * sa_m + gk * sa_k : 0);
            ra[r] = aok[r] ? ap[r][0] : 0.0;
            const int gj = col0 + b_j[r], gkb = k0 + b_k[r];
            bok[r] = gj < N && gkb < k_end;
            bp[r] = B + (bok[r] ? gkb * sb_k + gj * sb_n : 0);
            rb[r] = bok[r] ? bp[r][0] : 0.0;
        }
        for (int s = 1; s < nslab; s += 3) {
            double t[3][NR];
#pragma unroll
            for (int u = 0; u < 3; ++u)
#pragma unroll
                for (int r = 0; r < NR; ++r) t[u][r] = (bok[r] && s + u < nslab) ? bp[r][(long)(s + u) * bslab] : 0.0;
#pragma unroll
            for (int r = 0; r < NR; ++r) rb[r] += (t[0][r] + t[1][r]) + t[2][r];
        }
        for (int s = 1; s < anslab; s += 3) {
            double t[3][NR];
#pragma unroll
            for (int u = 0; u < 3; ++u)
#pragma unroll
                for (int r = 0; r < NR; ++r) t[u][r] = (aok[r] && s + u < anslab) ? ap[r][(long)(s + u) * aslab] : 0.0;
#pragma unroll
            for (int r = 0; r < NR; ++r) ra[r] += (t[0][r] + t[1][r]) + t[2][r];
        }
    };

    vg_d4 acc[MB][NB];
#pragma unroll
    for (int i = 0; i < MB; ++i)
#pragma unroll
        for (int j = 0; j < NB; ++j) acc[i][j] = (vg_d4){0.0, 0.0, 0.0, 0.0};

    const int fi = lane & 15, fk = lane >> 4;
    constexpr int WT = T / 2, WTC = T / WC;
    auto ktile = [&](double (&ra)[NR], double (&rb)[NR], int knext) {
#pragma unroll
        for (int r = 0; r < NR; ++r) {
            As[a_i[r] * a_si + a_k[r] * a_sk] = ra[r];
            Bs[b_k[r] * b_sk + b_j[r] * b_sj] = rb[r];
        }
        __syncthreads();
        if (knext < k_end) load_tile(knext, ra, rb);
#pragma unroll
        for (int kk = 0; kk < BK; kk += 4) {
            double av[MB], bv[NB];
#pragma unroll
            for (int mb = 0; mb < MB; ++mb)
                av[mb] = As[(wr * WT + mb * 16 + fi) * a_si + (kk + fk) * a_sk];
#pragma unroll
            for (int nb = 0; nb < NB; ++nb)
                bv[nb] = Bs[(kk + fk) * b_sk + (wc * WTC + nb * 16 + fi) * b_sj];
#pragma unroll
            for (int mb = 0; mb < MB; ++mb)
#pragma unroll
                for (int nb = 0; nb < NB; ++nb)
                    acc[mb][nb] = __builtin_amdgcn_mfma_f64_16x16x4f64(av[mb], bv[nb], acc[mb][nb], 0, 0, 0);
        }
        __syncthreads();
    };
    const bool fast = row0 + T <= M && col0 + T <= N && k_begin < k_end && ((k_end - k_begin) % BK) == 0 &&
                      ((nslab == 1 && anslab == 1) || p.K <= 512);
    if (fast) {
        const double* pa[NR];
        const double* pb[NR];
        int la[NR], lb[NR];
#pragma unroll
        for (int r = 0; r < NR; ++r) {
            pa[r] = A + (long)(row0 + a_i[r]) * sa_m + (long)(k_begin + a_k[r]) * sa_k;
            pb[r] = B + (long)(k_begin + b_k[r]) * sb_k + (long)(col0 + b_j[r]) * sb_n;
            la[r] = a_i[r] * a_si + a_k[r] * a_sk;
            lb[r] = b_k[r] * b_sk + b_j[r] * b_sj;
        }
        const long da = (long)BK * sa_k, db = (long)BK * sb_k;
        const int nk = (k_end - k_begin) / BK;
        auto ld = [&](double (&ra)[NR], double (&rb)[NR]) {
#pragma unroll
            for (int r = 0; r < NR; ++r) { ra[r] = *pa[r]; rb[r] = *pb[r]; }
            for (int sl = 1; sl < nslab; sl += 3) {
                const long o0 = (long)sl * bslab, o1 = sl + 1 < nslab ? o0 + bslab : o0, o2 = sl + 2 < nslab ? o0 + 2 * bslab : o0;
                const double w1 = sl + 1 < nslab ? 1.0 : 0.0, w2 = sl + 2 < nslab ? 1.0 : 0.0;
#pragma unroll
                for (int r = 0; r < NR; ++r) rb[r] += (pb[r][o0] + w1 * pb[r][o1]) + w2 * pb[r][o2];
            }
            for (int sl = 1; sl < anslab; sl += 3) {
                const long o0 = (long)sl * aslab, o1 = sl + 1 < anslab ? o0 + aslab : o0, o2 = sl + 2 < anslab ? o0 + 2 * aslab : o0;
                const double w1 = sl + 1 < anslab ? 1.0 : 0.0, w2 = sl + 2 < anslab ? 1.0 : 0.0;
#pragma unroll
                for (int r = 0; r < NR; ++r) ra[r] += (pa[r][o0] + w1 * pa[r][o1]) + w2 * pa[r][o2];
            }
#pragma unroll
            for (int r = 0; r < NR; ++r) { pa[r] += da; pb[r] += db; }
        };
        auto kt = [&](double (&ra)[NR], double (&rb)[NR], bool more) {
#pragma unroll
            for (int r = 0; r < NR; ++r) { As[la[r]] = ra[r]; Bs[lb[r]] = rb[r]; }
            __syncthreads();
            if (more) ld(ra, rb);
#pragma unroll
            for (int kk = 0; kk < BK; kk += 4) {
                double av[MB], bv[NB];
#pragma unroll
                for (int mb = 0; mb < MB; ++mb) av[mb] = As[(wr * WT + mb * 16 + fi) * a_si + (kk + fk) * a_sk];
#pragma unroll
                for (int nb = 0; nb < NB; ++nb) bv[nb] = Bs[(kk + fk) * b_sk + (wc * WTC + nb * 16 + fi) * b_sj];
#pragma unroll
                for (int mb = 0; mb < MB; ++mb)
#pragma unroll
                    for (int nb = 0; nb < NB; ++nb)
                        acc[mb][nb] = __builtin_amdgcn_mfma_f64_16x16x4f64(av[mb], bv[nb], acc[mb][nb], 0, 0, 0);
            }
            __syncthreads();
        };
        ld(ra0, rb0);
        if (nk > 1) ld(ra1, rb1);
        for (int it = 0; it < nk; it += 2) {
            kt(ra0, rb0, it + 2 < nk);
            if (it + 1 < nk) kt(ra1, rb1, it + 3 < nk);
        }
    } else {
        if (k_begin < k_end) load_tile(k_begin, ra0, rb0);
        if (k_begin + BK < k_end) load_tile(k_begin + BK, ra1, rb1);
        for (int k0 = k_begin; k0 < k_end; k0 += 2 * BK) {
            ktile(ra0, rb0, k0 + 2 * BK);
            if (k0 + BK < k_end) ktile(ra1, rb1, k0 + 3 * BK);
        }
    }

    double* __restrict__ C = p.C ? p.C + (long)ks * p.c_slab : nullptr;
    const int ldc = p.ldc;
    const double* __restrict__ dotw = p.dotw;
    double dsum = 0.0;
#pragma unroll
    for (int mb = 0; mb < MB; ++mb)
#pragma unroll
        for (int nb = 0; nb < NB; ++nb)
#pragma unroll
            for (int r = 0; r < 4; ++r) {
                const int row = row0 + wr * WT + mb * 16 + fk + 4 * r;
                const int col = col0 + wc * WTC + nb * 16 + fi;
                if (row < M && col < N) {
                    const double v = p.alpha * acc[mb][nb][r];
                    if (dotw) dsum += v * dotw[(long)row * p.dotw_ld + col];
                    if (C) {
                        double* cp = C + (long)row * ldc + col;
                        *cp = p.accum ? *cp + v : v;
                    }
                }
            }
    if (p.dot_out) {
#pragma unroll
        for (int off = 32; off > 0; off >>= 1) dsum += __shfl_xor(dsum, off);
        if (lane == 0) lds[wave] = dsum;
        __syncthreads();
        if (tid == 0) {
            double tot = 0.0;
            for (int w = 0; w < NT / 64; ++w) tot += lds[w];
            p.dot_out[bid - p.tile_start] = tot;
        }
    }
}
```

Measured before the change: 5.428 billion grid-points/s.

## Fuse factor build into Cholesky launch and generate kernel entries on the fly

The separate factor-build kernel launch is removed on the points-basis path. Its tiles now run as extra blocks inside a combined Cholesky kernel. The Cholesky blocks rebuild the Gram matrix directly in LDS from the grid and theta, and the early projection GEMM computes its A operand (kernel values and derivatives) on the fly instead of reading it from memory. Level flags carry a theta-derived tag so that stale flags are not cleared between launches, which removes some clearing work but makes correctness depend on the tag changing each step.

```diff
diff --git a/variational_gridded_gaussian_processes_amd/build.py b/variational_gridded_gaussian_processes_amd/build.py
--- a/variational_gridded_gaussian_processes_amd/build.py
+++ b/variational_gridded_gaussian_processes_amd/build.py
@@ -8,7 +8,7 @@
 HERE = os.path.dirname(os.path.abspath(__file__))
 CSRC = os.path.join(HERE, "csrc")
 SOURCES = ["api.hip", "gemm.hip", "factor_build.hip", "chol.hip", "trsm.hip", "eigh.hip", "mspace.hip", "thin.hip", "masked.hip", "comm.hip", "paired.hip"]
-HEADERS = ["common.h", "ctx.h", "factor_elem.h", "gemm_body.h", os.path.join("..", "..", "include", "vggp.h")]
+HEADERS = ["common.h", "ctx.h", "factor_elem.h", "factor_tile.h", "gemm_body.h", os.path.join("..", "..", "include", "vggp.h")]
 LIB = os.path.join(HERE, "libvggp_hip.so")
 
 
diff --git a/variational_gridded_gaussian_processes_amd/csrc/api.hip b/variational_gridded_gaussian_processes_amd/csrc/api.hip
--- a/variational_gridded_gaussian_processes_amd/csrc/api.hip
+++ b/variational_gridded_gaussian_processes_amd/csrc/api.hip
@@ -493,7 +493,7 @@
 }
 
 int vg_partials_enqueue(vggp_ctx* c, const double* Y, double* payload, hipStream_t st, bool reduce, bool extrap, bool fused, bool apply_ns,
-                        int early) {
+                        int early, bool gen_ok) {
     const long n1 = c->desc.n1, n2 = c->desc.n2, m1 = c->desc.m1, m2 = c->desc.m2;
     VgDim &d1 = c->d[0], &d2 = c->d[1];
     hipStream_t sx = vg_side(c, st);
@@ -504,20 +504,23 @@
     VgCholJob cj[2];
     static const bool chol_legacy = getenv("VGGP_CHOL_LEGACY") != nullptr;
     const bool dinv_path = d1.m <= VG_TRSM_BLK && d2.m <= VG_TRSM_BLK && !chol_legacy;
+    static const bool chol_big_off = getenv("VGGP_NO_CHOL_BIG") != nullptr;
+    const bool any_big = (d1.m > VG_TRSM_BLK || d2.m > VG_TRSM_BLK) && !chol_legacy && !chol_big_off;
+    const bool gen = gen_ok && Y && dinv_path && !any_big && !c->prof && d1.basis == VGGP_BASIS_POINTS && d2.basis == VGGP_BASIS_POINTS;
     VgClearArgs clr;
     clr.n = 0;
     for (int k = 0; k < 2; ++k) {
         VgDim& d = c->d[k];
         fj[k] = VgFactorJob{d.x, d.grid, d.AD, d.AD + (long)d.m * d.n, d.K0, d.dK0, d.n, d.m, d.kind, d.basis, k, 0.0, c->desc.flags};
-        clr.ptr[clr.n] = d.status; clr.nwords[clr.n++] = 2;
-        clr.ptr[clr.n] = reinterpret_cast<int*>(d.chol_scratch); clr.nwords[clr.n++] = 16;
+        clr.ptr[clr.n] = d.status + (gen ? 1 : 0); clr.nwords[clr.n++] = gen ? 1 : 2;
+        if (!gen) { clr.ptr[clr.n] = reinterpret_cast<int*>(d.chol_scratch); clr.nwords[clr.n++] = 16; }
         clr.ptr[clr.n] = d.counters; clr.nwords[clr.n++] = 8;
         if (k == 0) { clr.ptr[clr.n] = reinterpret_cast<int*>(c->payload + c->payload_len); clr.nwords[clr.n++] = 2; }
         if (d.st8) { clr.ptr[clr.n] = d.st8; clr.nwords[clr.n++] = 8; }
         cj[k] = VgCholJob{d.K0, d.L0, dinv_path ? nullptr : d.Linv0, d.chol_scratch, d.jitter, d.status, d.m};
         cj[k].Dinv_out = d.Dinv0;
     }
-    VG_HIP(vg_factor_build_launch(fj, 2, c->d_htheta, st, c->theta, &clr));
+    if (!gen) VG_HIP(vg_factor_build_launch(fj, 2, c->d_htheta, st, c->theta, &clr));
     VG_MARK(0);
 
     const bool ns_on_chol = extrap && apply_ns && dinv_path;
@@ -528,8 +531,6 @@
             VgDim& d = c->d[k];
             vg_gemm_add(&gns, d.Wp, d.m, 1, d.Ep, d.m, 1, d.Fp, d.m, d.m, d.m, d.m, 1, 0, 1, 0, -0.5, 1);
         }
-    static const bool chol_big_off = getenv("VGGP_NO_CHOL_BIG") != nullptr;
-    const bool any_big = (d1.m > VG_TRSM_BLK || d2.m > VG_TRSM_BLK) && !chol_legacy && !chol_big_off;
     VgGemmBatch gsp;
     vg_gemm_init(&gsp);
     int sp_slabs = 1;
@@ -558,7 +559,20 @@
                     vg_gemm_add(&gr2, d.Wp, d.m, 1, d.Ep, d.m, 1, d.Fp, d.m, d.m, d.m, d.m, 1, 0, 1, 0, -0.5, 1);
                 }
         }
-        VG_HIP(vg_chol_launch(cj, 2, st, ((early && !c->prof) || ns_on_chol) ? &gr2 : nullptr));
+        const VgGemmBatch* rider = ((early && !c->prof) || ns_on_chol) ? &gr2 : nullptr;
+        if (gen) {
+            VgCholGen g;
+            g.theta = c->d_htheta;
+            g.theta_copy = c->theta;
+            g.job[0] = fj[0]; g.job[1] = fj[1];
+            g.spA.job = fj[1];
+            g.spA.theta = c->d_htheta;
+            g.spA.prob = early ? 0 : -1;
+            g.clr = clr;
+            VG_HIP(vg_chol_gen_launch(cj, 2, st, rider, g));
+        } else {
+            VG_HIP(vg_chol_launch(cj, 2, st, rider));
+        }
     } else {
         int big[2], nbig = 0;
         for (int k = 0; k < 2; ++k) {
@@ -1447,7 +1461,7 @@
     const bool extrap = sp.extrap;
     const bool apply_ns = extrap && !c->pred_consumed;
     rc = run_graph(c, extrap ? VG_G_PARTIALS_X : VG_G_PARTIALS, key, st,
-                   [&] { return vg_partials_enqueue(c, Y, payload, st, true, extrap, false, apply_ns); }, extrap && !apply_ns);
+                   [&] { return vg_partials_enqueue(c, Y, payload, st, true, extrap, false, apply_ns, 0, true); }, extrap && !apply_ns);
     if (rc) return rc;
     if (extrap) c->pred_consumed = true;
     c->have_partials = true;
@@ -1555,7 +1569,7 @@
         static const bool no_early_reg_mr = getenv("VGGP_NO_EARLY_REG") != nullptr;
         const bool early_mr = thin_early || (warm && !thin && !subspace && early_ok && !no_early_reg_mr);
         rc = run_graph(c, early_mr ? (extrap ? VG_G_PARTIALS_XE : VG_G_PARTIALS_E) : extrap ? VG_G_PARTIALS_X : VG_G_PARTIALS, kp, st,
-                       [&] { return vg_partials_enqueue(c, Y, c->payload, st, true, extrap, false, apply_ns, early_mr ? 1 : 0); }, extrap && !apply_ns);
+                       [&] { return vg_partials_enqueue(c, Y, c->payload, st, true, extrap, false, apply_ns, early_mr ? 1 : 0, true); }, extrap && !apply_ns);
         {
             static const long fault_at = [] { const char* e = getenv("VGGP_FAULT_PARTIALS_AT"); return e ? atol(e) : -1L; }();
             if (!rc && fault_at >= 0 && c->seq == fault_at) { vg_set_error("injected fault in the partials of step %ld", c->seq); rc = VGGP_EHIP; }
@@ -1594,7 +1608,7 @@
         const int keep[2] = {c->d[0].sub_r, c->d[1].sub_r};
         c->d[0].sub_r = c->d[1].sub_r = VG_COLD_THIN_R;
         rc = run_graph(c, VG_G_STEP_COLD_T, key, st, [&] {
-            int r1 = vg_partials_enqueue(c, Y, c->payload, st, true, false, true, false, early);
+            int r1 = vg_partials_enqueue(c, Y, c->payload, st, true, false, true, false, early, true);
             if (!r1) r1 = vg_cold_thin_prepass(c, c->payload, st);
             return r1 ? r1 : finish_enqueue(c, c->payload, yy_total, true, st, false, false, false, false, true,
                                             true, 0, early);
@@ -1616,7 +1630,7 @@
     const int early_mode = thin_early ? 1 : (early_reg ? 2 : 0);
     rc = run_graph(c, warm ? (thin ? VG_G_STEP_WARM_T : newton ? VG_G_STEP_WARM_N : subspace ? VG_G_STEP_WARM_S : extrap ? (refine ? VG_G_STEP_WARM_XR : VG_G_STEP_WARM_X) : VG_G_STEP_WARM)
                             : VG_G_STEP_COLD, key, st, [&] {
-        const int r1 = vg_partials_enqueue(c, Y, c->payload, st, !warm, extrap, true, apply_ns, early_mode);
+        const int r1 = vg_partials_enqueue(c, Y, c->payload, st, !warm, extrap, true, apply_ns, early_mode, true);
         return r1 ? r1 : finish_enqueue(c, c->payload, yy_total, warm, st, false, warm, extrap, refine, subspace, thin, newton,
                                         thin_early);
     }, extrap && !apply_ns);
diff --git a/variational_gridded_gaussian_processes_amd/csrc/chol.hip b/variational_gridded_gaussian_processes_amd/csrc/chol.hip
--- a/variational_gridded_gaussian_processes_amd/csrc/chol.hip
+++ b/variational_gridded_gaussian_processes_amd/csrc/chol.hip
@@ -1,4 +1,5 @@
 #include "gemm_body.h"
+#include "factor_tile.h"
 
 #include <cstdlib>
 
@@ -276,8 +277,37 @@
 }
 #define VG_WAVE_SYNC() do { __builtin_amdgcn_fence(__ATOMIC_RELEASE, "wavefront"); __builtin_amdgcn_wave_barrier(); __builtin_amdgcn_fence(__ATOMIC_ACQUIRE, "wavefront"); } while (0)
 
-__device__ void vg_chol_mfma(const VgCholJob& J, int lvl, double* Lm, double* Dinv, double* Db, double* colbuf, double* xrow,
-                             double* sdv, int* s_i) {
+template <int KIND>
+__device__ __forceinline__ void vg_chol_gen_rows(double* Lm, int m, int mp, int wave, int nw, int lane, double zc0, double zc1,
+                                                 double inv_ell, double jit) {
+    for (int i0 = wave; i0 < mp; i0 += 4 * nw) {
+        double e[4][2];
+#pragma unroll
+        for (int s = 0; s < 4; ++s) {
+            const int i = i0 + s * nw;
+            const double zi = __shfl(i < 64 ? zc0 : zc1, i & 63);
+#pragma unroll
+            for (int h = 0; h < 2; ++h) {
+                const int j = lane + 64 * h;
+                double de;
+                e[s][h] = 0.0;
+                if (i < m && j <= i) vg_kappa(KIND, fabs(zi - (h ? zc1 : zc0)), inv_ell, e[s][h], de);
+            }
+        }
+#pragma unroll
+        for (int s = 0; s < 4; ++s) {
+            const int i = i0 + s * nw;
+#pragma unroll
+            for (int h = 0; h < 2; ++h) {
+                const int j = lane + 64 * h;
+                if (i < mp && j < mp) Lm[i * VG_CLD + j] = e[s][h] + (i == j ? (i < m ? jit : 1.0) : 0.0);
+            }
+        }
+    }
+}
+
+__device__ __forceinline__ void vg_chol_mfma(const VgCholJob& J, int lvl, double* Lm, double* Dinv, double* Db, double* colbuf, double* xrow,
+                             double* sdv, int* s_i, const VgFactorJob* G = nullptr, const double* theta = nullptr) {
     const int m = J.m, nb = (m + VG_CB - 1) / VG_CB, mp = nb * VG_CB;
     const int tid = threadIdx.x, nthr = blockDim.x, lane = tid & 63, wave = tid >> 6;
     const int fi = lane & 15, fk = lane >> 4;
@@ -292,8 +322,20 @@
 #define CM(var)
 #endif
 
-    {
-        const int nw = nthr >> 6;
+    int tag = 0;
+    const int nw = nthr >> 6;
+    if (G) {
+        const double ell = theta[G->theta_idx], sq = theta[5];
+        const double zc0 = lane < m ? G->grid[lane] : 0.0, zc1 = lane + 64 < m ? G->grid[lane + 64] : 0.0;
+        const double inv_ell = 1.0 / ell;
+        tag = (int)sq & 0x1fffffff;
+        switch (G->kind) {
+            case VGGP_KIND_MATERN12: vg_chol_gen_rows<VGGP_KIND_MATERN12>(Lm, m, mp, wave, nw, lane, zc0, zc1, inv_ell, jit); break;
+            case VGGP_KIND_MATERN32: vg_chol_gen_rows<VGGP_KIND_MATERN32>(Lm, m, mp, wave, nw, lane, zc0, zc1, inv_ell, jit); break;
+            case VGGP_KIND_MATERN52: vg_chol_gen_rows<VGGP_KIND_MATERN52>(Lm, m, mp, wave, nw, lane, zc0, zc1, inv_ell, jit); break;
+            default: vg_chol_gen_rows<VGGP_KIND_RBF>(Lm, m, mp, wave, nw, lane, zc0, zc1, inv_ell, jit); break;
+        }
+    } else {
         double v[16][2];
 #pragma unroll
         for (int u = 0; u < 16; ++u) {
@@ -457,16 +499,16 @@
     if (J.only_level0) {
         if (tid == 0) { s_i[0] = ok ? 1 : 0; s_i[1] = ok ? 0 : 1; }
     } else if (tid == 0) {
-        __hip_atomic_store(&flags[lvl], ok ? 1 : 2, __ATOMIC_RELAXED, __HIP_MEMORY_SCOPE_AGENT);
+        __hip_atomic_store(&flags[lvl], (tag << 2) | (ok ? 1 : 2), __ATOMIC_RELAXED, __HIP_MEMORY_SCOPE_AGENT);
         int win = ok ? 1 : 0, spins = 0;
         bool all_failed = !ok;
         for (int l = 0; l < lvl; ++l) {
             int f;
-            while ((f = __hip_atomic_load(&flags[l], __ATOMIC_RELAXED, __HIP_MEMORY_SCOPE_AGENT)) == 0) {
+            while (((f = __hip_atomic_load(&flags[l], __ATOMIC_RELAXED, __HIP_MEMORY_SCOPE_AGENT)) & 3) == 0 || (f >> 2) != tag) {
                 if (++spins > (1 << 22)) { f = 2; break; }
                 __builtin_amdgcn_s_sleep(4);
             }
-            if (f == 1) { win = 0; all_failed = false; }
+            if ((f & 3) == 1) { win = 0; all_failed = false; }
         }
         s_i[0] = win;
         s_i[1] = (lvl == 3 && all_failed) ? 1 : 0;
@@ -481,6 +523,7 @@
     }
     if (!winner) return;
     if (tid == 0 && J.jitter_out) *J.jitter_out = jit;
+    if (tid == 0 && G) *J.status = VGGP_OK;
     CM(T[3]);
     if (J.Dinv_out) for (int idx = tid; idx < nb * VG_CB * VG_CB; idx += nthr) J.Dinv_out[idx] = Dinv[idx];
 
@@ -555,6 +598,44 @@
     if (J.only_level0 && lvl > 0) return;
     const int nb = (J.m + VG_CB - 1) / VG_CB, mp = nb * VG_CB;
     vg_chol_mfma(J, lvl, vg_cm_dyn, vg_cm_dyn + mp * VG_CLD, Db, colbuf, xrow, sdv, s_i);
+}
+
+__global__ __launch_bounds__(512) void vg_chol_gen_kernel(const VgCholArgs a, const VgGemmBatch rider, const VgCholGen g) {
+    extern __shared__ double vg_cm_dyn[];
+    const int bid = blockIdx.x, nch = 4 * a.njobs, tid = threadIdx.x, nwr = (g.ntiles + 1) / 2;
+    if (bid >= nch && bid < nch + nwr) {
+        const int w = bid - nch;
+        if (w == 0) {
+            if (g.theta_copy && tid < 6) g.theta_copy[tid] = g.theta[tid];
+            for (int k = 0; k < g.clr.n; ++k)
+                for (int i = tid; i < g.clr.nwords[k]; i += 512) g.clr.ptr[k][i] = 0;
+        }
+        const int t = 2 * w + (tid >> 8);
+        double* s_grid = vg_cm_dyn + (tid >> 8) * (VG_FB_MAXROWS + 2);
+        if (t < g.ntiles) {
+            int pi = 0;
+            for (int i = 1; i < g.nparts; ++i)
+                if (t >= g.part[i].block_start) pi = i;
+            const VgFbPart& P = g.part[pi];
+            vg_factor_tile(g.job[P.job], P, t - P.block_start, tid & 255, s_grid, g.theta);
+        } else {
+            __syncthreads();
+        }
+        return;
+    }
+    if (bid >= nch) {
+        vg_gemm_body<64, 16, 512, true>(rider, vg_cm_dyn, bid - nch - nwr, &g.spA);
+        return;
+    }
+    __shared__ double Db[16 * 17];
+    __shared__ double colbuf[16 * 16];
+    __shared__ double xrow[4 * 16];
+    __shared__ double sdv[16];
+    __shared__ int s_i[4];
+    const VgCholJob& J = a.job[bid >> 2];
+    const int lvl = bid & 3;
+    const int nb = (J.m + VG_CB - 1) / VG_CB, mp = nb * VG_CB;
+    vg_chol_mfma(J, lvl, vg_cm_dyn, vg_cm_dyn + mp * VG_CLD, Db, colbuf, xrow, sdv, s_i, &g.job[bid >> 2], g.theta);
 }
 
 __global__ __launch_bounds__(1024) void vg_chol_kernel(const VgCholArgs a) {
@@ -618,6 +699,8 @@
 hipError_t vg_chol_setup() {
     hipError_t e = hipFuncSetAttribute(reinterpret_cast<const void*>(vg_chol_mfma_kernel),
                                        hipFuncAttributeMaxDynamicSharedMemorySize, 152 * 1024);
+    if (e != hipSuccess) return e;
+    e = hipFuncSetAttribute(reinterpret_cast<const void*>(vg_chol_gen_kernel), hipFuncAttributeMaxDynamicSharedMemorySize, 152 * 1024);
     if (e != hipSuccess) return e;
     return hipFuncSetAttribute(reinterpret_cast<const void*>(vg_chol_kernel),
                                hipFuncAttributeMaxDynamicSharedMemorySize, 140 * 1024);
@@ -665,3 +748,34 @@
     hipLaunchKernelGGL(vg_chol_kernel, dim3(4, njobs), dim3(1024), lds, st, a);
     return hipGetLastError();
 }
+
+#define VG_GEN_TMW 8
+hipError_t vg_chol_gen_launch(const VgCholJob* jobs, int njobs, hipStream_t st, const VgGemmBatch* rider, const VgCholGen& g0) {
+    if (njobs < 1 || njobs > 2) return hipErrorInvalidValue;
+    VgCholArgs a;
+    a.njobs = njobs;
+    size_t lds = 0;
+    for (int j = 0; j < njobs; ++j) {
+        if (jobs[j].m < 1 || jobs[j].m > VG_CHOL_FAST_MAX_M || jobs[j].only_level0 || g0.job[j].m != jobs[j].m ||
+            g0.job[j].basis != VGGP_BASIS_POINTS || g0.job[j].theta_idx < 0)
+            return hipErrorInvalidValue;
+        a.job[j] = jobs[j];
+        a.fast[j] = 1;
+        const size_t mp = (size_t)((jobs[j].m + VG_CB - 1) / VG_CB) * VG_CB;
+        const size_t need = (mp * VG_CLD + mp * VG_CB) * sizeof(double);
+        if (need > lds) lds = need;
+    }
+    VgCholGen g = g0;
+    g.ntiles = vg_factor_plan(g.job, njobs, VG_GEN_TMW, g.part, &g.nparts);
+    VgGemmBatch rb;
+    rb.nprob = 0; rb.total_tiles = 0;
+    if (rider && rider->nprob > 0 && rider->total_tiles > 0) rb = *rider;
+    if (g.spA.prob >= rb.nprob || (g.spA.prob >= 0 && g.spA.job.basis != VGGP_BASIS_POINTS)) return hipErrorInvalidValue;
+    size_t rl = rb.nprob ? 2 * VgTile<64, 16>::TILE * sizeof(double) : 0;
+    if (g.spA.prob >= 0) rl += (size_t)rb.p[g.spA.prob].kchunk * sizeof(double);
+    if (rl > lds) lds = rl;
+    if (2 * (VG_FB_MAXROWS + 2) * sizeof(double) > lds) lds = 2 * (VG_FB_MAXROWS + 2) * sizeof(double);
+    if (lds > 152 * 1024) return hipErrorInvalidValue;
+    hipLaunchKernelGGL(vg_chol_gen_kernel, dim3(4 * njobs + rb.total_tiles + (g.ntiles + 1) / 2), dim3(512), lds, st, a, rb, g);
+    return hipGetLastError();
+}
diff --git a/variational_gridded_gaussian_processes_amd/csrc/common.h b/variational_gridded_gaussian_processes_amd/csrc/common.h
--- a/variational_gridded_gaussian_processes_amd/csrc/common.h
+++ b/variational_gridded_gaussian_processes_amd/csrc/common.h
@@ -111,7 +111,8 @@
     double ell_imm;
     int flags;
 };
-struct VgClearArgs;
+#define VG_CLEAR_MAX 12
+struct VgClearArgs { int* ptr[VG_CLEAR_MAX]; int nwords[VG_CLEAR_MAX]; int n; };
 hipError_t vg_factor_build_launch(const VgFactorJob* jobs, int njobs, const double* theta_dev, hipStream_t st,
                                   double* theta_copy = nullptr, const VgClearArgs* clr = nullptr);
 
@@ -130,6 +131,26 @@
 struct VgGemmBatch;
 hipError_t vg_chol_launch(const VgCholJob* jobs, int njobs, hipStream_t st, const VgGemmBatch* rider = nullptr);
 hipError_t vg_chol_setup();
+struct VgFbPart {
+    int job, kpart;
+    int ncols, tiles_c, tmw, wide, block_start;
+};
+int vg_factor_plan(const VgFactorJob* jobs, int njobs, int tmw, VgFbPart* part, int* nparts);
+struct VgGemmGenA {
+    VgFactorJob job;
+    const double* theta;
+    int prob;
+};
+struct VgCholGen {
+    const double* theta;
+    double* theta_copy;
+    VgFactorJob job[2];
+    VgFbPart part[4];
+    int nparts, ntiles;
+    VgGemmGenA spA;
+    VgClearArgs clr;
+};
+hipError_t vg_chol_gen_launch(const VgCholJob* jobs, int njobs, hipStream_t st, const VgGemmBatch* rider, const VgCholGen& g);
 hipError_t vg_jitcopy_launch(const double* K, int m, double* Kc, hipStream_t st);
 hipError_t vg_cholsel_launch(const double* Lc, const double* Dc, const int* st8, int m, double* L0, double* Dinv0, double* jitter_out,
                              int* status, hipStream_t st);
@@ -278,8 +299,6 @@
 hipError_t vg_zdot_launch(const double* theta, int self, const double* z, const double* x, int m, long n, const double* Abar,
                           const double* dA0, const double* Kbar, const double* dK0, double* out, hipStream_t st);
 
-#define VG_CLEAR_MAX 12
-struct VgClearArgs { int* ptr[VG_CLEAR_MAX]; int nwords[VG_CLEAR_MAX]; int n; };
 hipError_t vg_clear_launch(const VgClearArgs* a, hipStream_t st);
 
 hipError_t vg_readout_weights_launch(const double* theta, const double* beta, const double* invD, double* w, long n, int literal,
diff --git a/variational_gridded_gaussian_processes_amd/csrc/ctx.h b/variational_gridded_gaussian_processes_amd/csrc/ctx.h
--- a/variational_gridded_gaussian_processes_amd/csrc/ctx.h
+++ b/variational_gridded_gaussian_processes_amd/csrc/ctx.h
@@ -129,7 +129,8 @@
 struct VgDenseChol { double *S, *L, *X, *DI, *Tmp, *scratch, *jit; int* status; long M; double* Sinv; };
 int vg_blocked_chol_inverse(const VgDenseChol& w, hipStream_t st);
 int vg_partials_enqueue(vggp_ctx* c, const double* Y, double* payload, hipStream_t st, bool reduce = true, bool extrap = false, bool fused = false,
-                        bool apply_ns = false, int early = 0);
+                        bool apply_ns = false, int early = 0,
+                        bool gen_ok = false);
 void vg_masked_free(vggp_ctx* c);
 int vg_paired_plan(vggp_ctx* c, const vggp_desc* desc);
 void vg_paired_free(vggp_ctx* c);
diff --git a/variational_gridded_gaussian_processes_amd/csrc/factor_build.hip b/variational_gridded_gaussian_processes_amd/csrc/factor_build.hip
--- a/variational_gridded_gaussian_processes_amd/csrc/factor_build.hip
+++ b/variational_gridded_gaussian_processes_amd/csrc/factor_build.hip
@@ -1,21 +1,7 @@
 #include "common.h"
-#include "factor_elem.h"
+#include "factor_tile.h"
 
 #define VG_FB_MAXJOBS 4
-struct VgFactorArgs {
-    VgFactorJob job[VG_FB_MAXJOBS];
-    int block_start[2 * VG_FB_MAXJOBS + 1];
-    int njobs;
-};
-
-#define VG_FB_TN_WIDE 512
-#define VG_FB_TN_TALL 128
-#define VG_FB_MAXROWS 64
-
-struct VgFbPart {
-    int job, kpart;
-    int ncols, tiles_c, tmw, wide, block_start;
-};
 struct VgFactorArgs2 {
     VgFactorJob job[VG_FB_MAXJOBS];
     VgFbPart part[2 * VG_FB_MAXJOBS];
@@ -35,138 +21,18 @@
     for (int i = 1; i < args.nparts; ++i)
         if (bid >= args.part[i].block_start) pi = i;
     const VgFbPart& P = args.part[pi];
-    const VgFactorJob& J = args.job[P.job];
-    const bool kpart = P.kpart != 0;
-    const double ell = (J.theta_idx >= 0) ? theta[J.theta_idx] : J.ell_imm;
-    const int m = J.m, ncols = P.ncols, tmw = P.tmw;
-    const int t = bid - P.block_start;
-    const int tr = t / P.tiles_c, tc = t - tr * P.tiles_c;
-    const int lane = tid & 63, wave = tid >> 6;
-    const int rows_tile = P.wide ? tmw : 4 * tmw;
-    const int row0 = tr * rows_tile;
-    const int c = tc * (P.wide ? VG_FB_TN_WIDE : VG_FB_TN_TALL) + (P.wide ? wave * 128 : 0) + 2 * lane;
-    const int rw0 = P.wide ? 0 : wave * tmw;
-
-    const int glen = (J.basis == VGGP_BASIS_B0) ? m + 1 : m;
-    const bool rowgrid = J.basis == VGGP_BASIS_B0 || J.basis == VGGP_BASIS_POINTS || J.basis == VGGP_BASIS_B1;
-    if (tid <= rows_tile) {
-        const int gi = row0 + tid;
-        s_grid[tid] = (rowgrid && gi < glen) ? J.grid[gi] : 0.0;
-    }
-    const double* __restrict__ xsrc = kpart ? J.grid : J.x;
-    const bool colcoord = !(kpart && (J.basis == VGGP_BASIS_VFF)) && J.basis != VGGP_BASIS_ONE && xsrc != nullptr;
-    double x0 = 0.0, x1 = 0.0;
-    if (colcoord) {
-        if (c + 1 < ncols && ((reinterpret_cast<uintptr_t>(xsrc + c) & 15) == 0)) {
-            const double2 xx = *reinterpret_cast<const double2*>(xsrc + c);
-            x0 = xx.x; x1 = xx.y;
-        } else {
-            if (c < ncols) x0 = xsrc[c];
-            if (c + 1 < ncols) x1 = xsrc[c + 1];
-        }
-    }
-    __syncthreads();
-    if (c >= ncols) return;
-    double* __restrict__ O = kpart ? J.K0 : J.A0;
-    double* __restrict__ dO = kpart ? J.dK0 : J.dA0;
-    const bool vec = c + 1 < ncols && (ncols & 1) == 0 && ((reinterpret_cast<uintptr_t>(O) | reinterpret_cast<uintptr_t>(dO)) & 15) == 0;
-    const bool two = c + 1 < ncols;
-
-    if (J.basis == VGGP_BASIS_B0 && !kpart) {
-        auto edge = [&](double g, double x, double& E, double& dE) {
-            const double u = fabs(x - g), e = exp(-u / ell);
-            E = ell * e;
-            dE = e * (1.0 + u / ell);
-        };
-        double Ea0, dEa0, Ea1, dEa1;
-        edge(s_grid[rw0], x0, Ea0, dEa0);
-        edge(s_grid[rw0], x1, Ea1, dEa1);
-        for (int r = 0; r < tmw; ++r) {
-            const int k = row0 + rw0 + r;
-            if (k >= m) break;
-            const double a = s_grid[rw0 + r], b = s_grid[rw0 + r + 1];
-            double Eb0, dEb0, Eb1, dEb1;
-            edge(b, x0, Eb0, dEb0);
-            edge(b, x1, Eb1, dEb1);
-            double v0, d0, v1, d1;
-            if (x0 > a && x0 <= b) { v0 = 2.0 * ell - (Ea0 + Eb0); d0 = 2.0 - (dEa0 + dEb0); }
-            else { const double sg = (x0 <= a) ? 1.0 : -1.0; v0 = sg * (Ea0 - Eb0); d0 = sg * (dEa0 - dEb0); }
-            if (x1 > a && x1 <= b) { v1 = 2.0 * ell - (Ea1 + Eb1); d1 = 2.0 - (dEa1 + dEb1); }
-            else { const double sg = (x1 <= a) ? 1.0 : -1.0; v1 = sg * (Ea1 - Eb1); d1 = sg * (dEa1 - dEb1); }
-            const long o = (long)k * ncols + c;
-            if (vec) {
-                if (O) *reinterpret_cast<double2*>(O + o) = make_double2(v0, v1);
-                if (dO) *reinterpret_cast<double2*>(dO + o) = make_double2(d0, d1);
-            } else {
-                if (O) { O[o] = v0; if (two) O[o + 1] = v1; }
-                if (dO) { dO[o] = d0; if (two) dO[o + 1] = d1; }
-            }
-            Ea0 = Eb0; dEa0 = dEb0; Ea1 = Eb1; dEa1 = dEb1;
-        }
-        return;
-    }
-    if (J.basis == VGGP_BASIS_B0 && kpart && !(J.flags & VGGP_FLAG_B0_F32_KDELTA)) {
-        const double t = (J.grid[1] - J.grid[0]) / ell, sh = sinh(0.5 * t), s4 = 4.0 * sh * sh, sh2 = 2.0 * sinh(t);
-        const double em1 = expm1(-t), l2 = ell * ell, toe = t / ell;
-        const double v_diag = l2 * 2.0 * (em1 + t), d_diag = 2.0 * ell * 2.0 * (em1 + t) + l2 * (2.0 * toe) * em1;
-        auto el = [&](int kd, double& v, double& dv) {
-            const double e = exp(-(double)kd * t), r = e * s4, dr = toe * e * ((double)kd * s4 - sh2);
-            v = kd ? l2 * r : v_diag;
-            dv = kd ? 2.0 * ell * r + l2 * dr : d_diag;
-        };
-        for (int r = 0; r < tmw; ++r) {
-            const int k = row0 + rw0 + r;
-            if (k >= m) break;
-            double v0, d0, v1, d1;
-            el(k > c ? k - c : c - k, v0, d0);
-            el(k > c + 1 ? k - c - 1 : c + 1 - k, v1, d1);
-            const long o = (long)k * ncols + c;
-            if (vec) {
-                if (O) *reinterpret_cast<double2*>(O + o) = make_double2(v0, v1);
-                if (dO) *reinterpret_cast<double2*>(dO + o) = make_double2(d0, d1);
-            } else {
-                if (O) { O[o] = v0; if (two) O[o + 1] = v1; }
-                if (dO) { dO[o] = d0; if (two) dO[o + 1] = d1; }
-            }
-        }
-        return;
-    }
-    for (int r = 0; r < tmw; ++r) {
-        const int k = row0 + rw0 + r;
-        if (k >= m) break;
-        const double gk = s_grid[rw0 + r], gk1 = s_grid[rw0 + r + 1];
-        double v0, d0, v1 = 0.0, d1 = 0.0;
-        vg_factor_elem(J, kpart, k, c, x0, gk, gk1, ell, v0, d0);
-        if (two) vg_factor_elem(J, kpart, k, c + 1, x1, gk, gk1, ell, v1, d1);
-        const long o = (long)k * ncols + c;
-        if (vec) {
-            if (O) *reinterpret_cast<double2*>(O + o) = make_double2(v0, v1);
-            if (dO) *reinterpret_cast<double2*>(dO + o) = make_double2(d0, d1);
-        } else {
-            if (O) { O[o] = v0; if (two) O[o + 1] = v1; }
-            if (dO) { dO[o] = d0; if (two) dO[o + 1] = d1; }
-        }
-    }
+    vg_factor_tile(args.job[P.job], P, bid - P.block_start, tid, s_grid, theta);
 }
 
-hipError_t vg_factor_build_launch(const VgFactorJob* jobs, int njobs, const double* theta_dev, hipStream_t st,
-                                  double* theta_copy, const VgClearArgs* clr) {
-    if (njobs < 1 || njobs > VG_FB_MAXJOBS) return hipErrorInvalidValue;
-    VgFactorArgs2 a;
-    a.nparts = 0;
+int vg_factor_plan(const VgFactorJob* jobs, int njobs, int tmw, VgFbPart* part, int* nparts) {
     int blocks = 0;
-    long total = 0;
+    *nparts = 0;
     for (int j = 0; j < njobs; ++j) {
-        total += ((jobs[j].A0 || jobs[j].dA0) ? (long)jobs[j].m * jobs[j].n : 0) + ((jobs[j].K0 || jobs[j].dK0) ? (long)jobs[j].m * jobs[j].m : 0);
-    }
-    const int tmw = total >= (1L << 24) ? 16 : (total >= (1L << 21) ? 8 : (total >= (1L << 18) ? 4 : 2));
-    for (int j = 0; j < njobs; ++j) {
-        a.job[j] = jobs[j];
         for (int kp = 0; kp < 2; ++kp) {
             const bool want = kp ? (jobs[j].K0 || jobs[j].dK0) : (jobs[j].A0 || jobs[j].dA0);
             const int ncols = kp ? jobs[j].m : jobs[j].n;
             if (!want || ncols <= 0 || jobs[j].m <= 0) continue;
-            VgFbPart& P = a.part[a.nparts++];
+            VgFbPart& P = part[(*nparts)++];
             P.job = j; P.kpart = kp; P.ncols = ncols; P.tmw = tmw;
             P.wide = ncols >= VG_FB_TN_WIDE ? 1 : 0;
             const int tn = P.wide ? VG_FB_TN_WIDE : VG_FB_TN_TALL, rows = P.wide ? tmw : 4 * tmw;
@@ -175,6 +41,21 @@
             blocks += P.tiles_c * ((jobs[j].m + rows - 1) / rows);
         }
     }
+    return blocks;
+}
+
+hipError_t vg_factor_build_launch(const VgFactorJob* jobs, int njobs, const double* theta_dev, hipStream_t st,
+                                  double* theta_copy, const VgClearArgs* clr) {
+    if (njobs < 1 || njobs > VG_FB_MAXJOBS) return hipErrorInvalidValue;
+    VgFactorArgs2 a;
+    int blocks = 0;
+    long total = 0;
+    for (int j = 0; j < njobs; ++j) {
+        total += ((jobs[j].A0 || jobs[j].dA0) ? (long)jobs[j].m * jobs[j].n : 0) + ((jobs[j].K0 || jobs[j].dK0) ? (long)jobs[j].m * jobs[j].m : 0);
+    }
+    const int tmw = total >= (1L << 24) ? 16 : (total >= (1L << 21) ? 8 : (total >= (1L << 18) ? 4 : 2));
+    for (int j = 0; j < njobs; ++j) a.job[j] = jobs[j];
+    blocks = vg_factor_plan(jobs, njobs, tmw, a.part, &a.nparts);
     if (blocks == 0) return hipSuccess;
     VgClearArgs c0;
     c0.n = 0;
diff --git a/variational_gridded_gaussian_processes_amd/csrc/factor_tile.h b/variational_gridded_gaussian_processes_amd/csrc/factor_tile.h
--- /dev/null
+++ b/variational_gridded_gaussian_processes_amd/csrc/factor_tile.h
@@ -0,0 +1,120 @@
+#pragma once
+#include "factor_elem.h"
+
+#define VG_FB_TN_WIDE 512
+#define VG_FB_TN_TALL 128
+#define VG_FB_MAXROWS 64
+
+__device__ __forceinline__ void vg_factor_tile(const VgFactorJob& J, const VgFbPart& P, const int t, const int tid, double* s_grid,
+                                               const double* __restrict__ theta) {
+    const bool kpart = P.kpart != 0;
+    const double ell = (J.theta_idx >= 0) ? theta[J.theta_idx] : J.ell_imm;
+    const int m = J.m, ncols = P.ncols, tmw = P.tmw;
+    const int tr = t / P.tiles_c, tc = t - tr * P.tiles_c;
+    const int lane = tid & 63, wave = tid >> 6;
+    const int rows_tile = P.wide ? tmw : 4 * tmw;
+    const int row0 = tr * rows_tile;
+    const int c = tc * (P.wide ? VG_FB_TN_WIDE : VG_FB_TN_TALL) + (P.wide ? wave * 128 : 0) + 2 * lane;
+    const int rw0 = P.wide ? 0 : wave * tmw;
+
+    const int glen = (J.basis == VGGP_BASIS_B0) ? m + 1 : m;
+    const bool rowgrid = J.basis == VGGP_BASIS_B0 || J.basis == VGGP_BASIS_POINTS || J.basis == VGGP_BASIS_B1;
+    if (tid <= rows_tile) {
+        const int gi = row0 + tid;
+        s_grid[tid] = (rowgrid && gi < glen) ? J.grid[gi] : 0.0;
+    }
+    const double* __restrict__ xsrc = kpart ? J.grid : J.x;
+    const bool colcoord = !(kpart && (J.basis == VGGP_BASIS_VFF)) && J.basis != VGGP_BASIS_ONE && xsrc != nullptr;
+    double x0 = 0.0, x1 = 0.0;
+    if (colcoord) {
+        if (c + 1 < ncols && ((reinterpret_cast<uintptr_t>(xsrc + c) & 15) == 0)) {
+            const double2 xx = *reinterpret_cast<const double2*>(xsrc + c);
+            x0 = xx.x; x1 = xx.y;
+        } else {
+            if (c < ncols) x0 = xsrc[c];
+            if (c + 1 < ncols) x1 = xsrc[c + 1];
+        }
+    }
+    __syncthreads();
+    if (c >= ncols) return;
+    double* __restrict__ O = kpart ? J.K0 : J.A0;
+    double* __restrict__ dO = kpart ? J.dK0 : J.dA0;
+    const bool vec = c + 1 < ncols && (ncols & 1) == 0 && ((reinterpret_cast<uintptr_t>(O) | reinterpret_cast<uintptr_t>(dO)) & 15) == 0;
+    const bool two = c + 1 < ncols;
+
+    if (J.basis == VGGP_BASIS_B0 && !kpart) {
+        auto edge = [&](double g, double x, double& E, double& dE) {
+            const double u = fabs(x - g), e = exp(-u / ell);
+            E = ell * e;
+            dE = e * (1.0 + u / ell);
+        };
+        double Ea0, dEa0, Ea1, dEa1;
+        edge(s_grid[rw0], x0, Ea0, dEa0);
+        edge(s_grid[rw0], x1, Ea1, dEa1);
+        for (int r = 0; r < tmw; ++r) {
+            const int k = row0 + rw0 + r;
+            if (k >= m) break;
+            const double a = s_grid[rw0 + r], b = s_grid[rw0 + r + 1];
+            double Eb0, dEb0, Eb1, dEb1;
+            edge(b, x0, Eb0, dEb0);
+            edge(b, x1, Eb1, dEb1);
+            double v0, d0, v1, d1;
+            if (x0 > a && x0 <= b) { v0 = 2.0 * ell - (Ea0 + Eb0); d0 = 2.0 - (dEa0 + dEb0); }
+            else { const double sg = (x0 <= a) ? 1.0 : -1.0; v0 = sg * (Ea0 - Eb0); d0 = sg * (dEa0 - dEb0); }
+            if (x1 > a && x1 <= b) { v1 = 2.0 * ell - (Ea1 + Eb1); d1 = 2.0 - (dEa1 + dEb1); }
+            else { const double sg = (x1 <= a) ? 1.0 : -1.0; v1 = sg * (Ea1 - Eb1); d1 = sg * (dEa1 - dEb1); }
+            const long o = (long)k * ncols + c;
+            if (vec) {
+                if (O) *reinterpret_cast<double2*>(O + o) = make_double2(v0, v1);
+                if (dO) *reinterpret_cast<double2*>(dO + o) = make_double2(d0, d1);
+            } else {
+                if (O) { O[o] = v0; if (two) O[o + 1] = v1; }
+                if (dO) { dO[o] = d0; if (two) dO[o + 1] = d1; }
+            }
+            Ea0 = Eb0; dEa0 = dEb0; Ea1 = Eb1; dEa1 = dEb1;
+        }
+        return;
+    }
+    if (J.basis == VGGP_BASIS_B0 && kpart && !(J.flags & VGGP_FLAG_B0_F32_KDELTA)) {
+        const double t = (J.grid[1] - J.grid[0]) / ell, sh = sinh(0.5 * t), s4 = 4.0 * sh * sh, sh2 = 2.0 * sinh(t);
+        const double em1 = expm1(-t), l2 = ell * ell, toe = t / ell;
+        const double v_diag = l2 * 2.0 * (em1 + t), d_diag = 2.0 * ell * 2.0 * (em1 + t) + l2 * (2.0 * toe) * em1;
+        auto el = [&](int kd, double& v, double& dv) {
+            const double e = exp(-(double)kd * t), r = e * s4, dr = toe * e * ((double)kd * s4 - sh2);
+            v = kd ? l2 * r : v_diag;
+            dv = kd ? 2.0 * ell * r + l2 * dr : d_diag;
+        };
+        for (int r = 0; r < tmw; ++r) {
+            const int k = row0 + rw0 + r;
+            if (k >= m) break;
+            double v0, d0, v1, d1;
+            el(k > c ? k - c : c - k, v0, d0);
+            el(k > c + 1 ? k - c - 1 : c + 1 - k, v1, d1);
+            const long o = (long)k * ncols + c;
+            if (vec) {
+                if (O) *reinterpret_cast<double2*>(O + o) = make_double2(v0, v1);
+                if (dO) *reinterpret_cast<double2*>(dO + o) = make_double2(d0, d1);
+            } else {
+                if (O) { O[o] = v0; if (two) O[o + 1] = v1; }
+                if (dO) { dO[o] = d0; if (two) dO[o + 1] = d1; }
+            }
+        }
+        return;
+    }
+    for (int r = 0; r < tmw; ++r) {
+        const int k = row0 + rw0 + r;
+        if (k >= m) break;
+        const double gk = s_grid[rw0 + r], gk1 = s_grid[rw0 + r + 1];
+        double v0, d0, v1 = 0.0, d1 = 0.0;
+        vg_factor_elem(J, kpart, k, c, x0, gk, gk1, ell, v0, d0);
+        if (two) vg_factor_elem(J, kpart, k, c + 1, x1, gk, gk1, ell, v1, d1);
+        const long o = (long)k * ncols + c;
+        if (vec) {
+            if (O) *reinterpret_cast<double2*>(O + o) = make_double2(v0, v1);
+            if (dO) *reinterpret_cast<double2*>(dO + o) = make_double2(d0, d1);
+        } else {
+            if (O) { O[o] = v0; if (two) O[o + 1] = v1; }
+            if (dO) { dO[o] = d0; if (two) dO[o + 1] = d1; }
+        }
+    }
+}
diff --git a/variational_gridded_gaussian_processes_amd/csrc/gemm_body.h b/variational_gridded_gaussian_processes_amd/csrc/gemm_body.h
--- a/variational_gridded_gaussian_processes_amd/csrc/gemm_body.h
+++ b/variational_gridded_gaussian_processes_amd/csrc/gemm_body.h
@@ -1,5 +1,6 @@
 #pragma once
 #include "common.h"
+#include "factor_elem.h"
 
 typedef double vg_d4 __attribute__((ext_vector_type(4)));
 
@@ -12,8 +13,8 @@
     static constexpr int MB = T / 32;
 };
 
-template <int T, int BK, int NT = 256>
-__device__ __forceinline__ void vg_gemm_body(const VgGemmBatch& b, double* lds, const int bid) {
+template <int T, int BK, int NT = 256, bool GEN = false>
+__device__ __forceinline__ void vg_gemm_body(const VgGemmBatch& b, double* lds, const int bid, const VgGemmGenA* gen = nullptr) {
     using C_ = VgTile<T, BK>;
     constexpr int NR = T * BK / NT;
     constexpr int WC = NT / 128;
@@ -78,6 +79,33 @@
     const int a_si = a_kc ? C_::RS : 1, a_sk = a_kc ? 1 : C_::KS;
     const int b_sj = b_nc ? 1 : C_::RS, b_sk = b_nc ? C_::KS : 1;
 
+    const bool gen_a = GEN && gen->prob == pi;
+    double g_row[NR];
+    bool g_d[NR];
+    double g_inv = 0.0;
+    const double* g_x = lds + 2 * C_::TILE;
+    if constexpr (GEN) {
+        if (gen_a) {
+            const VgFactorJob& J = gen->job;
+            g_inv = 1.0 / gen->theta[J.theta_idx];
+#pragma unroll
+            for (int r = 0; r < NR; ++r) {
+                const int gi = row0 + a_i[r];
+                g_d[r] = gi >= J.m;
+                g_row[r] = gi < M ? J.grid[g_d[r] ? gi - J.m : gi] : 0.0;
+            }
+            for (int k = k_begin + tid; k < k_end; k += NT) lds[2 * C_::TILE + (k - k_begin)] = J.x[k];
+            __syncthreads();
+        }
+    }
+    auto gen_el = [&](int r, int gk) -> double {
+        double v = 0.0, dv = 0.0;
+        if constexpr (GEN) {
+            vg_kappa(gen->job.kind, fabs(g_row[r] - g_x[gk - k_begin]), g_inv, v, dv);
+        }
+        return g_d[r] ? dv : v;
+    };
+
     double ra0[NR], rb0[NR], ra1[NR], rb1[NR];
     auto load_tile = [&](int k0, double (&ra)[NR], double (&rb)[NR]) {
         const double* bp[NR];
@@ -88,7 +116,8 @@
             const int gi = row0 + a_i[r], gk = k0 + a_k[r];
             aok[r] = gi < M && gk < k_end;
             ap[r] = A + (aok[r] ? gi * sa_m + gk * sa_k : 0);
-            ra[r] = aok[r] ? ap[r][0] : 0.0;
+            if (GEN && gen_a) ra[r] = aok[r] ? gen_el(r, gk) : 0.0;
+            else ra[r] = aok[r] ? ap[r][0] : 0.0;
             const int gj = col0 + b_j[r], gkb = k0 + b_k[r];
             bok[r] = gj < N && gkb < k_end;
             bp[r] = B + (bok[r] ? gkb * sb_k + gj * sb_n : 0);
@@ -162,9 +191,16 @@
         }
         const long da = (long)BK * sa_k, db = (long)BK * sb_k;
         const int nk = (k_end - k_begin) / BK;
+        int ka = k_begin;
         auto ld = [&](double (&ra)[NR], double (&rb)[NR]) {
-#pragma unroll
-            for (int r = 0; r < NR; ++r) { ra[r] = *pa[r]; rb[r] = *pb[r]; }
+            if (GEN && gen_a) {
+#pragma unroll
+                for (int r = 0; r < NR; ++r) { rb[r] = *pb[r]; ra[r] = gen_el(r, ka + a_k[r]); }
+                ka += BK;
+            } else {
+#pragma unroll
+                for (int r = 0; r < NR; ++r) { ra[r] = *pa[r]; rb[r] = *pb[r]; }
+            }
             for (int sl = 1; sl < nslab; sl += 3) {
                 const long o0 = (long)sl * bslab, o1 = sl + 1 < nslab ? o0 + bslab : o0, o2 = sl + 2 < nslab ? o0 + 2 * bslab : o0;
                 const double w1 = sl + 1 < nslab ? 1.0 : 0.0, w2 = sl + 2 < nslab ? 1.0 : 0.0;
```

New measurement: 5.452 billion grid-points/s (median of 6 runs). Within noise of the previous version (+0.4%).
